# atoms-ufrj/atomsmm

Measured on AMD Instinct MI355X. Metric: ns/day on 100k-atom TIP3P RESPA box; near-nonbonded HBM GB/s vs 8 TB/s peak, higher is better.
Workload: dtype f64

## Files before the change

atomsmm_amd/backend.py:

```python
import ctypes as C
import os

import numpy as np

HERE = os.path.dirname(os.path.abspath(__file__))
LIB_PATH = os.environ.get('AMM_LIB') or os.path.join(HERE, 'libatomsmm_hip.so')

NEAR_NONE, NEAR_SHIFT, NEAR_FSWITCH, DAMPED, NONBONDED, SOFTCORE, LJ_VIRIAL = range(7)
GUARD_RC0, COULOMB_EWALD, COULOMB_RF, SWITCH, NO_SHIFT, GROUP_LJ, GROUP_Q = 1, 2, 4, 8, 16, 32, 64
BOND_HARMONIC, ANGLE_HARMONIC, BOND_LJC, BOND_NEAR, TORSION_PERIODIC, BOND_EWALD_EXCL = range(6)
BOND_VIRIAL_HARMONIC, BOND_VIRIAL_LJ = 6, 7
OP_EVAL, OP_KICK, OP_MOVE, OP_COPY, OP_COMBINE, OP_EXPR, OP_BATH = 1, 2, 3, 4, 5, 6, 7
OP_SAVE_REF, OP_CONSTRAIN_X, OP_CONSTRAIN_V = 8, 9, 10
OP_ALLREDUCE = 11
EXCHANGE_REDUCE, EXCHANGE_GATHER = 0, 1
COMM_ID_BYTES = 128
MAX_SLOTS, SLOT_X, SLOT_V = 64, 62, 63
MAX_STATES = 64
GROUP_ALL = 32
KC = 138.935456
ARITY = {BOND_HARMONIC: 2, ANGLE_HARMONIC: 3, BOND_LJC: 2, BOND_NEAR: 2, TORSION_PERIODIC: 4, BOND_EWALD_EXCL: 2,
         BOND_VIRIAL_HARMONIC: 2, BOND_VIRIAL_LJ: 2}
NPAR = {BOND_HARMONIC: 2, ANGLE_HARMONIC: 2, BOND_LJC: 3, BOND_NEAR: 3, TORSION_PERIODIC: 3, BOND_EWALD_EXCL: 1,
        BOND_VIRIAL_HARMONIC: 2, BOND_VIRIAL_LJ: 3}

EXPORTS = [
    'amm_abi_version', 'amm_last_error', 'amm_create', 'amm_destroy', 'amm_set_stream', 'amm_set_slice',
    'amm_synchronize', 'amm_check', 'amm_pair_create', 'amm_pair_set_params', 'amm_pair_share_list', 'amm_bonded_create',
    'amm_bonded_add_terms', 'amm_bonded_finalize', 'amm_bonded_set_sliced', 'amm_bonded_release', 'amm_force_eval', 'amm_kick',
    'amm_move', 'amm_copy', 'amm_mvv', 'amm_bind_state', 'amm_bind_buffer', 'amm_group_define', 'amm_run_ops',
    'amm_set_fuse_inner', 'amm_set_outer_skin',
    'amm_pair_get_stats', 'amm_profile_enable', 'amm_profile_read', 'amm_pair_count_within', 'amm_pair_row_padding', 'amm_kernel_revision',
    'amm_pme_create', 'amm_pme_set_charges', 'amm_pme_set_sliced', 'amm_pair_set_lambda', 'amm_pair_set_lambda_dev', 'amm_expr_eval', 'amm_expr_eval_scalar', 'amm_expr_define', 'amm_expr_seed', 'amm_bath_define', 'amm_bath_define_nhl', 'amm_bath_define_sin', 'amm_iso_define', 'amm_regulated_define', 'amm_bath_define_regulated', 'amm_pair_energy_derivative', 'amm_constraints_create', 'amm_pair_set_scale',
    'amm_comm_unique_id', 'amm_comm_init', 'amm_comm_destroy', 'amm_comm_allreduce', 'amm_comm_stats', 'amm_group_set_exchange', 'amm_bind_exchange', 'amm_exchange_finish',
    'amm_set_option', 'amm_positions_changed', 'amm_exchange_per', 'amm_run_stats', 'amm_run_ops_from', 'amm_exchange_pending',
    'amm_pair_energy_states',
]


class PairDesc(C.Structure):
    _fields_ = [('family', C.c_int32), ('flags', C.c_int32), ('degree', C.c_int32), ('pad_', C.c_int32),
                ('sign', C.c_double), ('rc', C.c_double), ('rswitch', C.c_double), ('rc0', C.c_double),
                ('rs0', C.c_double), ('alpha', C.c_double), ('Kc', C.c_double), ('krf', C.c_double),
                ('crf', C.c_double)]


class Op(C.Structure):
    _fields_ = [('op', C.c_int32), ('a', C.c_int32), ('b', C.c_int32), ('c', C.c_int32), ('coef', C.c_double)]


class PairStats(C.Structure):
    _fields_ = [('n_builds', C.c_int64), ('n_evals', C.c_int64), ('n_list_pairs', C.c_int64),
                ('n_slice_atoms', C.c_int64), ('capacity', C.c_int32), ('max_neighbors', C.c_int32),
                ('lanes_per_atom', C.c_int32), ('n_cells', C.c_int32), ('rlist', C.c_double),
                ('shares_list', C.c_int32), ('list_kind', C.c_int32), ('n_outer_builds', C.c_int64),
                ('n_outer_pairs', C.c_int64), ('rlist_outer', C.c_double), ('tab_error', C.c_double),
                ('has_table', C.c_int32), ('rode_along', C.c_int32),
                ('has_site_table', C.c_int32), ('n_rest_atoms', C.c_int32), ('site_tab_error', C.c_double),
                ('n_candidates', C.c_int32), ('n_candidate_walks', C.c_int32), ('chargeless', C.c_int32), ('build_split', C.c_int32)]


def slice_per(n, world):
    return 3 * (((n + 2) // 3 + world - 1) // world)


def pair_desc(family, rc, rc0=0.0, rs0=0.0, rswitch=0.0, alpha=0.0, degree=1, flags=0, sign=1.0, Kc=KC,
              krf=0.0, crf=0.0):
    return PairDesc(int(family), int(flags), int(degree), 0, float(sign), float(rc), float(rswitch), float(rc0),
                    float(rs0), float(alpha), float(Kc), float(krf), float(crf))


class HipError(RuntimeError):
    pass


class _LiveSet:

    def __init__(self):
        import weakref
        self._refs = weakref.WeakValueDictionary()

    def add(self, obj):
        self._refs[id(obj)] = obj

    def discard(self, obj):
        self._refs.pop(id(obj), None)

    def close_all(self):
        for obj in list(self._refs.values()):
            try:
                obj.close()
            except Exception:
                pass


_LIVE = _LiveSet()
import atexit
atexit.register(_LIVE.close_all)


_LIB = None


def kernel_revision():
    return lib().amm_kernel_revision().decode()


def lib():
    global _LIB
    if _LIB is None:
        if not os.path.exists(LIB_PATH):
            raise HipError('libatomsmm_hip.so not found at %s: build it with `python -m atomsmm_amd.build` '
                           '(hipcc --offload-arch=gfx950). The HIP path has no CPU fallback.' % LIB_PATH)
        L = C.CDLL(LIB_PATH)
        vp, dp, ip = C.c_void_p, C.POINTER(C.c_double), C.POINTER(C.c_int32)
        L.amm_kernel_revision.restype = C.c_char_p
        revision = L.amm_kernel_revision().decode()
        if revision.endswith('-tune') and os.environ.get('AMM_ALLOW_TUNE') != '1':
            raise HipError('%s is a tuning build (kernel revision %s): rebuild with `python -m atomsmm_amd.build --force`, or set '
                           'AMM_ALLOW_TUNE=1 for a probe script' % (LIB_PATH, revision))
        L.amm_abi_version.restype = C.c_int
        L.amm_last_error.restype = C.c_char_p
        L.amm_create.argtypes = [C.c_int32, dp, C.c_int32, vp, C.POINTER(vp)]
        L.amm_destroy.argtypes = [vp]
        L.amm_set_stream.argtypes = [vp, vp]
        L.amm_set_slice.argtypes = [vp, C.c_int32, C.c_int32]
        L.amm_synchronize.argtypes = [vp]
        L.amm_comm_unique_id.argtypes = [C.c_char_p, C.c_char_p]
        L.amm_comm_init.argtypes = [vp, C.c_char_p, C.c_char_p, C.c_int32, C.c_int32]
        L.amm_comm_allreduce.argtypes = [vp, vp, C.c_int64]
        L.amm_comm_destroy.argtypes = [vp]
        L.amm_comm_stats.argtypes = [vp, C.POINTER(C.c_int64)]
        L.amm_run_stats.argtypes = [vp, C.POINTER(C.c_int64)]
        L.amm_group_set_exchange.argtypes = [vp, C.c_int32, C.c_int32]
        L.amm_bind_exchange.argtypes = [vp, vp, C.c_int64]
        L.amm_exchange_finish.argtypes = [vp]
        L.amm_exchange_pending.argtypes = [vp, C.POINTER(C.c_int32)]
        L.amm_check.argtypes = [vp]
        L.amm_pair_create.argtypes = [vp, C.POINTER(PairDesc), dp, dp, dp, ip, C.c_int32, C.c_double, ip]
# ... 289 lines not shown
                                 int(counter) & (2 ** 64 - 1), _ptr(dst), _ptr(total)))

    def force_eval(self, fid, pos, force, accumulate=False, energy=None):
        _chk(lib().amm_force_eval(self.h, fid, _ptr(pos), _ptr(force), int(bool(accumulate)), _ptr(energy)))

    def kick(self, v, f, mass, coef, fsub=None, fadd=None):
        second = fsub if fsub is not None else fadd
        _chk(lib().amm_kick(self.h, _ptr(v), _ptr(f), _ptr(second), int(fadd is not None), _ptr(mass), float(coef)))

    def move(self, x, v, coef):
        _chk(lib().amm_move(self.h, _ptr(x), _ptr(v), float(coef)))

    def copy(self, dst, src):
        _chk(lib().amm_copy(self.h, _ptr(dst), _ptr(src)))

    def mvv(self, v, mass, out):
        _chk(lib().amm_mvv(self.h, _ptr(v), _ptr(mass), _ptr(out)))

    def bind_state(self, x, v, mass):
        self._keep += [x, v, mass]
        _chk(lib().amm_bind_state(self.h, _ptr(x), _ptr(v), _ptr(mass)))

    def bind_buffer(self, slot, buf):
        self._keep.append(buf)
        _chk(lib().amm_bind_buffer(self.h, slot, _ptr(buf)))

    def group_define(self, group, slot, force_ids):
        ids, p = _hi(np.asarray(force_ids, dtype=np.int32).reshape(-1))
        _chk(lib().amm_group_define(self.h, group, slot, p, len(ids)))

    def group_set_exchange(self, group, mode):
        _chk(lib().amm_group_set_exchange(self.h, int(group), int(mode)))

    def bind_exchange(self, tensor):
        self._keep.append(tensor)
        _chk(lib().amm_bind_exchange(self.h, _ptr(tensor), tensor.numel()))

    def exchange_finish(self):
        _chk(lib().amm_exchange_finish(self.h))

    def run_ops(self, ops, repeat=1):
        arr = (Op * len(ops))(*ops)
        _chk(lib().amm_run_ops(self.h, arr, len(ops), int(repeat)))

    def run_ops_host_exchanges(self, ops, repeat, exchange):
        arr = (Op * len(ops))(*ops)
        cursor = C.c_int64(0)
        total = len(ops) * int(repeat)
        while True:
            _chk(lib().amm_run_ops_from(self.h, arr, len(ops), int(repeat), C.byref(cursor)))
            nf = C.c_int32(0)
            _chk(lib().amm_exchange_pending(self.h, C.byref(nf)))
            if nf.value:
                exchange(nf.value)
            elif cursor.value >= total:
                return

    def set_outer_skin(self, skin_out):
        _chk(lib().amm_set_outer_skin(self.h, float(skin_out)))

    def set_option(self, name, value):
        _chk(lib().amm_set_option(self.h, name.encode(), float(value)))

    def positions_changed(self):
        _chk(lib().amm_positions_changed(self.h))

    def exchange_per(self):
        per = C.c_int32(0)
        _chk(lib().amm_exchange_per(self.h, C.byref(per)))
        return per.value

    def set_fuse_inner(self, on=True):
        _chk(lib().amm_set_fuse_inner(self.h, int(bool(on))))

    def synchronize(self):
        _chk(lib().amm_synchronize(self.h))

    def check(self):
        _chk(lib().amm_check(self.h))

    def pair_stats(self, fid):
        st = PairStats()
        _chk(lib().amm_pair_get_stats(self.h, fid, C.byref(st)))
        return {name: getattr(st, name) for name, _ in PairStats._fields_}

    def pair_row_padding(self, fid):
        out = (C.c_int64 * 2)()
        _chk(lib().amm_pair_row_padding(self.h, fid, out))
        return int(out[0]), int(out[1])

    def pair_count_within(self, fid, pos, r_within):
        n = C.c_int64()
        _chk(lib().amm_pair_count_within(self.h, fid, _ptr(pos), float(r_within), C.byref(n)))
        return n.value

    def profile_enable(self, on=True, only=None):
        _chk(lib().amm_profile_enable(self.h, -(int(only) + 1) if (on and only is not None) else int(bool(on))))

    def profile_read(self, fid):
        n = C.c_int64(); ms = C.c_double()
        _chk(lib().amm_profile_read(self.h, fid, C.byref(n), C.byref(ms)))
        return n.value, ms.value
```

atomsmm_amd/csrc/abi.hip:

```cpp
#include <algorithm>
#include <cmath>
#include <cstring>
#include <numeric>

#include "amm_ctx.h"
#include "cluster.h"

int amm_pair_setup_grid(amm_ctx *ctx, PairForce *pf);
static bool amm_family_allows_cluster(int family, int flags) {
    const bool tab_family = family == AMM_NEAR_NONE || family == AMM_NEAR_SHIFT || family == AMM_NEAR_FSWITCH || family == AMM_DAMPED || family == AMM_NONBONDED;
    return tab_family && !(flags & (AMM_GROUP_LJ | AMM_GROUP_Q));
}
int amm_bonded_arity(int kind);
int amm_bonded_npar(int kind);

static thread_local std::string g_error;
void amm_set_error(const std::string &msg) { g_error = msg; }

static PairForce *get_pair(amm_ctx *ctx, int id) {
    if (!ctx || id < 0 || id >= (int)ctx->forces.size() || ctx->forces[id].type != 1) {
        amm_set_error("invalid pair force id");
        return nullptr;
    }
    return ctx->forces[id].pair;
// ... 1647 lines not shown
                if (amm_bath_impl(ctx, ctx->baths[op.a], ctx->d_v, (1ull << 63) | ++ctx->expr_counter)) return 1;
            } break;
            case AMM_OP_ALLREDUCE: {
                auto bound = [&](const amm_op &o) { return o.a >= 0 && o.a < AMM_MAX_SLOTS && ctx->slots[o.a]; };
                if (!bound(op)) {
                    amm_set_error("amm_run_ops: ALLREDUCE of an unbound buffer");
                    return 1;
                }
                const size_t n3 = 3 * (size_t)ctx->n;
                double *lo = ctx->slots[op.a];
                size_t count = n3;
                while (k + 1 < n_ops && ops[k + 1].op == AMM_OP_ALLREDUCE && bound(ops[k + 1])) {
                    double *nb = ctx->slots[ops[k + 1].a];
                    if (nb == lo + count) count += n3;
                    else if (nb + n3 == lo) { lo = nb; count += n3; }
                    else break;
                    ++k;
                }
                if (amm_comm_allreduce_impl(ctx, lo, count)) return 1;
            } break;
            default: amm_set_error("amm_run_ops: unknown op"); return 1;
            }
        }
    }
    if (flush_deferred()) return 1;
    if (cursor && !yielded) *cursor = total_ops;
    if (!yielded && !ctx->own_only.empty()) {
        const std::vector<const double *> left = ctx->own_only;
        for (const double *b : left)
            if (complete(b)) return 1;
    }
    if (swapped) {
        const size_t bytes = sizeof(double) * 3 * (size_t)ctx->n;
        AMM_HIP(hipMemcpyAsync(user_x, ctx->d_x, bytes, hipMemcpyDeviceToDevice, ctx->stream));
        AMM_HIP(hipMemcpyAsync(user_v, ctx->d_v, bytes, hipMemcpyDeviceToDevice, ctx->stream));
        AMM_HIP(hipMemcpyAsync(user_f0, ctx->slots[f0_slot], bytes, hipMemcpyDeviceToDevice, ctx->stream));
    }
    bindings.restore(false);
    return 0;
}

int amm_pair_get_stats(amm_ctx *ctx, int32_t force_id, amm_pair_stats *out) {
    PairForce *pf = get_pair(ctx, force_id);
    if (!pf || !out) return 1;
    std::memset(out, 0, sizeof(*out));
    AMM_HIP(hipStreamSynchronize(ctx->stream));
    out->n_evals = pf->n_evals;
    PairForce *L = pf->host ? pf->host : pf;
    out->capacity = L->cap;
    out->lanes_per_atom = L->lpa;
    out->n_cells = L->grid.ncell;
    out->rlist = pf->rlist;
    out->n_slice_atoms = L->s_end - L->s_begin;
    out->shares_list = pf->host ? 1 : 0;
    out->list_kind = L->last_kind;
    out->tab_error = pf->tab_error;
    out->has_table = (pf->pc.tab.nint > 0 && pf->d_tab) ? 1 : 0;
    out->rode_along = pf->last_fused;
    out->chargeless = pf->last_chargeless;
    out->build_split = (L->cl && L->last_kind != 0) ? L->cl->split_parts : 0;
    out->has_site_table = (ctx->opt_site_tab && pf->d_tab_ss && pf->pc.tab.ss_first >= 0) ? 1 : 0;
    out->site_tab_error = pf->ss_error;
    out->n_rest_atoms = L->hybrid ? L->n_rest : 0;
    if (pf->small) {
        int cs[2];
        if (amm_small_group_stats(pf->small, cs)) return 1;
        out->n_candidates = cs[0];
        out->n_candidate_walks = cs[1];
    }
    if (L->last_kind >= 1 && L->cl && L->cl->built) {
        ClusterList *cl = L->cl;
        int flags[8];
        unsigned long long cnt[8];
        AMM_HIP(hipMemcpy(flags, cl->d_flags, sizeof(flags), hipMemcpyDeviceToHost));
        AMM_HIP(hipMemcpy(cnt, cl->d_counters, sizeof(cnt), hipMemcpyDeviceToHost));
        out->capacity = cl->cap;
        out->lanes_per_atom = cl->lpa;
        out->n_cells = cl->grid.ncell;
        out->n_slice_atoms = 3 * (int64_t)(cl->c_end - cl->c_begin);
        out->n_builds = (int64_t)cnt[0];
        out->n_list_pairs = 9 * (int64_t)(pf->host ? cnt[2] : cnt[1]);
        out->max_neighbors = flags[2];
        out->rlist_outer = L->desc.rc + L->skin;
        if (L->last_kind == 2 && L->rest && L->rest->built) {
            AMM_HIP(hipMemcpy(cnt, L->rest->d_counters, sizeof(cnt), hipMemcpyDeviceToHost));
            out->n_list_pairs += (int64_t)(pf->host ? cnt[2] : cnt[1]);
        }
        return 0;
    }
    if (L->built) {
        int flags[8];
        unsigned long long cnt[8];
        AMM_HIP(hipMemcpy(flags, L->d_flags, sizeof(flags), hipMemcpyDeviceToHost));
        AMM_HIP(hipMemcpy(cnt, L->d_counters, sizeof(cnt), hipMemcpyDeviceToHost));
        out->n_builds = (int64_t)cnt[0];
        out->n_outer_builds = (int64_t)cnt[4];
        out->n_outer_pairs = (int64_t)cnt[3];
        out->rlist_outer = L->desc.rc + L->skin_out;
        out->n_list_pairs = (int64_t)(pf->host ? cnt[2] : cnt[1]);
        out->max_neighbors = flags[2];
    }
    return 0;
}

int amm_pair_row_padding(amm_ctx *ctx, int32_t force_id, int64_t out[2]) {
    PairForce *pf = get_pair(ctx, force_id);
    if (!pf || !out) {
        amm_set_error("amm_pair_row_padding: null argument or not a pair force");
        return 1;
    }
    PairForce *L = pf->host ? pf->host : pf;
    out[0] = out[1] = 0;
    if (!(L->last_kind >= 1 && L->cl && L->cl->built)) return 0;
    long long v[2];
    if (amm_cluster_row_padding_impl(ctx, pf, v)) return 1;
    out[0] = v[0];
    out[1] = v[1];
    return 0;
}

int amm_pair_count_within(amm_ctx *ctx, int32_t force_id, const double *d_pos, double r_within, int64_t *count) {
    PairForce *pf = get_pair(ctx, force_id);
    if (!pf || !d_pos || !count) {
        amm_set_error("amm_pair_count_within: null argument or not a pair force");
        return 1;
    }
    long long c = 0;
    PairForce *Lw = pf->host ? pf->host : pf;
    if (Lw->last_kind >= 1 && Lw->cl && Lw->cl->built) {
        if (amm_cluster_count_within_impl(ctx, pf, d_pos, r_within, &c)) return 1;
        if (Lw->last_kind == 2 && pf->rest && Lw->rest && Lw->rest->built) {
            long long c2 = 0;
            if (amm_pair_count_within_impl(ctx, pf->rest, d_pos, r_within, &c2)) return 1;
            c += c2;
        }
    } else if (amm_pair_count_within_impl(ctx, pf, d_pos, r_within, &c)) return 1;
    *count = (int64_t)c;
    return 0;
}

const char *amm_kernel_revision(void) { return amm_kernel_revision_impl(); }

int amm_set_outer_skin(amm_ctx *ctx, double skin_out) {
    ctx->skin_out = skin_out;
    return 0;
}

int amm_set_option(amm_ctx *ctx, const char *name, double value) {
    if (!ctx || !name) {
        amm_set_error("amm_set_option: null argument");
        return 1;
    }
    const std::string k(name);
    const int v = (int)value;
    if (k == "cluster") ctx->opt_cluster = v;
    else if (k == "hybrid") ctx->opt_hybrid = v;
    else if (k == "small_group") ctx->opt_small_group = v;
    else if (k == "mixed_terms") ctx->opt_mixed_terms = v;
    else if (k == "rest_skin_factor") ctx->opt_rest_skin_factor = value;
    else if (k == "tab") ctx->opt_tab = v;
    else if (k == "site_trips") ctx->site_trips = v != 0;
    else if (k == "lanes_per_row") ctx->opt_lpa = v;
    else if (k == "build_parts") ctx->opt_parts = v;
    else if (k == "build_split") ctx->opt_build_split = v;
    else if (k == "unroll") ctx->opt_unroll = v;
    else if (k == "dual_unroll") ctx->opt_dual_unroll = v;
    else if (k == "tab_block") ctx->opt_tab_bs = v;
    else if (k == "tab_dual_block") ctx->opt_tab_dual_bs = v;
    else if (k == "no_dual") ctx->opt_no_dual = v;
    else if (k == "fuse_rows") ctx->opt_fuse_rows = v;
    else if (k == "row_phases") ctx->opt_row_phases = v;
    else if (k == "group_candidates") ctx->opt_group_candidates = v;
    else if (k == "positions_private") ctx->opt_positions_private = v;
    else if (k == "site_tab") ctx->opt_site_tab = v;
    else if (k == "no_defer") ctx->opt_no_defer = v;
    else if (k == "terms_from") ctx->opt_terms_from = v;
    else if (k == "no_term_lanes") ctx->opt_no_term_lanes = v;
    else if (k == "fuse_epilogue") ctx->opt_fuse_epilogue = v;
    else if (k == "comm_timeout") ctx->opt_comm_timeout = value;
    else if (k == "spec_assign") ctx->opt_spec_assign = v;
    else if (k == "chargeless") ctx->opt_chargeless = v;
    else if (k == "state_exchange") ctx->opt_state_exchange = v;
    else {
        amm_set_error("amm_set_option: unknown option '" + k + "'");
        return 1;
    }
    return 0;
}

int amm_run_stats(amm_ctx *ctx, int64_t out[4]) {
    if (!ctx || !out) return 1;
    out[0] = ctx->n_epilogues;
    out[1] = ctx->n_copies_current;
    out[2] = ctx->n_state_exchanges;
    out[3] = 0;
    return 0;
}

int amm_exchange_per(amm_ctx *ctx, int32_t *per) {
    if (!ctx || !per) return 1;
    *per = amm_slice_per(ctx->n, ctx->world);
    return 0;
}

int amm_set_fuse_inner(amm_ctx *ctx, int32_t on) {
    ctx->fuse_inner = on != 0;
    return 0;
}

int amm_profile_enable(amm_ctx *ctx, int32_t on) {
    ctx->profile = on != 0;
    ctx->profile_only = on < 0 ? -on - 1 : -1;
    return 0;
}

int amm_profile_read(amm_ctx *ctx, int32_t force_id, int64_t *n_launches, double *total_ms) {
    PairForce *pf = get_pair(ctx, force_id);
    if (!pf) return 1;
    AMM_HIP(hipStreamSynchronize(ctx->stream));
    double tot = 0.0;
    for (size_t k = 0; k + 1 < pf->ev_used; k += 2) {
        float ms = 0.f;
        AMM_HIP(hipEventElapsedTime(&ms, pf->ev[k], pf->ev[k + 1]));
        tot += ms;
    }
    if (n_launches) *n_launches = (int64_t)(pf->ev_used / 2);
    pf->ev_used = 0;
    if (pf->rest) {
        PairForce *rc = pf->rest;
        for (size_t k = 0; k + 1 < rc->ev_used; k += 2) {
            float ms = 0.f;
            AMM_HIP(hipEventElapsedTime(&ms, rc->ev[k], rc->ev[k + 1]));
            tot += ms;
        }
        rc->ev_used = 0;
    }
    if (total_ms) *total_ms = tot;
    return 0;
}

}
```

atomsmm_amd/csrc/amm_ctx.h:

```cpp
#pragma once
#include <hip/hip_runtime.h>

#include <cstdint>
#include <string>
#include <vector>

#include "../../include/atomsmm_hip.h"

#define AMM_WAVE 64
#define AMM_MAX_PRE 6
#define AMM_DERIV_LAMBDA 1024
#define AMM_MAX_GROUPS 33

void amm_set_error(const std::string &msg);
#define AMM_HIP(call)                                                                            \
    do {                                                                                         \
        hipError_t e_ = (call);                                                                  \
        if (e_ != hipSuccess) {                                                                  \
            amm_set_error(std::string(#call) + ": " + hipGetErrorString(e_));                    \
            return 1;                                                                            \
        }                                                                                        \
    } while (0)

struct PairTab {
// ... 200 lines not shown
};

struct RegDef {
    bool on = false;
    double alpha = 1, an_kT = 0;
};

struct IsoDef {
    bool on = false;
    double LkT = 0, Q1 = 0;
    int slot = -1;
};

struct GroupDef {
    int slot = -1;
    std::vector<int> forces;
    int exchange = 0;
};

struct PendingExchange {
    bool active = false;
    int per = 0, nf = 0;
    const int *perm = nullptr;
    double *force = nullptr, *gforce = nullptr;
    int kind = 0;
    ClusterList *cl = nullptr;
    PairForce *next = nullptr;
};

#define AMM_MAX_WATCH 4
struct ListWatch {
    const double *xref = nullptr;
    double thr2 = 0;
    int *flags = nullptr;
    long *pre_epoch = nullptr;
    const double **pre_pos = nullptr;
};

static inline int amm_slice_per(int n, int world) {
    const int nc = (n + 2) / 3;
    return 3 * ((nc + world - 1) / world);
}

struct EpiPlan {
    BondedSet *bs = nullptr;
    double *f0 = nullptr;
    int npre = 0, niter = 0;
    const double *pre_a[AMM_MAX_PRE] = {nullptr}, *pre_b[AMM_MAX_PRE] = {nullptr};
    double pre_coef[AMM_MAX_PRE] = {0};
    int pre_plus[AMM_MAX_PRE] = {0};
    double c1 = 0, d = 0, c2 = 0;
    PairForce *next = nullptr;
    int kind = 0;
    int with_move = 0;
    double dcoef = 0;
};

struct amm_ctx {
    int n = 0;
    int opt_spec_assign = 1;
    int opt_state_exchange = 1;
    int opt_chargeless = 1;
    int opt_fuse_epilogue = 1;
    const EpiPlan *epi_request = nullptr;
    bool epi_done = false;
    long long n_epilogues = 0;
    long long n_state_exchanges = 0;
    std::vector<const double *> own_only;
    long long n_copies_current = 0;
    int opt_cluster = 1;
    int opt_hybrid = 1;
    double opt_rest_skin_factor = 2.0;
    int opt_mixed_terms = 1;
    int opt_small_group = 1;
    bool creating_rest = false;
    int opt_tab = 1;
    int opt_build_split = 0;
    int opt_lpa = 0, opt_parts = 0, opt_unroll = 2, opt_dual_unroll = 2, opt_tab_bs = 0, opt_tab_dual_bs = 0;
    int opt_site_tab = 1;
    CZeroRows zero_rows = CZeroRows{0, nullptr, nullptr, nullptr};
    int opt_positions_private = 0;
    int opt_group_candidates = 1;
    int opt_row_phases = 1;
    int opt_fuse_rows = 1;
    int opt_no_dual = 0, opt_no_defer = 0, opt_terms_from = 8192, opt_no_term_lanes = 0;
    ListWatch watched[AMM_MAX_WATCH];
    int n_watched = 0;
    int device = 0;
    hipStream_t stream = nullptr;
    Box box;
    int rank = 0, world = 1;
    std::vector<ForceObj> forces;
    double *d_x = nullptr, *d_v = nullptr;
    const double *d_mass = nullptr;
    double *slots[AMM_MAX_SLOTS] = {nullptr};
    GroupDef groups[AMM_MAX_GROUPS];
    bool profile = false;
    int profile_only = -1;
    double *d_scratch = nullptr;
    double *d_expr_part = nullptr;
    double *d_fscratch = nullptr;
    ConstraintSet *constraints = nullptr;
    std::vector<ExprDef> exprs;
    std::vector<BathDef> baths;
    IsoDef iso;
    RegDef reg;
    unsigned long long expr_seed = 0, expr_counter = 0;
    double *alt_x = nullptr, *alt_v = nullptr, *alt_f = nullptr;
    bool fuse_inner = true;
    bool site_trips = true;
    long pos_epoch = 0;
    double skin_out = -1.0;
    void *comm = nullptr;
    bool comm_failed = false;
    double opt_comm_timeout = 0;
    double *d_xchg = nullptr;
    long long xchg_doubles = 0;
    PendingExchange pending;
    long long comm_calls = 0, comm_doubles = 0;
};

struct KickList {
    const double *f[4], *f2[4];
    int plus[4];
    double coef[4];
    int n;
};

#define AMM_FLAG_FAR 12
struct WatchArgs {
    int n;
    const double *xref[AMM_MAX_WATCH];
    double thr2[AMM_MAX_WATCH];
    int *flags[AMM_MAX_WATCH];
};
void amm_collect_watches(amm_ctx *ctx, WatchArgs &W);
void amm_watch_moved(amm_ctx *ctx);

int amm_comm_unique_id_impl(const char *rccl_path, unsigned char *out);
int amm_comm_init_impl(amm_ctx *ctx, const char *rccl_path, const unsigned char *id_bytes, int rank, int world);
int amm_comm_destroy_impl(amm_ctx *ctx);
int amm_comm_poll_impl(amm_ctx *ctx);
int amm_comm_wait_impl(amm_ctx *ctx, const char *who);
int amm_comm_allreduce_impl(amm_ctx *ctx, double *d_buf, size_t count);
int amm_comm_allgather_impl(amm_ctx *ctx, double *d_buf, size_t count_per_rank);
int amm_exchange_finish_impl(amm_ctx *ctx);

int amm_small_group_setup(amm_ctx *ctx, PairForce *pf, const std::vector<float> &member);
int amm_small_group_eval_impl(amm_ctx *ctx, PairForce *pf, const double *d_pos, double *d_force, int accumulate, double *d_energy,
                              BondedSet *carry_terms = nullptr, const double **own_rows = nullptr, int rows_unused = 0);
bool amm_small_group_supported(const PairForce *pf);
int amm_small_group_energy_states(amm_ctx *ctx, PairForce *pf, const double *d_pos, const double *d_lambdas, int K, double *d_out);
int amm_small_group_free(SmallGroup *sg);
int amm_small_group_failed(SmallGroup *sg);
int amm_small_group_stats(SmallGroup *sg, int out[2]);
int amm_pair_build_consts(const amm_pair_desc &d, PairConsts &pc);
int amm_pair_eval_impl(amm_ctx *ctx, PairForce *pf, const double *d_pos, double *d_force, int accumulate,
                       double *d_energy, PairForce *guest = nullptr, double *g_force = nullptr, int g_accumulate = 0,
                       int exchange = 0);
bool amm_pair_can_eval_dual(amm_ctx *ctx, PairForce *guest, PairForce *host);
bool amm_pair_can_fuse_discount(amm_ctx *ctx, PairForce *guest, PairForce *host);
int amm_pair_free(PairForce *pf);
int amm_pair_build_table(PairForce *pf);
int amm_pair_count_within_impl(amm_ctx *ctx, PairForce *pf, const double *d_pos, double r_within, long long *count);
const char *amm_kernel_revision_impl();
int amm_bonded_eval_impl(amm_ctx *ctx, BondedSet *bs, const double *d_pos, double *d_force, int accumulate,
                         double *d_energy);
int amm_bonded_finalize_impl(amm_ctx *ctx, BondedSet *bs);
int amm_bonded_eval_kicks_impl(amm_ctx *ctx, BondedSet *bs, const double *d_pos, double *d_force, int accumulate, const KickList &K,
                               int with_move, double dcoef, int terms_done = 0, const double *pair_rows = nullptr);
int amm_bonded_free(BondedSet *bs);
int amm_kicks_move_impl(amm_ctx *ctx, const double *const *fa, const double *const *fb, const int *plus, const double *coef, int nk,
                        int with_move, double dcoef);
int amm_inner_components_impl(amm_ctx *ctx, BondedSet *bs, double *x, double *v, double *f0, int npre, const double *const *pre_a,
                              const double *const *pre_b, const double *pre_coef, const int *pre_plus, double c1, double d,
                              double c2, int niter, const BathDef *bath = nullptr, double d2 = 0.0);
int amm_bath_impl(amm_ctx *ctx, const BathDef &bath, double *d_v, unsigned long long counter);
int amm_isokick_impl(amm_ctx *ctx, double *d_v, const double *d_f, const double *d_f2, int plus, const double *d_mass, double coef);
int amm_constraints_create_impl(amm_ctx *ctx, const int32_t *h_pairs, const double *h_dist, int n_cons, double tol,
                                ConstraintSet **out);
int amm_constraints_save_reference(amm_ctx *ctx, ConstraintSet *cs, const double *d_x);
int amm_constrain_positions(amm_ctx *ctx, ConstraintSet *cs, double *d_x);
int amm_constrain_velocities(amm_ctx *ctx, ConstraintSet *cs, const double *d_x, double *d_v);
int amm_constraints_failed(amm_ctx *ctx, ConstraintSet *cs);
int amm_constraints_free(ConstraintSet *cs);
int amm_fused_inner_impl(amm_ctx *ctx, BondedSet *bs, const double *x_in, const double *v_in, const double *f_in,
                         double *x_out, double *v_out, double *f_out, double c1, double d, double c2);
int amm_pme_create_impl(amm_ctx *ctx, double alpha, const int *K, double Kc, const double *h_q, PmeForce **out);
int amm_pme_set_charges_impl(amm_ctx *ctx, PmeForce *pm, const double *h_q);
int amm_pme_eval_impl(amm_ctx *ctx, PmeForce *pm, const double *d_pos, double *d_force, int accumulate, double *d_energy);
int amm_pme_set_sliced_impl(PmeForce *pm, int on);
int amm_pme_free(PmeForce *pm);
int amm_expr_eval_scalar_impl(amm_ctx *ctx, const int32_t *code, int n_code, const double *consts, int n_consts, double *d_scalars,
                              int n_scalars);
int amm_expr_eval_impl(amm_ctx *ctx, const int32_t *code, int n_code, const double *consts, int n_consts, const double *globals,
                       int n_globals, unsigned long long seed, unsigned long long counter, double *d_dst, double *d_sum);
int amm_kick_impl(amm_ctx *ctx, double *d_v, const double *d_f, const double *d_f2, int plus, const double *d_mass, double coef);
int amm_combine_impl(amm_ctx *ctx, double *d_dst, const double *d_a, const double *d_b, double coef);
int amm_move_impl(amm_ctx *ctx, double *d_x, const double *d_v, double coef);
int amm_copy_impl(amm_ctx *ctx, double *d_dst, const double *d_src);
int amm_mvv_impl(amm_ctx *ctx, const double *d_v, const double *d_m, double *d_out);
int amm_reduce_add(amm_ctx *ctx, const double *d_part, int n, double scale, double *d_out);
```

atomsmm_amd/csrc/bonded.hip:

```cpp
#include <algorithm>
#include <cmath>
#include <type_traits>
#include <cstring>

#include "amm_ctx.h"
#include "cluster.h"
#include "expr_vm.h"
#include "pair_math.h"

#include "bonded_terms.h"

template <class P, bool LOCAL = false>
__device__ __forceinline__ void bonded_atom(const BondedArgs &A, const P &pos, int iglobal, int i, double *f, double &esum) {
    const int rb = A.ref_ptr[iglobal], re = A.ref_ptr[iglobal + 1];
    for (int r = rb; r < re; ++r) {
        const int4 at = LOCAL ? A.rec_l[r] : A.rec_a[r];
        const double4 q = A.rec_q[r];
        const long long code = __double_as_longlong(q.w);
        const int kind = (int)(code & 7), role = (int)((code >> 3) & 3), periodic = (int)((code >> 5) & 1);
        const int ix[4] = {at.x, at.y, at.z, at.w};
        const double p[3] = {q.x, q.y, q.z};
        double fo[4][3], e;
        bonded_term_forces(A, pos, ix, p, kind, periodic, fo, e);
#pragma unroll
// ... 467 lines not shown
            const int ix[4] = {al.x, al.y, al.z, al.w};
            const double p[3] = {q.x, q.y, q.z};
            double fo[4][3], e;
            bonded_term_forces(A, pos, ix, p, kind, periodic, fo, e);
#pragma unroll
            for (int xx = 0; xx < 3; ++xx)
                f[xx] += role == 0 ? fo[0][xx] : (role == 1 ? fo[1][xx] : (role == 2 ? fo[2][xx] : fo[3][xx]));
        };
        if (TERMS) {
            double fo[4][3] = {{0.0, 0.0, 0.0}, {0.0, 0.0, 0.0}, {0.0, 0.0, 0.0}, {0.0, 0.0, 0.0}};
            if (my_tl.x >= 0) {
                const long long code = __double_as_longlong(my_tq.w);
                const int ix[4] = {my_tl.x, my_tl.y, my_tl.z, my_tl.w};
                const double p[3] = {my_tq.x, my_tq.y, my_tq.z};
                double e;
                bonded_term_forces(A, pos, ix, p, HONLY ? (int)(code & 1) : (int)(code & 7), (int)((code >> 5) & 1), fo, e);
            }
#pragma unroll
            for (int r = 0; r < (HONLY ? 3 : 4); ++r)
#pragma unroll
                for (int xx = 0; xx < 3; ++xx) s_out[TERMS ? r * 3 + xx : 0][TERMS ? threadIdx.x : 0] = fo[r][xx];
            __builtin_amdgcn_fence(__ATOMIC_RELEASE, "wavefront");
            __builtin_amdgcn_wave_barrier();
            __builtin_amdgcn_fence(__ATOMIC_ACQUIRE, "wavefront");
            const double *so = &s_out[0][0];
#pragma unroll
            for (int t = 0; t < 4; ++t)
                if (t < rec_n) {
                    f[0] += so[TERMS ? rec_at[t] : 0];
                    f[1] += so[TERMS ? rec_at[t] + 256 : 0];
                    f[2] += so[TERMS ? rec_at[t] + 512 : 0];
                }
            if (rec_n > 4) {
                unsigned long long rr = my_recs >> 20;
                for (int t = 4; t < rec_n; ++t) {
                    const int rcode = (int)(rr & 31ull);
                    rr >>= 5;
                    const int src = gbase + (rcode & 7), row = 3 * (rcode >> 3);
                    f[0] += s_out[TERMS ? row : 0][TERMS ? src : 0];
                    f[1] += s_out[TERMS ? row + 1 : 0][TERMS ? src : 0];
                    f[2] += s_out[TERMS ? row + 2 : 0][TERMS ? src : 0];
                }
            }
        } else
        for (int t = 0; t < nrec; ++t) {
            const bool cached = t < MAXR;
            const int4 al = cached ? s_tl[cached ? t : 0][threadIdx.x] : A.rec_l[rb + t];
            const double4 q = cached ? s_tq[cached ? t : 0][threadIdx.x] : A.rec_q[rb + t];
            do_rec(al, q);
        }
        {
#pragma clang fp contract(off)
#pragma unroll
            for (int j = 0; j < 3; ++j) {
                if (ISO && C.iso) {
                    amm_iso_kick(v[j], u1[j], f[j], m, C.c2, C.iso_LkT, C.iso_Q1);
                    continue;
                }
                const double num = C.c2 * f[j];
                const double dv = amm_div_mass(num, m, rm, rok);
                v[j] = v[j] + dv;
            }
        }
    }
    if (has) {
#pragma unroll
        for (int j = 0; j < 3; ++j) {
            C.x[3 * a + j] = x[j];
            C.v[3 * a + j] = v[j];
            C.f0[3 * a + j] = f[j];
        }
        if (BATH) {
            if (C.bath_kind >= 1) {
#pragma unroll
                for (int j = 0; j < 3; ++j) C.bath_w[3 * a + j] = w[j];
            }
        }
        if (ISO && C.iso) {
#pragma unroll
            for (int j = 0; j < 3; ++j) C.iso_v1[3 * a + j] = u1[j];
        }
        for (int q = 0; q < C.nwatch; ++q) {
            const double dx = x[0] - C.wref[q][3 * a], dy = x[1] - C.wref[q][3 * a + 1], dz = x[2] - C.wref[q][3 * a + 2];
            const double d2 = dx * dx + dy * dy + dz * dz;
            if (!(d2 <= C.wthr2[q])) {
                C.wflags[q][0] = 1;
                if (!(d2 <= 4.0 * C.wthr2[q])) C.wflags[q][AMM_FLAG_FAR] = 1;
            }
        }
    }
}

static const int kArity[8] = {2, 3, 2, 2, 4, 2, 2, 2};
static const int kNpar[8] = {2, 2, 3, 3, 3, 1, 2, 3};

int amm_bonded_finalize_impl(amm_ctx *ctx, BondedSet *bs) {
    const int n = ctx->n;
    std::vector<int> cnt(n + 1, 0);
    for (int kind = 0; kind < 8; ++kind) {
        const int nt = (int)bs->h_idx[kind].size() / kArity[kind];
        bs->n_terms[kind] = nt;
        for (int t = 0; t < nt; ++t)
            for (int r = 0; r < kArity[kind]; ++r) {
                int a = bs->h_idx[kind][t * kArity[kind] + r];
                if (a < 0 || a >= n) {
                    amm_set_error("bonded term references an atom index out of range");
                    return 1;
                }
                cnt[a + 1]++;
            }
        if (nt >= (1 << 26)) {
            amm_set_error("too many bonded terms of one kind");
            return 1;
        }
    }
    for (int i = 0; i < n; ++i) cnt[i + 1] += cnt[i];
    const size_t nref = (size_t)cnt[n];
    std::vector<int4> rec_a(nref);
    std::vector<double4> rec_q(nref);
    std::vector<int> rec_src(nref);
    std::vector<int> fill(cnt.begin(), cnt.end() - 1);
    int gterm = 0;
    for (int kind = 0; kind < 8; ++kind)
        for (int t = 0; t < bs->n_terms[kind]; ++t, ++gterm)
            for (int r = 0; r < kArity[kind]; ++r) {
                const int a = bs->h_idx[kind][t * kArity[kind] + r];
                const size_t slot = (size_t)fill[a]++;
                rec_src[slot] = gterm * 4 + r;
                int at[4] = {-1, -1, -1, -1};
                for (int k = 0; k < kArity[kind]; ++k) at[k] = bs->h_idx[kind][t * kArity[kind] + k];
                rec_a[slot] = make_int4(at[0], at[1], at[2], at[3]);
                double pr[3] = {0.0, 0.0, 0.0};
                for (int k = 0; k < kNpar[kind]; ++k) pr[k] = bs->h_par[kind][(size_t)t * kNpar[kind] + k];
                const long long code = (long long)kind | ((long long)r << 3) | ((long long)(bs->periodic[kind] ? 1 : 0) << 5);
                double w;
                std::memcpy(&w, &code, sizeof(w));
                rec_q[slot] = make_double4(pr[0], pr[1], pr[2], w);
            }
    std::vector<int> parent(n);
    for (int i = 0; i < n; ++i) parent[i] = i;
    auto find = [&](int a) {
        while (parent[a] != a) {
            parent[a] = parent[parent[a]];
            a = parent[a];
        }
        return a;
    };
    for (int kind = 0; kind < 8; ++kind)
        for (int t = 0; t < bs->n_terms[kind]; ++t)
            for (int r = 1; r < kArity[kind]; ++r) {
                int a = find(bs->h_idx[kind][t * kArity[kind]]), b = find(bs->h_idx[kind][t * kArity[kind] + r]);
                if (a != b) parent[std::max(a, b)] = std::min(a, b);
            }
    std::vector<int> comp_of(n), csize;
    std::vector<int> root_to_comp(n, -1);
    for (int i = 0; i < n; ++i) {
        int r = find(i);
        if (root_to_comp[r] < 0) {
            root_to_comp[r] = (int)csize.size();
            csize.push_back(0);
        }
        comp_of[i] = root_to_comp[r];
        csize[comp_of[i]]++;
    }
    const int ncomp = (int)csize.size();
    int maxc = 0;
    for (int c2 = 0; c2 < ncomp; ++c2) maxc = std::max(maxc, csize[c2]);
    std::vector<int> comp_ptr(ncomp + 1, 0), comp_atoms(n), local_of(n);
    for (int c2 = 0; c2 < ncomp; ++c2) comp_ptr[c2 + 1] = comp_ptr[c2] + csize[c2];
    {
        std::vector<int> fillc(comp_ptr.begin(), comp_ptr.end() - 1);
// ... 509 lines not shown
```

atomsmm_amd/csrc/bonded_terms.h:

```cpp
#pragma once
#include "amm_ctx.h"
#include "pair_math.h"

struct BondedArgs {
    int n, row_begin, row_end;
    const int *ref_ptr;
    const int4 *rec_a;
    const double4 *rec_q;
    const int4 *rec_l;
    const double *pos;
    double *force;
    double *epart;
    int accumulate, want_energy;
    Box box;
    PairConsts near_pc;
    double ewald_alpha, ewald_tasp;
    double Kc_ljc;
};

struct PosPlain {
    const double *pos;
    __device__ __forceinline__ double get(int a, int k) const { return pos[3 * a + k]; }
};
struct PosAdvanced {
    const double *x, *v, *f, *m;
    double c1, d;
    __device__ __forceinline__ double vel(int a, int k) const {
#pragma clang fp contract(off)
        const double num = c1 * f[3 * a + k];
        const double dv = num / m[a];
        return v[3 * a + k] + dv;
    }
    __device__ __forceinline__ double get(int a, int k) const {
#pragma clang fp contract(off)
        const double dx = d * vel(a, k);
        return x[3 * a + k] + dx;
    }
};

__device__ __forceinline__ double amm_reg_dx(double v, double m, double coef, double alpha, double an_kT) {
#pragma clang fp contract(off)
    const double c = sqrt(an_kT / m);
    const double t = tanh((alpha * v) / c);
    return (c * t) * coef;
}

__device__ __forceinline__ void amm_watch_atom(const WatchArgs &W, int a, const double *xn) {
    for (int q = 0; q < W.n; ++q) {
        const double dx = xn[0] - W.xref[q][3 * a], dy = xn[1] - W.xref[q][3 * a + 1], dz = xn[2] - W.xref[q][3 * a + 2];
        const double d2 = dx * dx + dy * dy + dz * dz;
        if (!(d2 <= W.thr2[q])) {
            W.flags[q][0] = 1;
            if (!(d2 <= 4.0 * W.thr2[q])) W.flags[q][AMM_FLAG_FAR] = 1;
        }
    }
}

__device__ __forceinline__ double amm_div_mass(double num, double m, double r, bool exact_r) {
    const double q = num * r;
    const double e = fma(-q, m, num);
    const double fast = fma(e, r, q);
    if (__builtin_amdgcn_ballot_w64(!exact_r) == 0ull) return fast;
    return exact_r ? fast : num / m;
}

struct PosLds {
    const double *sx, *sy, *sz;
    __device__ __forceinline__ double get(int slot, int k) const { return k == 0 ? sx[slot] : (k == 1 ? sy[slot] : sz[slot]); }
};

template <class P>
__device__ __forceinline__ void delta3(const P &pos, int a, int b, const Box &box, int periodic, double *d) {
#pragma unroll
    for (int k = 0; k < 3; ++k) {
        double v = pos.get(a, k) - pos.get(b, k);
        if (periodic) v = amm_min_image(v, box.L[k], box.invL[k]);
        d[k] = v;
    }
}
__device__ __forceinline__ double dot3(const double *a, const double *b) { return a[0] * b[0] + a[1] * b[1] + a[2] * b[2]; }
__device__ __forceinline__ void cross3(const double *a, const double *b, double *c) {
    c[0] = a[1] * b[2] - a[2] * b[1];
    c[1] = a[2] * b[0] - a[0] * b[2];
    c[2] = a[0] * b[1] - a[1] * b[0];
}

template <class P>
__device__ __forceinline__ void bonded_term_forces(const BondedArgs &A, const P &pos, const int *ix, const double *p, int kind,
                                                   int periodic, double fo[4][3], double &e) {
    switch (kind) {
    case AMM_BOND_HARMONIC: {
        double d[3];
        delta3(pos, ix[0], ix[1], A.box, periodic, d);
        const double r2 = dot3(d, d);
        const double rinv = amm_rsqrt(r2);
        const double dr = r2 * rinv - p[0];
        const double fr = -p[1] * dr * rinv;
#pragma unroll
        for (int x = 0; x < 3; ++x) {
            fo[0][x] = fr * d[x];
            fo[1][x] = -fo[0][x];
        }
        e = 0.5 * p[1] * dr * dr;
    } break;
    case AMM_ANGLE_HARMONIC: {
        double d1[3], d2[3];
        delta3(pos, ix[0], ix[1], A.box, periodic, d1);
        delta3(pos, ix[2], ix[1], A.box, periodic, d2);
        const double i1 = amm_rsqrt(dot3(d1, d1)), i2 = amm_rsqrt(dot3(d2, d2));
        double c = dot3(d1, d2) * i1 * i2;
        c = c > 1.0 ? 1.0 : (c < -1.0 ? -1.0 : c);
        const double th = acos(c), dth = th - p[0];
        double s2 = 1.0 - c * c;
        if (s2 < 1e-24) s2 = 1e-24;
        const double g = p[1] * dth * amm_rsqrt(s2);
#pragma unroll
        for (int x = 0; x < 3; ++x) {
            const double u1 = d1[x] * i1, u2 = d2[x] * i2;
            const double fi = g * (u2 - c * u1) * i1;
            const double fk = g * (u1 - c * u2) * i2;
            fo[0][x] = fi;
            fo[2][x] = fk;
            fo[1][x] = -(fi + fk);
        }
        e = 0.5 * p[1] * dth * dth;
    } break;
    case AMM_BOND_LJC:
    case AMM_BOND_NEAR: {
        double d[3];
        delta3(pos, ix[0], ix[1], A.box, periodic, d);
        const double r2 = dot3(d, d);
        double fr;
        if (kind == AMM_BOND_LJC) {
            const double rinv2 = 1.0 / r2, rinv = sqrt(rinv2);
            const double s2 = p[1] * p[1] * rinv2, x6 = s2 * s2 * s2;
            e = 4.0 * p[2] * x6 * (x6 - 1.0) + A.Kc_ljc * p[0] * rinv;
            fr = (4.0 * p[2] * (12.0 * x6 * x6 - 6.0 * x6) + A.Kc_ljc * p[0] * rinv) * rinv2;
// ... 76 lines not shown
```

atomsmm_amd/csrc/cluster.h:

```cpp
#pragma once
#include "amm_ctx.h"

struct ClusterList {
    int nc = 0;
    const int *d_first = nullptr;
    const int *d_rest = nullptr;
    int nrest = 0;
    bool built = false;
    CellGrid grid;
    int capc = 0;
    int parts = 1;
    int *d_slice_cells = nullptr;
    int split_parts = 0;
    double rext = 0;
    double rlist_build = 0, rnear_build = 0, skin = 0;
    int *d_cell_count = nullptr, *d_cell_start = nullptr, *d_cell_members = nullptr;
    int *d_cperm = nullptr;
    int *d_aperm = nullptr;
    float4 *d_pos4f = nullptr;
    double *d_xref = nullptr;
    int c_begin = 0, c_end = 0;
    int cap = 0;
    int lpa = 8;
    int *d_nl = nullptr, *d_nnb = nullptr, *d_nnb_near = nullptr;
    int *d_flags = nullptr;
    unsigned long long *d_counters = nullptr;
    unsigned long long *d_blockstats = nullptr;
    int *d_ticket = nullptr;
    long checked_epoch = -1, pre_epoch = -1;
    const double *checked_pos = nullptr, *pre_pos = nullptr;
    PairForce *sorted_for = nullptr;
    long sorted_epoch = -1;
    const double *sorted_pos = nullptr;
    int *d_spec_count[2] = {nullptr, nullptr};
    int *d_spec_ticket = nullptr;
    int spec_parity = 0;
    long assigned_epoch = -1;
    const double *assigned_pos = nullptr;
    bool per_pair_image = false;
};

void amm_cluster_classify(int n, const std::vector<int> &excl_ptr, const std::vector<int> &excl_idx, std::vector<int> &mol_first,
                          std::vector<int> &rest);
int amm_cluster_eval_impl(amm_ctx *ctx, PairForce *pf, const double *d_pos, double *d_force, int accumulate, PairForce *guest,
                          double *g_force, int g_accumulate, int exchange);
int amm_cluster_count_within_impl(amm_ctx *ctx, PairForce *pf, const double *d_pos, double r_within, long long *count);
int amm_cluster_row_padding_impl(amm_ctx *ctx, PairForce *pf, long long out[2]);
int amm_cluster_state_finish_impl(amm_ctx *ctx);
int amm_cluster_free(ClusterList *cl);
```

atomsmm_amd/csrc/cluster.hip:

```cpp
#include <algorithm>
#include <cmath>
#include <cstdio>
#include <cstdlib>
#include <cstring>
#include <type_traits>
#include <vector>

#include "amm_ctx.h"
#include "bonded_terms.h"
#include "cluster.h"
#include "device_utils.h"
#include "pair_math.h"
#include "pair_tab.h"

#ifndef AMM_EXP_NOLJ
#define AMM_EXP_NOLJ 0
#endif

__device__ double amm_erfcx_table_dev_c[AMM_ERFCX_NI * AMM_ERFCX_NC];
static bool g_erfcx_uploaded_c[64] = {false};

void amm_cluster_classify(int n, const std::vector<int> &ptr, const std::vector<int> &idx, std::vector<int> &mol_first, std::vector<int> &rest) {
    mol_first.clear();
    rest.clear();
    auto own_pairs_only = [&](int i, int i0) {
        if (ptr[i + 1] - ptr[i] != 2) return false;
        const int a = i - i0;
        const int p0 = i0 + (a == 0 ? 1 : 0), p1 = i0 + (a == 2 ? 1 : 2);
        const int e0 = idx[ptr[i]], e1 = idx[ptr[i] + 1];
        return (e0 == p0 && e1 == p1) || (e0 == p1 && e1 == p0);
    };
    int i = 0;
    while (i < n) {
        if (i + 2 < n && own_pairs_only(i, i) && own_pairs_only(i + 1, i) && own_pairs_only(i + 2, i)) {
            mol_first.push_back(i);
            i += 3;
        } else {
            rest.push_back(i);
            i += 1;
        }
    }
}

__device__ __forceinline__ double cwrap1(double x, double L, double invL) {
    double w = x - L * floor(x * invL);
    if (w >= L) w -= L;
    if (w < 0.0) w = 0.0;
    return w;
}

__global__ void k_ccheck_displacement(int n, const double *__restrict__ pos, const double *__restrict__ xref, double thr2, int *flags) {
    const int i = blockIdx.x * blockDim.x + threadIdx.x;
    if (i >= n) return;
    const double dx = pos[3 * i] - xref[3 * i], dy = pos[3 * i + 1] - xref[3 * i + 1], dz = pos[3 * i + 2] - xref[3 * i + 2];
    const double d2 = dx * dx + dy * dy + dz * dz;
    if (!(d2 <= thr2)) {
        flags[0] = 1;
        if (!(d2 <= 4.0 * thr2)) flags[AMM_FLAG_FAR] = 1;
    }
}

__device__ __forceinline__ int cfirst(const int *__restrict__ first, int m) { return first ? first[m] : 3 * m; }

__global__ void __launch_bounds__(256) k_cassign(int nc, const double *__restrict__ pos, Box box, CellGrid g, int *count, int *start,
                                                 int *members, int capc, double *xref, int *flags, int *ticket, int force,
                                                 const int *__restrict__ first, const int *__restrict__ rest, int nrest) {
    if (!force && !flags[0]) return;
    const int m = blockIdx.x * blockDim.x + threadIdx.x;
    if (m >= nc && m < nc + nrest && xref) {
        const int i = rest[m - nc];
#pragma unroll
        for (int k = 0; k < 3; ++k) xref[3 * i + k] = pos[3 * i + k];
    }
    if (m < nc) {
        const int i0 = cfirst(first, m);
        int cidx[3];
#pragma unroll
        for (int k = 0; k < 3; ++k) {
            const double w = cwrap1(pos[3 * i0 + k], box.L[k], box.invL[k]);
            const int ck = (w == w) ? (int)(w * g.inv_cw[k]) : 0;
            cidx[k] = ck >= g.nc[k] ? g.nc[k] - 1 : (ck < 0 ? 0 : ck);
        }
        const int cell = (cidx[2] * g.nc[1] + cidx[1]) * g.nc[0] + cidx[0];
        const int rank = atomicAdd(&count[cell], 1);
        if (members) {
            if (rank < capc) members[(size_t)cell * capc + rank] = m;
            else flags[7] = 1;
        }
    }
    if (!amm_last_block(ticket)) return;
    const int fullest = amm_block_scan_counts(g.ncell, count, start);
    if (threadIdx.x == 0) flags[6] = fullest;
}

__device__ __forceinline__ double csorted_image(double x, double x0, double sh, double L, double invL) {
    return x + (sh - L * rint((x - x0) * invL));
}

__device__ __forceinline__ void cgather_one(int c, int i0, const double *__restrict__ pos, Box box, const double *__restrict__ q,
                                            const double *__restrict__ hsig, const double *__restrict__ seps2, double4 *posq_s, double2 *lj_s) {
    double sh[3];
#pragma unroll
    for (int k = 0; k < 3; ++k) sh[k] = cwrap1(pos[3 * i0 + k], box.L[k], box.invL[k]) - pos[3 * i0 + k];
#pragma unroll
    for (int a = 0; a < 3; ++a) {
        const int i = i0 + a;
        double4 p;
        p.x = csorted_image(pos[3 * i], pos[3 * i0], sh[0], box.L[0], box.invL[0]);
        p.y = csorted_image(pos[3 * i + 1], pos[3 * i0 + 1], sh[1], box.L[1], box.invL[1]);
        p.z = csorted_image(pos[3 * i + 2], pos[3 * i0 + 2], sh[2], box.L[2], box.invL[2]);
        p.w = q[i];
        posq_s[3 * c + a] = p;
        lj_s[3 * c + a] = make_double2(hsig[i], seps2[i]);
    }
}

__global__ void __launch_bounds__(256) k_csort_gather(int ncell, int nc, const int *__restrict__ start, const int *__restrict__ members,
                                                      int capc, int *cperm, int *aperm, const double *__restrict__ pos, Box box,
                                                      float4 *pos4f, const int *flags, int *wflags, int force, const double *__restrict__ q,
                                                      const double *__restrict__ hsig, const double *__restrict__ seps2, double4 *posq_s,
                                                      double2 *lj_s, float rext, const double *__restrict__ site_eps,
                                                      const int *__restrict__ first, CZeroRows Z, int copies_current, double *xref,
                                                      int c_begin, int c_end, int *slice_cells) {
    const int gid = blockIdx.x * blockDim.x + threadIdx.x;
    if (gid < Z.n) {
        const int i = Z.idx[gid];
        if (Z.f0) Z.f0[3 * i] = Z.f0[3 * i + 1] = Z.f0[3 * i + 2] = 0.0;
        if (Z.f1) Z.f1[3 * i] = Z.f1[3 * i + 1] = Z.f1[3 * i + 2] = 0.0;
    }
    if (!force && !flags[0]) {
        if (!copies_current && posq_s && gid < nc) cgather_one(gid, cfirst(first, cperm[gid]), pos, box, q, hsig, seps2, posq_s, lj_s);
        return;
    }
    const int wave = gid >> 6, lane = threadIdx.x & 63;
    if (wave >= ncell) return;
    const int b = start[wave];
    const int cnt = min(start[wave + 1] - b, capc);
    if (lane == 0 && c_begin < c_end) {
        if (b <= c_begin && c_begin < start[wave + 1]) slice_cells[0] = wave;
        if (b <= c_end - 1 && c_end - 1 < start[wave + 1]) slice_cells[1] = wave;
    }
    const int *mem = members + (size_t)wave * capc;
    for (int a0 = 0; a0 < cnt; a0 += 64) {
        const int a = a0 + lane;
        const int me = a < cnt ? mem[a] : 0x7fffffff;
        int rank = 0;
        for (int k0 = 0; k0 < cnt; k0 += 64) {
            const int kk = k0 + lane;
            const int other = kk < cnt ? mem[kk] : 0x7fffffff;
            const int nk = min(64, cnt - k0);
            for (int jj = 0; jj < nk; ++jj) rank += __builtin_amdgcn_readlane(other, jj) < me;
        }
        if (a >= cnt) continue;
        const int sl = b + rank;
        cperm[sl] = me;
        const int i0 = cfirst(first, me);
        double sh[3], p0[3];
#pragma unroll
        for (int k = 0; k < 3; ++k) {
            p0[k] = pos[3 * i0 + k];
            sh[k] = cwrap1(p0[k], box.L[k], box.invL[k]) - p0[k];
        }
        float ext2 = 0.f;
        int sites = 0;
        float4 pf[3];
#pragma unroll
        for (int t = 0; t < 3; ++t) {
            const int i = i0 + t;
            aperm[3 * sl + t] = i;
            const double x = csorted_image(pos[3 * i], p0[0], sh[0], box.L[0], box.invL[0]);
            const double y = csorted_image(pos[3 * i + 1], p0[1], sh[1], box.L[1], box.invL[1]);
            const double z = csorted_image(pos[3 * i + 2], p0[2], sh[2], box.L[2], box.invL[2]);
            if (xref) {
                xref[3 * i] = pos[3 * i];
                xref[3 * i + 1] = pos[3 * i + 1];
                xref[3 * i + 2] = pos[3 * i + 2];
            }
            pf[t] = make_float4((float)x, (float)y, (float)z, 0.f);
            const float dx = pf[t].x - pf[0].x, dy = pf[t].y - pf[0].y, dz = pf[t].z - pf[0].z;
            ext2 = fmaxf(ext2, dx * dx + dy * dy + dz * dz);
            if (site_eps[i] != 0.0) sites |= 1 << t;
            if (posq_s) {
                posq_s[3 * sl + t] = make_double4(x, y, z, q[i]);
                lj_s[3 * sl + t] = make_double2(hsig[i], seps2[i]);
            }
        }
        const float ext = sqrtf(ext2) * 1.000001f + 1e-6f;
        if (!(ext <= rext)) wflags[7] = 1;
        pf[0].w = ext;
        pf[1].w = __int_as_float(sites);
        pos4f[3 * sl] = pf[0];
        pos4f[3 * sl + 1] = pf[1];
        pos4f[3 * sl + 2] = pf[2];
    }
}

struct CBoxF {
    float L[3], invL[3];
};

#ifndef CB_BATCH
#define CB_BATCH 5
#endif
#define CB_COARSE 256
#define CB_QCAP 256
__device__ __forceinline__ int cq_wrap(int i) { return i & (CB_QCAP - 1); }
typedef float v2f __attribute__((ext_vector_type(2)));

__device__ void cfinish_build_block(int *flags, unsigned long long *counters, const unsigned long long *blockstats, int nblocks, int count_only) {
    __shared__ unsigned long long sh_part[4][3];
    unsigned long long sum = 0, mx = 0, nr = 0;
    for (int b0 = threadIdx.x; b0 < nblocks; b0 += 8 * 256) {
        unsigned long long v[8][3];
#pragma unroll
        for (int j = 0; j < 8; ++j) {
            const int b = b0 + j * 256;
            const bool in = b < nblocks;
#pragma unroll
            for (int q = 0; q < 3; ++q) v[j][q] = in ? amm_ld_l2(&blockstats[3 * (in ? b : 0) + q]) : 0ull;
        }
#pragma unroll
        for (int j = 0; j < 8; ++j) {
            sum += v[j][0];
            mx = max(mx, v[j][1]);
            nr += v[j][2];
        }
    }
    for (int off = 32; off > 0; off >>= 1) {
        sum += __shfl_xor(sum, off);
        nr += __shfl_xor(nr, off);
        mx = max(mx, __shfl_xor(mx, off));
    }
    if ((threadIdx.x & 63) == 0) {
        sh_part[threadIdx.x >> 6][0] = sum;
        sh_part[threadIdx.x >> 6][1] = mx;
        sh_part[threadIdx.x >> 6][2] = nr;
    }
    __syncthreads();
    if (threadIdx.x == 0) {
        flags[2] = (int)max(max(sh_part[0][1], sh_part[1][1]), max(sh_part[2][1], sh_part[3][1]));
        counters[1] = sh_part[0][0] + sh_part[1][0] + sh_part[2][0] + sh_part[3][0];
        counters[2] = sh_part[0][2] + sh_part[1][2] + sh_part[2][2] + sh_part[3][2];
        if (!count_only) {
            flags[0] = 0;
            flags[AMM_FLAG_FAR] = 0;
            counters[0] += 1;
        }
    }
}

#ifndef CB_WAVES
#define CB_WAVES 5
#endif
#define CB_OCC __attribute__((amdgpu_waves_per_eu(CB_WAVES)))
#ifdef AMM_CBS_TIMING
__device__ unsigned long long g_cbs_t[8];
#define CBS_STAMP(i) do { const unsigned long long now_ = wall_clock64(); if (w == 0 && lane == 0) atomicAdd(&g_cbs_t[i], now_ - t_last); t_last = now_; } while (0)
#else
#define CBS_STAMP(i) do { } while (0)
#endif
template <bool COUNT_ONLY, bool RINT, bool SLICE = false>
__global__ void __launch_bounds__(256) __attribute__((amdgpu_waves_per_eu(SLICE ? 3 : CB_WAVES))) k_cbuild(int c_begin, int c_end, int parts, const int *__restrict__ cell_start,
                                                const float4 *__restrict__ pos4f, CBoxF box, CellGrid g, float rlist, float rnear2, int cap,
                                                int *nl, int *nnb, int *nnb_near, int *flags, unsigned long long *blockstats,
                                                unsigned long long *counters, int *ticket, int force, const int *slice_cells) {
    if (!force && !flags[0]) return;
    __shared__ int s_rstart[4][128];
    __shared__ int s_rpref[4][128];
    __shared__ float s_rshift[4][3][128];
    __shared__ int s_q[4][CB_BATCH][CB_QCAP];
    __shared__ unsigned char s_coarse[4][CB_COARSE];
    const int lane = threadIdx.x & 63, w = threadIdx.x >> 6;
    const int wave = __builtin_amdgcn_readfirstlane((int)((blockIdx.x * blockDim.x + threadIdx.x) >> 6));
    const float FAR = 1.0e9f;
    const float rlist2 = rlist * rlist;
    unsigned long long wsum = 0, wnear = 0;
    int wmax = 0;
    const int first_cell = SLICE ? __builtin_amdgcn_readfirstlane(slice_cells[0]) : 0;
    const int nunits = SLICE ? (__builtin_amdgcn_readfirstlane(slice_cells[1]) - first_cell + 1) * parts : g.ncell * parts;
    int unit = wave;
#ifdef AMM_CBS_TIMING
    unsigned long long t_last = wall_clock64(), t_drain = 0, n_drain = 0;
#endif
    do {
    const int c = unit < nunits ? first_cell + unit / parts : g.ncell, part = unit % parts;
    int a_begin = 0, a_end = 0;
    if (c < g.ncell) {
        const int cb0 = __builtin_amdgcn_readfirstlane(cell_start[c]), cb1 = __builtin_amdgcn_readfirstlane(cell_start[c + 1]);
        const int per = (cb1 - cb0 + parts - 1) / parts;
        a_begin = max(cb0 + part * per, c_begin);
        a_end = min(min(cb0 + (part + 1) * per, cb1), c_end);
    }
    if (a_begin < a_end) {
        const int ncx = g.nc[0], ncy = g.nc[1], ncz = g.nc[2];
        const int cx = c % ncx, cy = (c / ncx) % ncy, cz = c / (ncx * ncy);
        const int nsx = g.nstencil[0], nsy = g.nstencil[1], ne = nsx * nsy * g.nstencil[2];
        int total;
        {
            int ecs[2] = {0, 0}, len[2] = {0, 0}, inc[2];
            float esx[2] = {0.f, 0.f}, esy[2] = {0.f, 0.f}, esz[2] = {0.f, 0.f};
#pragma unroll
            for (int hh = 0; hh < 2; ++hh) {
                const int e = lane + 64 * hh;
                if (e < ne) {
                    const int ox = e % nsx, oy = (e / nsx) % nsy, oz = e / (nsx * nsy);
                    int nz = ncz < 2 * g.h[2] + 1 ? oz : cz - g.h[2] + oz;
                    esz[hh] = nz < 0 ? -box.L[2] : (nz >= ncz ? box.L[2] : 0.f);
                    nz = nz < 0 ? nz + ncz : (nz >= ncz ? nz - ncz : nz);
                    int ny = ncy < 2 * g.h[1] + 1 ? oy : cy - g.h[1] + oy;
                    esy[hh] = ny < 0 ? -box.L[1] : (ny >= ncy ? box.L[1] : 0.f);
                    ny = ny < 0 ? ny + ncy : (ny >= ncy ? ny - ncy : ny);
                    int nx = ncx < 2 * g.h[0] + 1 ? ox : cx - g.h[0] + ox;
                    esx[hh] = nx < 0 ? -box.L[0] : (nx >= ncx ? box.L[0] : 0.f);
                    nx = nx < 0 ? nx + ncx : (nx >= ncx ? nx - ncx : nx);
                    const int cc = (nz * ncy + ny) * ncx + nx;
                    ecs[hh] = cell_start[cc];
                    len[hh] = cell_start[cc + 1] - ecs[hh];
                }
                inc[hh] = len[hh];
                for (int off = 1; off < 64; off <<= 1) {
                    const int v = __shfl_up(inc[hh], off);
                    if (lane >= off) inc[hh] += v;
                }
            }
            const int lower = __builtin_amdgcn_readlane(inc[0], 63);
            total = lower + __builtin_amdgcn_readlane(inc[1], 63);
#pragma unroll
            for (int hh = 0; hh < 2; ++hh) {
                s_rstart[w][lane + 64 * hh] = ecs[hh];
                s_rpref[w][lane + 64 * hh] = (hh ? lower : 0) + inc[hh] - len[hh];
                s_rshift[w][0][lane + 64 * hh] = esx[hh];
                s_rshift[w][1][lane + 64 * hh] = esy[hh];
                s_rshift[w][2][lane + 64 * hh] = esz[hh];
            }
            __builtin_amdgcn_fence(__ATOMIC_RELEASE, "wavefront");
            __builtin_amdgcn_wave_barrier();
            __builtin_amdgcn_fence(__ATOMIC_ACQUIRE, "wavefront");
        }
        int cshift = 3;
        while (((total + 127) >> cshift) > CB_COARSE) ++cshift;
#pragma unroll
        for (int q = 0; q < CB_COARSE / 64; ++q) {
            const int idx = (lane + 64 * q) << cshift;
            int r = 0;
#pragma unroll
            for (int step = 64; step > 0; step >>= 1)
                if (s_rpref[w][r + step] <= idx) r += step;
            s_coarse[w][lane + 64 * q] = (unsigned char)r;
// ... 8 lines not shown
            const int nt = min(CB_BATCH, a_end - tb);
            float4 my = make_float4(0.f, 0.f, 0.f, 0.f);
            if (lane < 3 * nt) my = pos4f[3 * tb + lane];
            int row_cnt = 0;
            int q_head = 0, q_cnt = 0;
            auto rl = [&](float v, int l) { return __int_as_float(__builtin_amdgcn_readlane(__float_as_int(v), l)); };
            auto drain = [&](int t, int n) {
#ifdef AMM_CBS_TIMING
                const unsigned long long t_d0 = wall_clock64();
                n_drain++;
#endif
                const int head = __builtin_amdgcn_readlane(q_head, t);
                int slot[2];
                bool v[2];
                float4 A[2][3];
#pragma unroll
                for (int u = 0; u < 2; ++u) {
                    const bool v0 = lane + 64 * u < n;
                    slot[u] = v0 ? s_q[w][t][cq_wrap(head + lane + 64 * u)] : tb + t;
                    v[u] = v0 && slot[u] != tb + t;
                }
#pragma unroll
                for (int u = 0; u < 2; ++u)
#pragma unroll
                    for (int b = 0; b < 3; ++b) A[u][b] = pos4f[3 * slot[u] + b];
                const int sites[2] = {__float_as_int(A[0][1].w), __float_as_int(A[1][1].w)};
                float px[3], py[3], pz[3];
#pragma unroll
                for (int a = 0; a < 3; ++a) {
                    px[a] = rl(my.x, 3 * t + a);
                    py[a] = rl(my.y, 3 * t + a);
                    pz[a] = rl(my.z, 3 * t + a);
                }
                v2f ax[3], ay[3], az[3];
#pragma unroll
                for (int b = 0; b < 3; ++b) {
                    ax[b] = v2f{A[0][b].x, A[1][b].x};
                    ay[b] = v2f{A[0][b].y, A[1][b].y};
                    az[b] = v2f{A[0][b].z, A[1][b].z};
                }
                if (!RINT) {
                    const v2f sx = box.L[0] * __builtin_elementwise_rint((ax[0] - px[0]) * box.invL[0]);
                    const v2f sy = box.L[1] * __builtin_elementwise_rint((ay[0] - py[0]) * box.invL[1]);
                    const v2f sz = box.L[2] * __builtin_elementwise_rint((az[0] - pz[0]) * box.invL[2]);
#pragma unroll
                    for (int b = 0; b < 3; ++b) {
                        ax[b] -= sx;
                        ay[b] -= sy;
                        az[b] -= sz;
                    }
                }
                v2f m2 = v2f{3.0e38f, 3.0e38f};
#pragma unroll
                for (int a = 0; a < 3; ++a)
#pragma unroll
                    for (int b = 0; b < 3; ++b) {
                        v2f dx = px[a] - ax[b], dy = py[a] - ay[b], dz = pz[a] - az[b];
                        if (RINT) {
                            dx -= box.L[0] * __builtin_elementwise_rint(dx * box.invL[0]);
                            dy -= box.L[1] * __builtin_elementwise_rint(dy * box.invL[1]);
                            dz -= box.L[2] * __builtin_elementwise_rint(dz * box.invL[2]);
                        }
                        v2f r2 = dx * dx;
                        r2 = __builtin_elementwise_fma(dy, dy, r2);
                        r2 = __builtin_elementwise_fma(dz, dz, r2);
                        m2 = __builtin_elementwise_min(m2, r2);
                    }
#pragma unroll
                for (int u = 0; u < 2; ++u) {
                    const float m2u = u ? m2.y : m2.x;
                    const bool pass = v[u] && m2u < rlist2;
                    const unsigned long long m_pass = __builtin_amdgcn_ballot_w64(pass);
                    if (m_pass != 0ull) {
                        const bool is_near = pass && m2u < rnear2;
                        const unsigned long long m_near = __builtin_amdgcn_ballot_w64(is_near);
                        const int np_ = __popcll(m_pass), nn_ = __popcll(m_near);
                        const int c2 = __builtin_amdgcn_readlane(row_cnt, t);
                        const int cnt = c2 & 0xffff, cntf = (int)((unsigned)c2 >> 16);
                        if (!COUNT_ONLY) {
                            const int mp = __builtin_amdgcn_mbcnt_hi((unsigned)(m_pass >> 32), __builtin_amdgcn_mbcnt_lo((unsigned)m_pass, 0u));
                            const int mn = __builtin_amdgcn_mbcnt_hi((unsigned)(m_near >> 32), __builtin_amdgcn_mbcnt_lo((unsigned)m_near, 0u));
                            const int pos_near = cnt + mn, pos_far = (cap - 1 - cntf) - (mp - mn);
                            if (cnt + cntf + np_ <= cap) {
                                int *row_out = nl + (size_t)(tb + t - c_begin) * cap;
                                if (pass) row_out[is_near ? pos_near : pos_far] = slot[u] | (sites[u] << 29);
                            }
                        }
                        row_cnt = lane == t ? c2 + nn_ + ((np_ - nn_) << 16) : row_cnt;
                    }
                }
                q_head = lane == t ? cq_wrap(head + n) : q_head;
                q_cnt = lane == t ? q_cnt - n : q_cnt;
#ifdef AMM_CBS_TIMING
                t_drain += wall_clock64() - t_d0;
#endif
            };
            auto fetch = [&](int cb, float4 (&cand)[2], int (&js)[2]) {
#pragma unroll
                for (int u = 0; u < 2; ++u) {
                    const int idx = cb + u * 64 + lane;
                    const bool in = idx < total;
                    int r = s_coarse[w][idx >> cshift];
                    while (r < 127 && s_rpref[w][r + 1] <= idx) ++r;
                    const int slot = in ? s_rstart[w][r] + idx - s_rpref[w][r] : 0;
                    float4 q = pos4f[3 * slot];
                    if (!RINT) {
                        const float sx = s_rshift[w][0][r], sy = s_rshift[w][1][r], sz = s_rshift[w][2][r];
                        q.x = in ? q.x + sx : FAR;
                        q.y = in ? q.y + sy : FAR;
                        q.z = in ? q.z + sz : FAR;
                    } else if (!in) {
                        q.w = -1.0e9f;
                    }
                    cand[u] = q;
                    js[u] = slot;
                }
            };
            float4 cand[2], cand_n[2];
            int js[2], js_n[2];
            fetch(0, cand, js);
            const float plim_l = my.w + rlist;
            for (int cb = 0; cb < total; cb += 128) {
                if (cb + 128 < total) fetch(cb + 128, cand_n, js_n);
                const v2f cx = v2f{cand[0].x, cand[1].x}, cy = v2f{cand[0].y, cand[1].y}, cz = v2f{cand[0].z, cand[1].z};
                const v2f cw = v2f{cand[0].w, cand[1].w};
                for (int t = 0; t < nt; ++t) {
                    const float p0x = rl(my.x, 3 * t), p0y = rl(my.y, 3 * t), p0z = rl(my.z, 3 * t), plim = rl(plim_l, 3 * t);
                    int qn = __builtin_amdgcn_readlane(q_cnt, t);
                    const int head = __builtin_amdgcn_readlane(q_head, t);
                    v2f dx = p0x - cx, dy = p0y - cy, dz = p0z - cz;
                    if (RINT) {
                        dx -= box.L[0] * __builtin_elementwise_rint(dx * box.invL[0]);
                        dy -= box.L[1] * __builtin_elementwise_rint(dy * box.invL[1]);
                        dz -= box.L[2] * __builtin_elementwise_rint(dz * box.invL[2]);
                    }
                    v2f r2 = dx * dx;
                    r2 = __builtin_elementwise_fma(dy, dy, r2);
                    r2 = __builtin_elementwise_fma(dz, dz, r2);
                    const v2f lim = plim + cw;
                    const v2f lim2 = lim * lim;
#pragma unroll
                    for (int u = 0; u < 2; ++u) {
                        const bool pass = (u ? r2.y < lim2.y : r2.x < lim2.x) && (!RINT || (u ? lim.y : lim.x) > 0.f);
                        const unsigned long long m = __builtin_amdgcn_ballot_w64(pass);
                        if (m == 0ull) continue;
                        const int at = qn + __builtin_amdgcn_mbcnt_hi((unsigned)(m >> 32), __builtin_amdgcn_mbcnt_lo((unsigned)m, 0u));
                        if (pass) s_q[w][t][cq_wrap(head + at)] = js[u];
                        qn += __popcll(m);
                    }
                    q_cnt = lane == t ? qn : q_cnt;
                    if (qn >= 128) {
                        __builtin_amdgcn_fence(__ATOMIC_RELEASE, "wavefront");
                        __builtin_amdgcn_wave_barrier();
                        __builtin_amdgcn_fence(__ATOMIC_ACQUIRE, "wavefront");
                        drain(t, 128);
                    }
                }
#pragma unroll
                for (int u = 0; u < 2; ++u) {
                    cand[u] = cand_n[u];
                    js[u] = js_n[u];
                }
            }
            __builtin_amdgcn_fence(__ATOMIC_RELEASE, "wavefront");
            __builtin_amdgcn_wave_barrier();
            __builtin_amdgcn_fence(__ATOMIC_ACQUIRE, "wavefront");
            for (int t = 0; t < nt; ++t) {
                const int n = __builtin_amdgcn_readlane(q_cnt, t);
                if (n > 0) drain(t, n);
            }
            __builtin_amdgcn_fence(__ATOMIC_RELEASE, "wavefront");
            __builtin_amdgcn_wave_barrier();
            if (lane < nt) {
                const int count = row_cnt & 0xffff, countf = (int)((unsigned)row_cnt >> 16);
                const int total_nb = count + countf;
                if (!COUNT_ONLY) {
                    const bool over = total_nb > cap;
                    nnb[tb + lane - c_begin] = over ? 0 : total_nb;
                    nnb_near[tb + lane - c_begin] = over ? 0 : count;
                    if (over) flags[1] = 1;
                }
                wsum += (unsigned long long)total_nb;
                wnear += (unsigned long long)count;
                wmax = max(wmax, total_nb);
            }
        }
    }
#ifdef AMM_CBS_TIMING
    if (SLICE && lane == 0 && a_begin < a_end) { atomicAdd(&g_cbs_t[1], wall_clock64() - t_last); atomicAdd(&g_cbs_t[2], t_drain); atomicAdd(&g_cbs_t[3], n_drain); }
#endif
    unit += (int)(gridDim.x * (blockDim.x >> 6));
    } while (SLICE && unit < nunits);
    for (int off = 32; off > 0; off >>= 1) {
        wsum += __shfl_xor(wsum, off);
        wnear += __shfl_xor(wnear, off);
        wmax = max(wmax, __shfl_xor(wmax, off));
    }
    __shared__ unsigned long long s_sum[4], s_near[4];
    __shared__ int s_max[4];
    if (lane == 0) {
        s_sum[w] = wsum;
        s_near[w] = wnear;
        s_max[w] = wmax;
    }
    __syncthreads();
    if (threadIdx.x == 0) {
        amm_st_l2(&blockstats[3 * blockIdx.x], s_sum[0] + s_sum[1] + s_sum[2] + s_sum[3]);
        amm_st_l2(&blockstats[3 * blockIdx.x + 1], (unsigned long long)max(max(s_max[0], s_max[1]), max(s_max[2], s_max[3])));
        amm_st_l2(&blockstats[3 * blockIdx.x + 2], s_near[0] + s_near[1] + s_near[2] + s_near[3]);
    }
    if (amm_last_block(ticket)) cfinish_build_block(flags, counters, blockstats, (int)gridDim.x, COUNT_ONLY ? 1 : 0);
}

#ifndef CBS_BATCH
#define CBS_BATCH 3
#endif
#ifndef CBS_SEG
#define CBS_SEG 384
#endif
#define CBS_MAXCH (4 * CBS_SEG / 128)
template <bool RINT>
__global__ void __launch_bounds__(256) k_cbuild_split(int c_begin, int c_end, int parts, const int *__restrict__ cell_start,
                                                      const float4 *__restrict__ pos4f, CBoxF box, CellGrid g, float rlist, float rnear2, int cap,
                                                      int *nl, int *nnb, int *nnb_near, int *flags, unsigned long long *blockstats,
                                                      unsigned long long *counters, int *ticket, int force, const int *slice_cells) {
    if (!force && !flags[0]) return;
    __shared__ int s_rstart[128];
    __shared__ int s_rpref[128];
    __shared__ float s_rshift[3][128];
    __shared__ unsigned char s_coarse[CB_COARSE];
    __shared__ int s_total;
    __shared__ int s_ring[4][CBS_BATCH][CBS_SEG];
    __shared__ int s_cnt[4][CBS_BATCH];
    __shared__ int s_stage[CBS_BATCH * CBS_MAXCH][128];
    __shared__ int s_ccnt[CBS_BATCH * CBS_MAXCH];
    const int lane = threadIdx.x & 63, w = threadIdx.x >> 6;
    const float FAR = 1.0e9f;
    const float rlist2 = rlist * rlist;
    unsigned long long wsum = 0, wnear = 0;
    int wmax = 0;
    const int first_cell = __builtin_amdgcn_readfirstlane(slice_cells[0]);
    const int nunits = (__builtin_amdgcn_readfirstlane(slice_cells[1]) - first_cell + 1) * parts;
    for (int unit = (int)blockIdx.x; unit < nunits; unit += (int)gridDim.x) {
    const int c = first_cell + unit / parts, part = unit % parts;
    int a_begin = 0, a_end = 0;
    if (c < g.ncell) {
        const int cb0 = __builtin_amdgcn_readfirstlane(cell_start[c]), cb1 = __builtin_amdgcn_readfirstlane(cell_start[c + 1]);
        const int per = (cb1 - cb0 + parts - 1) / parts;
        a_begin = max(cb0 + part * per, c_begin);
        a_end = min(min(cb0 + (part + 1) * per, cb1), c_end);
    }
    if (a_begin < a_end) {
#ifdef AMM_CBS_TIMING
        unsigned long long t_last = wall_clock64();
        if (w == 0 && lane == 0) atomicAdd(&g_cbs_t[7], 1ull);
#endif
        const int ncx = g.nc[0], ncy = g.nc[1], ncz = g.nc[2];
        const int cx = c % ncx, cy = (c / ncx) % ncy, cz = c / (ncx * ncy);
        if (w == 0) {
            const int nsx = g.nstencil[0], nsy = g.nstencil[1], ne = nsx * nsy * g.nstencil[2];
            int ecs[2] = {0, 0}, len[2] = {0, 0}, inc[2];
            float esx[2] = {0.f, 0.f}, esy[2] = {0.f, 0.f}, esz[2] = {0.f, 0.f};
#pragma unroll
            for (int hh = 0; hh < 2; ++hh) {
                const int e = lane + 64 * hh;
                if (e < ne) {
                    const int ox = e % nsx, oy = (e / nsx) % nsy, oz = e / (nsx * nsy);
                    int nz = ncz < 2 * g.h[2] + 1 ? oz : cz - g.h[2] + oz;
                    esz[hh] = nz < 0 ? -box.L[2] : (nz >= ncz ? box.L[2] : 0.f);
                    nz = nz < 0 ? nz + ncz : (nz >= ncz ? nz - ncz : nz);
                    int ny = ncy < 2 * g.h[1] + 1 ? oy : cy - g.h[1] + oy;
                    esy[hh] = ny < 0 ? -box.L[1] : (ny >= ncy ? box.L[1] : 0.f);
                    ny = ny < 0 ? ny + ncy : (ny >= ncy ? ny - ncy : ny);
                    int nx = ncx < 2 * g.h[0] + 1 ? ox : cx - g.h[0] + ox;
                    esx[hh] = nx < 0 ? -box.L[0] : (nx >= ncx ? box.L[0] : 0.f);
                    nx = nx < 0 ? nx + ncx : (nx >= ncx ? nx - ncx : nx);
                    const int cc = (nz * ncy + ny) * ncx + nx;
                    ecs[hh] = cell_start[cc];
                    len[hh] = cell_start[cc + 1] - ecs[hh];
                }
                inc[hh] = len[hh];
                for (int off = 1; off < 64; off <<= 1) {
                    const int v = __shfl_up(inc[hh], off);
                    if (lane >= off) inc[hh] += v;
                }
            }
            const int lower = __builtin_amdgcn_readlane(inc[0], 63);
            if (lane == 0) s_total = lower + __builtin_amdgcn_readlane(inc[1], 63);
#pragma unroll
            for (int hh = 0; hh < 2; ++hh) {
                s_rstart[lane + 64 * hh] = ecs[hh];
                s_rpref[lane + 64 * hh] = (hh ? lower : 0) + inc[hh] - len[hh];
                s_rshift[0][lane + 64 * hh] = esx[hh];
                s_rshift[1][lane + 64 * hh] = esy[hh];
                s_rshift[2][lane + 64 * hh] = esz[hh];
            }
        }
        __syncthreads();
        const int total = s_total;
        int cshift = 3;
        while (((total + 127) >> cshift) > CB_COARSE) ++cshift;
        {
            const int idx = (int)threadIdx.x << cshift;
            int r = 0;
#pragma unroll
            for (int step = 64; step > 0; step >>= 1)
                if (s_rpref[r + step] <= idx) r += step;
            s_coarse[threadIdx.x] = (unsigned char)r;
// ... 76 lines not shown
                CBS_STAMP(1);
                if (lane < CBS_BATCH) s_cnt[w][lane] = q_cnt;
                __syncthreads();
                CBS_STAMP(2);
                int j0 = 0;
                for (int t = 0; t < nt; ++t) {
                    const int c0 = __builtin_amdgcn_readfirstlane(s_cnt[0][t]), c1 = c0 + __builtin_amdgcn_readfirstlane(s_cnt[1][t]);
                    const int c2 = c1 + __builtin_amdgcn_readfirstlane(s_cnt[2][t]), T = c2 + __builtin_amdgcn_readfirstlane(s_cnt[3][t]);
                    const int nch = (T + 127) >> 7;
                    for (int k = 0; k < nch; ++k) {
                        const int j = j0 + k;
                        if ((j & 3) != w) continue;
                        const int n = min(128, T - 128 * k);
                        int slot[2];
                        bool v[2];
                        float4 A[2][3];
#pragma unroll
                        for (int u = 0; u < 2; ++u) {
                            const int gi = 128 * k + lane + 64 * u;
                            const bool v0 = lane + 64 * u < n;
                            const int ww = (gi >= c0 ? 1 : 0) + (gi >= c1 ? 1 : 0) + (gi >= c2 ? 1 : 0);
                            const int off = gi - (ww == 0 ? 0 : (ww == 1 ? c0 : (ww == 2 ? c1 : c2)));
                            slot[u] = v0 ? s_ring[ww][t][off] : tb + t;
                            v[u] = v0 && slot[u] != tb + t;
                        }
#pragma unroll
                        for (int u = 0; u < 2; ++u)
#pragma unroll
                            for (int b = 0; b < 3; ++b) A[u][b] = pos4f[3 * slot[u] + b];
                        const int sites[2] = {__float_as_int(A[0][1].w), __float_as_int(A[1][1].w)};
                        float px[3], py[3], pz[3];
#pragma unroll
                        for (int a = 0; a < 3; ++a) {
                            px[a] = rl(my.x, 3 * t + a);
                            py[a] = rl(my.y, 3 * t + a);
                            pz[a] = rl(my.z, 3 * t + a);
                        }
                        v2f ax[3], ay[3], az[3];
#pragma unroll
                        for (int b = 0; b < 3; ++b) {
                            ax[b] = v2f{A[0][b].x, A[1][b].x};
                            ay[b] = v2f{A[0][b].y, A[1][b].y};
                            az[b] = v2f{A[0][b].z, A[1][b].z};
                        }
                        if (!RINT) {
                            const v2f sx = box.L[0] * __builtin_elementwise_rint((ax[0] - px[0]) * box.invL[0]);
                            const v2f sy = box.L[1] * __builtin_elementwise_rint((ay[0] - py[0]) * box.invL[1]);
                            const v2f sz = box.L[2] * __builtin_elementwise_rint((az[0] - pz[0]) * box.invL[2]);
#pragma unroll
                            for (int b = 0; b < 3; ++b) {
                                ax[b] -= sx;
                                ay[b] -= sy;
                                az[b] -= sz;
                            }
                        }
                        v2f m2 = v2f{3.0e38f, 3.0e38f};
#pragma unroll
                        for (int a = 0; a < 3; ++a)
#pragma unroll
                            for (int b = 0; b < 3; ++b) {
                                v2f dx = px[a] - ax[b], dy = py[a] - ay[b], dz = pz[a] - az[b];
                                if (RINT) {
                                    dx -= box.L[0] * __builtin_elementwise_rint(dx * box.invL[0]);
                                    dy -= box.L[1] * __builtin_elementwise_rint(dy * box.invL[1]);
                                    dz -= box.L[2] * __builtin_elementwise_rint(dz * box.invL[2]);
                                }
                                v2f r2 = dx * dx;
                                r2 = __builtin_elementwise_fma(dy, dy, r2);
                                r2 = __builtin_elementwise_fma(dz, dz, r2);
                                m2 = __builtin_elementwise_min(m2, r2);
                            }
                        int cnt = 0, cntf = 0;
#pragma unroll
                        for (int u = 0; u < 2; ++u) {
                            const float m2u = u ? m2.y : m2.x;
                            const bool pass = v[u] && m2u < rlist2;
                            const unsigned long long m_pass = __builtin_amdgcn_ballot_w64(pass);
                            if (m_pass != 0ull) {
                                const bool is_near = pass && m2u < rnear2;
                                const unsigned long long m_near = __builtin_amdgcn_ballot_w64(is_near);
                                const int np_ = __popcll(m_pass), nn_ = __popcll(m_near);
                                const int mp = __builtin_amdgcn_mbcnt_hi((unsigned)(m_pass >> 32), __builtin_amdgcn_mbcnt_lo((unsigned)m_pass, 0u));
                                const int mn = __builtin_amdgcn_mbcnt_hi((unsigned)(m_near >> 32), __builtin_amdgcn_mbcnt_lo((unsigned)m_near, 0u));
                                if (pass) s_stage[j][is_near ? cnt + mn : 127 - cntf - (mp - mn)] = slot[u] | (sites[u] << 29);
                                cnt += nn_;
                                cntf += np_ - nn_;
                            }
                        }
                        if (lane == 0) s_ccnt[j] = cnt | (cntf << 16);
                    }
                    j0 += nch;
                }
                CBS_STAMP(3);
                __syncthreads();
                CBS_STAMP(4);
                j0 = 0;
                for (int t = 0; t < nt; ++t) {
                    const int T = __builtin_amdgcn_readfirstlane(s_cnt[0][t] + s_cnt[1][t] + s_cnt[2][t] + s_cnt[3][t]);
                    const int nch = (T + 127) >> 7;
                    const int have = __builtin_amdgcn_readlane(row_cnt, t);
                    int nf = have & 0xffff, nb_ = (int)((unsigned)have >> 16);
                    int *row_out = nl + (size_t)(tb + t - c_begin) * cap;
                    for (int k = 0; k < nch; ++k) {
                        const int j = j0 + k;
                        const int cc = __builtin_amdgcn_readfirstlane(s_ccnt[j]);
                        const int cn = cc & 0xffff, cf = (int)((unsigned)cc >> 16);
                        if ((j & 3) == w && nf + nb_ + cn + cf <= cap) {
                            for (int i = lane; i < cn; i += 64) row_out[nf + i] = s_stage[j][i];
                            for (int i = lane; i < cf; i += 64) row_out[cap - 1 - nb_ - i] = s_stage[j][127 - i];
                        }
                        nf = min(nf + cn, 0xffff);
                        nb_ = min(nb_ + cf, 0xffff);
                    }
                    row_cnt = lane == t ? (nf | (nb_ << 16)) : row_cnt;
                    j0 += nch;
                }
                CBS_STAMP(5);
                __syncthreads();
                CBS_STAMP(6);
            }
            if (w == 0 && lane < nt) {
                const int count = row_cnt & 0xffff, countf = (int)((unsigned)row_cnt >> 16);
                const int total_nb = count + countf;
                const bool over = total_nb > cap;
                nnb[tb + lane - c_begin] = over ? 0 : total_nb;
                nnb_near[tb + lane - c_begin] = over ? 0 : count;
                if (over) flags[1] = 1;
                wsum += (unsigned long long)total_nb;
                wnear += (unsigned long long)count;
                wmax = max(wmax, total_nb);
            }
        }
    }
    __syncthreads();
    }
    for (int off = 32; off > 0; off >>= 1) {
        wsum += __shfl_xor(wsum, off);
        wnear += __shfl_xor(wnear, off);
        wmax = max(wmax, __shfl_xor(wmax, off));
    }
    if (w == 0 && lane == 0) {
        amm_st_l2(&blockstats[3 * blockIdx.x], wsum);
        amm_st_l2(&blockstats[3 * blockIdx.x + 1], (unsigned long long)wmax);
        amm_st_l2(&blockstats[3 * blockIdx.x + 2], wnear);
    }
    if (amm_last_block(ticket)) cfinish_build_block(flags, counters, blockstats, (int)gridDim.x, 0);
}

#define AMM_CPHASES 6
struct CPairArgs {
    int c_begin, nrows, lpa_shift, cap;
    const int *aperm;
    const int *nl, *nnb, *nnb_total;
    const double4 *posq;
    const double2 *lj;
    double *force;
    int accumulate, sorted_out;
    Box box;
    const double *host_tab;
    int host_bytes;
    double margin;
    int ntask;
    int per_pair_image;
    int rpx, nphase;
    int ph_off[AMM_CPHASES], ph_shift[AMM_CPHASES], ph_ntask[AMM_CPHASES];
#ifdef AMM_CPAIR_TIMING
    unsigned long long *wave_times;
#endif
    const double *host_tab_ss;
    int host_ss_bytes, host_ss_off, site_atoms;
    double hsig_site, seps2_site;
    const double *guest_tab, *guest_tab_ss;
    int guest_bytes, guest_ss_bytes, guest_ss_off, g_accumulate;
    double *gforce;
    double gfac, gsr;
};

template <int FAM, int CMODE, int GFAM, int IMG, int SMASK>
__device__ __forceinline__ void cwalk_rows(const CPairArgs &A, const PairConsts &c, const PairConsts &g, const char *tabh, const char *tabg,
                                           const double *erfcx, const double4 (&pi)[3], const double2 *li, int i_sites, const int (&so)[3],
                                           const int (&sog)[3], double sign_lj, const int *row, int nfront, int nn, int sub, int lpa,
                                           int self, double (&f)[9], double (&fg)[9]) {
    constexpr bool DUAL = GFAM >= 0;
    constexpr bool SS = SMASK != 0;
    const int back = A.cap - 1 + nfront;
    const double r2low = DUAL ? fmax(c.tab.r2min, g.tab.r2min) : c.tab.r2min;
    const double r2low_ss = DUAL ? fmax(c.tab.ss_r2min, g.tab.ss_r2min) : c.tab.ss_r2min;
    auto entry = [&](int k) { return k < nn ? row[k < nfront ? k : back - k] : self; };
    auto load_pos = [&](int e, int b) {
        return *reinterpret_cast<const double4 *>(reinterpret_cast<const char *>(A.posq) + (size_t)((unsigned)e & 0x1fffffffu) * 96u + 32 * b);
    };
    auto load_lj = [&](int e, int b) {
        double2 l = make_double2(0.0, 0.0);
        if (i_sites != 0 && __builtin_amdgcn_ballot_w64((((unsigned)e >> 29) >> b) & 1u) != 0ull)
            l = *reinterpret_cast<const double2 *>(reinterpret_cast<const char *>(A.lj) + (size_t)((unsigned)e & 0x1fffffffu) * 48u + 16 * b);
        return l;
    };
    double4 pj[3];
    double2 lj[3];
    int k = sub;
    int e = entry(k), en = entry(k + lpa);
#pragma unroll
    for (int b = 0; b < 3; ++b) {
        pj[b] = load_pos(e, b);
        if (!SS) lj[b] = load_lj(e, b);
    }
    while (__builtin_amdgcn_ballot_w64(k < nn) != 0ull) {
        const bool ok = k < nn;
        const bool front = k < nfront;
        const bool any_front = DUAL && __builtin_amdgcn_ballot_w64(front) != 0ull;
        const unsigned bits = (unsigned)e >> 29;
        const int e2 = entry(k + 2 * lpa);
        double sx = 0.0, sy = 0.0, sz = 0.0;
        if (IMG == 1) {
            sx = A.box.L[0] * rint((pj[0].x - pi[0].x) * A.box.invL[0]);
            sy = A.box.L[1] * rint((pj[0].y - pi[0].y) * A.box.invL[1]);
            sz = A.box.L[2] * rint((pj[0].z - pi[0].z) * A.box.invL[2]);
        }
#pragma unroll
        for (int b = 0; b < 3; ++b) {
            const double xb = pj[b].x - sx, yb = pj[b].y - sy, zb = pj[b].z - sz, qb = pj[b].w;
            const int mb = SS ? -(int)((bits >> b) & 1u) : 0;
            double dx[3], dy[3], dz[3], r2[3], fr[3], gl[3];
            {
                TabLookup th[3];
#pragma unroll
                for (int a = 0; a < 3; ++a) {
                    dx[a] = pi[a].x - xb;
                    dy[a] = pi[a].y - yb;
                    dz[a] = pi[a].z - zb;
                    if (IMG == 2) {
                        dx[a] = amm_min_image(dx[a], A.box.L[0], A.box.invL[0]);
                        dy[a] = amm_min_image(dy[a], A.box.L[1], A.box.invL[1]);
                        dz[a] = amm_min_image(dz[a], A.box.L[2], A.box.invL[2]);
                    }
                    r2[a] = dx[a] * dx[a] + dy[a] * dy[a] + dz[a] * dz[a];
                    th[a] = amm_tab_fetch(tabh, c.tab, r2[a], ((SMASK >> a) & 1) ? (unsigned)(so[a] & mb) : 0u);
                    if (DUAL) gl[a] = 0.0;
                }
                __builtin_amdgcn_sched_barrier(0);
#pragma unroll
                for (int a = 0; a < 3; ++a) fr[a] = (pi[a].w * qb) * amm_tab_horner(th[a]);
            }
            if (!SS && !AMM_EXP_NOLJ && i_sites != 0 && __builtin_amdgcn_ballot_w64(ok && ((bits >> b) & 1u)) != 0ull) {
#pragma unroll
                for (int a = 0; a < 3; ++a)
                    if ((i_sites >> a) & 1) {
                        const double2 la = li[64 * a];
                        const double sig = la.x + lj[b].x, eps4 = la.y * lj[b].y;
                        const LJCommon L = amm_lj_common(r2[a], sig, eps4);
                        fr[a] = amm_sum_unfused(fr[a], amm_lj_force<FAM, CMODE>(c, L, sig, eps4));
                        if (DUAL && any_front) {
                            LJCommon Lg = L;
                            Lg.dlj_r *= A.gsr;
                            gl[a] = amm_lj_force<(DUAL ? GFAM : FAM), 0>(g, Lg, sig, eps4 * A.gsr);
                        }
                    }
            }
            bool any_low = false;
            bool lowp[3];
#pragma unroll
            for (int a = 0; a < 3; ++a) {
                bool low = r2[a] < r2low;
                if ((SMASK >> a) & 1) low = low || ((so[a] & mb) != 0 && r2[a] < r2low_ss);
                lowp[a] = low;
                const bool pass = ok && (r2[a] < c.rc2);
                any_low = any_low || (ok && low);
                const double fh = (pass && !low) ? fr[a] : 0.0;
                f[3 * a] += fh * dx[a];
                f[3 * a + 1] += fh * dy[a];
                f[3 * a + 2] += fh * dz[a];
            }
            if (DUAL) {
                __builtin_amdgcn_sched_barrier(0);
                if (any_front) {
                    TabLookup tg[3];
#pragma unroll
                    for (int a = 0; a < 3; ++a) tg[a] = amm_tab_fetch(tabg, g.tab, r2[a], ((SMASK >> a) & 1) ? (unsigned)(sog[a] & mb) : 0u);
                    __builtin_amdgcn_sched_barrier(0);
#pragma unroll
                    for (int a = 0; a < 3; ++a) {
                        const double gr = amm_sum_unfused(((pi[a].w * qb) * A.gfac) * amm_tab_horner(tg[a]), gl[a]);
                        const bool pass = front && (r2[a] < g.rc2) && !lowp[a];
                        const double gh = pass ? gr : 0.0;
                        fg[3 * a] += gh * dx[a];
                        fg[3 * a + 1] += gh * dy[a];
                        fg[3 * a + 2] += gh * dz[a];
                    }
                }
            }
            if (__builtin_amdgcn_ballot_w64(any_low) != 0ull) {
                for (int a = 0; a < 3; ++a) {
// ... 28 lines not shown
            pj[b] = load_pos(en, b);
            if (!SS) lj[b] = load_lj(en, b);
        }
        e = en;
        en = e2;
        k += lpa;
    }
}

struct CEpiPre {
    const double *a, *b;
    double coef;
    int plus;
};
struct CEpiArgs {
    int niter, npre;
    int recompute_f0;
    double *x, *v, *f0;
    const double *mass;
    double c1, d, c2;
    CEpiPre pre[AMM_MAX_PRE];
    const int *cperm;
    const int4 *term_l;
    const double4 *term_q;
    const unsigned long long *atom_recs;
    int *spec_count, *spec_clear, *spec_members, *spec_start, *spec_flags, *spec_ticket;
    int spec_capc;
    CellGrid grid;
    double *xchg_x, *xchg_v;
    int c_first;
    double4 *posq_next;
    double2 *lj_next;
    const double *q_next, *hsig_next, *seps2_next;
    WatchArgs W;
};

#ifndef CEPI_INLINE
#define CEPI_INLINE __forceinline__
#endif

struct CEpiArgs;
template <int Q>
__device__ __forceinline__ double cquad_bcast(double v) {
    constexpr int ctrl = Q | (Q << 2) | (Q << 4) | (Q << 6);
    const long long b = __double_as_longlong(v);
    const int lo = __builtin_amdgcn_mov_dpp((int)(b & 0xffffffffll), ctrl, 0xf, 0xf, true);
    const int hi = __builtin_amdgcn_mov_dpp((int)(b >> 32), ctrl, 0xf, 0xf, true);
    return __longlong_as_double(((long long)hi << 32) | (unsigned int)lo);
}

struct PosTermRegs {
    double p[3][3];
    __device__ __forceinline__ double get(int r, int k) const { return p[r][k]; }
};

__device__ __forceinline__ void cepi_positions_final(const CEpiArgs &E, const Box &box, int cs, int a, int l, int mol, bool has, const double (&x)[3],
                                                     double q_nx, double hs_nx, double se_nx) {
    double x0[3];
#pragma unroll
    for (int k = 0; k < 3; ++k) x0[k] = cquad_bcast<0>(x[k]);
    if (!has) return;
    if (l == 0 && E.spec_count) {
        int cidx[3];
#pragma unroll
        for (int k = 0; k < 3; ++k) {
            const double w = cwrap1(x[k], box.L[k], box.invL[k]);
            const int ck = (w == w) ? (int)(w * E.grid.inv_cw[k]) : 0;
            cidx[k] = ck >= E.grid.nc[k] ? E.grid.nc[k] - 1 : (ck < 0 ? 0 : ck);
        }
        const int cell = (cidx[2] * E.grid.nc[1] + cidx[1]) * E.grid.nc[0] + cidx[0];
        const int rank = atomicAdd(&E.spec_count[cell], 1);
        if (rank < E.spec_capc) E.spec_members[(size_t)cell * E.spec_capc + rank] = mol;
        else E.spec_flags[7] = 1;
    }
#pragma unroll
    for (int j = 0; j < 3; ++j) E.x[3 * a + j] = x[j];
    if (E.xchg_x) {
        const size_t sl = 3 * (size_t)(cs - E.c_first) + l;
#pragma unroll
        for (int j = 0; j < 3; ++j) E.xchg_x[3 * sl + j] = x[j];
    }
    for (int q = 0; q < E.W.n; ++q) {
        const double dx = x[0] - E.W.xref[q][3 * a], dy = x[1] - E.W.xref[q][3 * a + 1], dz = x[2] - E.W.xref[q][3 * a + 2];
        const double d2 = dx * dx + dy * dy + dz * dz;
        if (!(d2 <= E.W.thr2[q])) {
            amm_st_l2(&E.W.flags[q][0], 1);
            if (!(d2 <= 4.0 * E.W.thr2[q])) amm_st_l2(&E.W.flags[q][AMM_FLAG_FAR], 1);
        }
    }
    if (E.posq_next) {
        double4 pq;
        pq.x = csorted_image(x[0], x0[0], cwrap1(x0[0], box.L[0], box.invL[0]) - x0[0], box.L[0], box.invL[0]);
        pq.y = csorted_image(x[1], x0[1], cwrap1(x0[1], box.L[1], box.invL[1]) - x0[1], box.L[1], box.invL[1]);
        pq.z = csorted_image(x[2], x0[2], cwrap1(x0[2], box.L[2], box.invL[2]) - x0[2], box.L[2], box.invL[2]);
        pq.w = q_nx;
        E.posq_next[3 * cs + l] = pq;
        if (E.lj_next) E.lj_next[3 * cs + l] = make_double2(hs_nx, se_nx);
    }
}

#ifdef AMM_CPAIR_TIMING
#define CEPI_STAMP(k) (tstamp[k] = wall_clock64())
__device__ CEPI_INLINE void cepi_rows(const CEpiArgs &E, const Box box, int cs, bool valid, int sub, unsigned long long (&tstamp)[3]) {
#else
#define CEPI_STAMP(k)
__device__ CEPI_INLINE void cepi_rows(const CEpiArgs &E, const Box box, int cs, bool valid, int sub) {
#endif
    const int lane = threadIdx.x & 63;
    const int l = sub & 3;
    const int qb = lane - sub;
    const bool has = valid && sub < 3;
    const bool tlane = valid && sub < 4;
    const int mol = E.cperm[cs];
    const int a = 3 * mol + (l < 3 ? l : 0);
    const double m = E.mass[a];
    double x[3], v[3], f[3];
#pragma unroll
    for (int j = 0; j < 3; ++j) {
        x[j] = E.x[3 * a + j];
        v[j] = E.v[3 * a + j];
        f[j] = E.f0[3 * a + j];
    }
    int4 my_tl = make_int4(-1, -1, -1, -1);
    double4 my_tq = make_double4(0.0, 0.0, 0.0, 0.0);
    unsigned long long my_recs = 0ull;
    if (tlane) {
        my_tl = E.term_l[4 * mol + l];
        my_tq = E.term_q[4 * mol + l];
    }
    if (has) my_recs = E.atom_recs[a];
    double q_nx = 0.0, hs_nx = 0.0, se_nx = 0.0;
    if (has && E.posq_next && E.niter > 0) {
        q_nx = E.q_next[a];
        if (E.lj_next) {
            hs_nx = E.hsig_next[a];
            se_nx = E.seps2_next[a];
        }
    }
    const double rm = 1.0 / m;
    const bool rok = (__double_as_longlong(m) & 0xFFFFFFFFFFFFFll) != 0xFFFFFFFFFFFFFll && m > 1e-200 && m < 1e200;
    __builtin_amdgcn_fence(__ATOMIC_RELEASE, "workgroup");
    __builtin_amdgcn_fence(__ATOMIC_ACQUIRE, "workgroup");
    CEPI_STAMP(0);
    {
#pragma clang fp contract(off)
        double pa[4][3], pb[4][3];
#pragma unroll
        for (int p = 0; p < 4; ++p) {
            const bool on = p < E.npre;
#pragma unroll
            for (int j = 0; j < 3; ++j) {
                pa[p][j] = on ? E.pre[p].a[3 * a + j] : 0.0;
                pb[p][j] = (on && E.pre[p].b) ? E.pre[p].b[3 * a + j] : 0.0;
            }
        }
#pragma unroll
        for (int p = 0; p < 4; ++p) {
            if (p < E.npre) {
                const CEpiPre pk = E.pre[p];
#pragma unroll
                for (int j = 0; j < 3; ++j) {
                    double ff = pa[p][j];
                    if (pk.b) ff = pk.plus ? ff + pb[p][j] : ff - pb[p][j];
                    const double num = pk.coef * ff;
                    const double dv = amm_div_mass(num, m, rm, rok);
                    v[j] = v[j] + dv;
                }
            }
        }
        for (int p = 4; p < E.npre; ++p) {
            const CEpiPre pk = E.pre[p];
// ... 113 lines not shown
    if (lane == 63) {
        s_part[w] = incl;
        s_most[w] = most;
    }
    __syncthreads();
    int base = 0, all_most = 0;
#pragma unroll
    for (int k = 0; k < BS / 64; ++k) {
        if (k < w) base += s_part[k];
        all_most = max(all_most, s_most[k]);
    }
    int run = base + incl - sum;
    for (int c = c0; c < c1; ++c) {
        start[c] = run;
        run += amm_ld_l2(&count[c]);
    }
    if (t == BS - 1) start[ncell] = run;
    return all_most;
}

#ifndef AMM_CBS_SINGLE
#define AMM_CBS_SINGLE 512
#endif

#ifndef AMM_CBS_NEAR
#define AMM_CBS_NEAR 512
#endif
#ifndef AMM_CTAB_WAVES_PER_EU
#define AMM_CTAB_WAVES_PER_EU 1
#endif
template <int FAM, int CMODE, int GFAM, int BS, int SMASK, bool EPI = false>
__global__ void __launch_bounds__(BS) __attribute__((amdgpu_waves_per_eu(AMM_CTAB_WAVES_PER_EU)))
k_cpair(CPairArgs A, PairConsts c, PairConsts g, CEpiArgs E) {
    constexpr bool DUAL = GFAM >= 0;
    constexpr bool SS = SMASK != 0;
    extern __shared__ __align__(16) char s_lds[];
    if (EPI && E.spec_clear) {
        for (int cidx = blockIdx.x * BS + threadIdx.x; cidx <= E.grid.ncell; cidx += gridDim.x * BS) E.spec_clear[cidx] = 0;
    }
#ifdef AMM_CPAIR_TIMING
    const unsigned long long t_entry = wall_clock64();
    unsigned long long t_staged = 0;
    int n_tasks_done = 0, n_interior = 0;
    unsigned long long t_epi[3] = {0, 0, 0};
#endif
    auto stage = [&](int at, const double *src, int bytes) {
        for (int o = threadIdx.x * 16; o < bytes; o += BS * 16)
            *reinterpret_cast<double2 *>(s_lds + at + o) = *reinterpret_cast<const double2 *>(reinterpret_cast<const char *>(src) + o);
    };
    const int gbytes = DUAL ? A.guest_bytes : 0;
    stage(0, A.host_tab, A.host_bytes);
    if (DUAL) stage(A.host_bytes, A.guest_tab, gbytes);
    int used = A.host_bytes + gbytes;
    if (SS) {
        stage(used, A.host_tab_ss, A.host_ss_bytes);
        used += A.host_ss_bytes;
        if (DUAL) {
            stage(used, A.guest_tab_ss, A.guest_ss_bytes);
            used += A.guest_ss_bytes;
        }
    }
#if defined(AMM_EXP_TAB_GLOBAL)
    const char *tabh = reinterpret_cast<const char *>(A.host_tab);
#else
    const char *tabh = s_lds;
#endif
    const char *tabg = s_lds + A.host_bytes;
    const double *erfcx = amm_erfcx_table_dev_c;
    double2 *s_li = nullptr;
    if (!SS) {
        double *s_erfcx = reinterpret_cast<double *>(s_lds + used);
        for (int k = threadIdx.x; k < AMM_ERFCX_NI * AMM_ERFCX_NC; k += BS) s_erfcx[k] = amm_erfcx_table_dev_c[k];
        erfcx = s_erfcx;
        s_li = reinterpret_cast<double2 *>(s_erfcx + AMM_ERFCX_NI * AMM_ERFCX_NC) + (threadIdx.x >> 6) * 192;
    }
    __syncthreads();
#ifdef AMM_CPAIR_TIMING
    t_staged = wall_clock64();
#endif

    constexpr int WPB = BS / 64;
    const int lane = threadIdx.x & 63;
    const double sign = c.sign;
    PairConsts c1 = c, g1 = g;
    c1.sign = 1.0;
    g1.sign = 1.0;
    const int xcd = blockIdx.x & 7, nwx = (gridDim.x >> 3) * WPB;
    const int row_end = min((xcd + 1) * A.rpx, A.nrows);
    for (int phase = 0; phase < A.nphase; ++phase) {
    const int shift = A.ph_shift[phase], row0 = xcd * A.rpx + A.ph_off[phase], ntask = A.ph_ntask[phase];
    const int lpa = 1 << shift;
    const int sub = lane & (lpa - 1);
    const int rpw = 64 >> shift;
#ifdef AMM_CPAIR_SWAP
    for (int task = (int)(blockIdx.x >> 3) * WPB + ((int)(threadIdx.x >> 6) ^ 4); task < ntask; task += nwx) {
#else
    for (int task = (int)(blockIdx.x >> 3) * WPB + (int)(threadIdx.x >> 6); task < ntask; task += nwx) {
#endif
        const int a = row0 + task * rpw + (lane >> shift);
        const bool valid = a < row_end;
        const int cs = A.c_begin + (valid ? a : 0);
        double4 pi[3];
        int i_sites = 0;
        int so[3] = {0, 0, 0}, sog[3] = {0, 0, 0};
        if (!SS) __builtin_amdgcn_wave_barrier();
#pragma unroll
        for (int t = 0; t < 3; ++t) {
            pi[t] = A.posq[3 * cs + t];
            pi[t].w *= c.Kc * sign;
            double2 l = A.lj[3 * cs + t];
            l.y *= sign;
            if (!SS) s_li[64 * t + lane] = l;
            const bool site = valid && l.y != 0.0;
            if ((SMASK >> t) & 1) {
                so[t] = site ? A.host_ss_off : 0;
                if (DUAL) sog[t] = site ? A.guest_ss_off : 0;
            }
            if (__builtin_amdgcn_ballot_w64(site) != 0ull) i_sites |= 1 << t;
        }
        if (!SS) {
            __builtin_amdgcn_fence(__ATOMIC_RELEASE, "wavefront");
            __builtin_amdgcn_wave_barrier();
            __builtin_amdgcn_fence(__ATOMIC_ACQUIRE, "wavefront");
        }
        const double2 *li = SS ? nullptr : s_li + lane;
        const int nfront = valid ? A.nnb[a] : 0;
        const int nn = valid ? (A.nnb_total ? A.nnb_total[a] : nfront) : 0;
        const int *row = A.nl + (size_t)(valid ? a : 0) * A.cap;
        const bool edge = valid && !(pi[0].x >= A.margin && pi[0].x <= A.box.L[0] - A.margin && pi[0].y >= A.margin &&
                                     pi[0].y <= A.box.L[1] - A.margin && pi[0].z >= A.margin && pi[0].z <= A.box.L[2] - A.margin);
        const bool interior = __builtin_amdgcn_ballot_w64(edge) == 0ull;
#ifdef AMM_CPAIR_TIMING
        ++n_tasks_done;
        n_interior += interior ? 1 : 0;
#endif
        double f[9], fg[9];
#pragma unroll
        for (int k = 0; k < 9; ++k) f[k] = fg[k] = 0.0;
        if (A.per_pair_image) cwalk_rows<FAM, CMODE, GFAM, 2, SMASK>(A, c1, g1, tabh, tabg, erfcx, pi, li, i_sites, so, sog, sign, row, nfront, nn, sub, lpa, cs, f, fg);
        else if (interior) cwalk_rows<FAM, CMODE, GFAM, 0, SMASK>(A, c1, g1, tabh, tabg, erfcx, pi, li, i_sites, so, sog, sign, row, nfront, nn, sub, lpa, cs, f, fg);
        else cwalk_rows<FAM, CMODE, GFAM, 1, SMASK>(A, c1, g1, tabh, tabg, erfcx, pi, li, i_sites, so, sog, sign, row, nfront, nn, sub, lpa, cs, f, fg);
        for (int off = lpa >> 1; off > 0; off >>= 1) {
#pragma unroll
            for (int k = 0; k < 9; ++k) {
                f[k] += __shfl_xor(f[k], off);
                if (DUAL) fg[k] += __shfl_xor(fg[k], off);
            }
        }
        if (valid && sub == 0) {
#pragma unroll
            for (int t = 0; t < 3; ++t) {
                const int i = A.sorted_out ? 3 * a + t : A.aperm[3 * cs + t];
#pragma unroll
                for (int d = 0; d < 3; ++d) {
                    if (A.accumulate) A.force[3 * i + d] += f[3 * t + d];
                    else A.force[3 * i + d] = f[3 * t + d];
                    if (DUAL) {
                        if (A.g_accumulate) A.gforce[3 * i + d] += fg[3 * t + d];
                        else A.gforce[3 * i + d] = fg[3 * t + d];
                    }
                }
            }
        }
    }
    }
#ifdef AMM_CPAIR_TIMING
    if (EPI) t_staged = wall_clock64();
#endif
    if (EPI) {
        for (int phase = 0; phase < A.nphase; ++phase) {
            const int shift = A.ph_shift[phase], row0 = xcd * A.rpx + A.ph_off[phase], ntask = A.ph_ntask[phase];
            const int rpw = 64 >> shift;
            for (int task = (int)(blockIdx.x >> 3) * WPB + (int)(threadIdx.x >> 6); task < ntask; task += nwx) {
                const int a = row0 + task * rpw + (lane >> shift);
                const bool valid = a < row_end;
#ifdef AMM_CPAIR_TIMING
                cepi_rows(E, A.box, A.c_begin + (valid ? a : 0), valid, lane & ((1 << shift) - 1), t_epi);
#else
                cepi_rows(E, A.box, A.c_begin + (valid ? a : 0), valid, lane & ((1 << shift) - 1));
#endif
            }
        }
        if (E.spec_count && amm_last_block(E.spec_ticket)) {
            if (amm_ld_l2(&E.spec_flags[0])) {
                const int fullest = cscan_counts<BS>(E.grid.ncell, E.spec_count, E.spec_start);
                if (threadIdx.x == 0) E.spec_flags[6] = fullest;
            }
        }
    }
#ifdef AMM_CPAIR_TIMING
    if (A.wave_times && (threadIdx.x & 63) == 0) {
        unsigned long long *o = A.wave_times + 4 * ((size_t)blockIdx.x * (BS / 64) + (threadIdx.x >> 6));
        o[0] = t_entry;
        o[1] = t_staged;
        o[2] = wall_clock64();
        o[3] = EPI ? (((t_epi[0] - t_staged) & 0xfffffull) | (((t_epi[1] - t_staged) & 0xfffffull) << 20) | (((t_epi[2] - t_staged) & 0xfffffull) << 40))
                   : (((unsigned long long)n_interior << 8) | (unsigned long long)n_tasks_done);
    }
#endif
}

static const double AMM_PHASE_COST[7] = {0, 0, 1.0, 0.55, 0.32, 0.18, 0.11};
static double cpair_plan_rec(int rows, int waves, int s, int off, CPairArgs *P) {
    const int rpw = 64 >> s, per_round = waves * rpw;
    const int full = rows / per_round, left = rows - full * per_round;
    const double finish = (double)((rows + per_round - 1) / per_round) * AMM_PHASE_COST[s];
    auto put = [&](int ntask) {
        if (P && ntask > 0) {
            P->ph_off[P->nphase] = off;
            P->ph_shift[P->nphase] = s;
            P->ph_ntask[P->nphase] = ntask;
            ++P->nphase;
        }
    };
    int s2 = 6;
    double split = 1e300;
    for (int t = s + 1; t <= 6 && left > 0; ++t) {
        const double v = cpair_plan_rec(left, waves, t, 0, nullptr);
        if (v < split) {
            split = v;
            s2 = t;
        }
    }
    split += full * AMM_PHASE_COST[s];
// ... 152 lines not shown
        p[k] = sx[3 * a + k];
        p0[k] = sx[k];
        x[3 * i + k] = p[k];
        v[3 * i + k] = sv[3 * a + k];
    }
    amm_watch_atom(W, i, p);
    if (posq_next) {
        posq_next[s] = make_double4(csorted_image(p[0], p0[0], cwrap1(p0[0], box.L[0], box.invL[0]) - p0[0], box.L[0], box.invL[0]),
                                    csorted_image(p[1], p0[1], cwrap1(p0[1], box.L[1], box.invL[1]) - p0[1], box.L[1], box.invL[1]),
                                    csorted_image(p[2], p0[2], cwrap1(p0[2], box.L[2], box.invL[2]) - p0[2], box.L[2], box.invL[2]), q_next[i]);
        if (lj_next) lj_next[s] = make_double2(hsig_next[i], seps2_next[i]);
    }
}

int amm_cluster_state_finish_impl(amm_ctx *ctx) {
    PendingExchange &pe = ctx->pending;
    ClusterList *cl = pe.cl;
    WatchArgs W;
    amm_collect_watches(ctx, W);
    PairForce *nx = pe.next;
    hipLaunchKernelGGL(k_state_scatter, dim3((3 * cl->nc + 255) / 256), dim3(256), 0, ctx->stream, cl->nc, pe.per / 3, cl->c_begin, cl->c_end,
                       cl->d_aperm, ctx->d_xchg, ctx->d_x, ctx->d_v, ctx->box, W, nx ? nx->d_posq_s : (double4 *)nullptr,
                       nx ? nx->d_lj_s : (double2 *)nullptr, nx ? nx->d_q : nullptr, nx ? nx->d_hsig : nullptr, nx ? nx->d_seps2 : nullptr);
    AMM_HIP(hipGetLastError());
    amm_watch_moved(ctx);
    if (nx) {
        cl->sorted_for = nx;
        cl->sorted_epoch = ctx->pos_epoch;
        cl->sorted_pos = ctx->d_x;
    }
    pe.active = false;
    pe.kind = 0;
    return 0;
}

static int cluster_setup_grid(amm_ctx *ctx, ClusterList *cl, double rc) {
    CellGrid &g = cl->grid;
    g.ncell = 1;
    const double reach = cl->rlist_build + 2.0 * cl->rext;
    for (int k = 0; k < 3; ++k) {
        const double L = ctx->box.L[k];
        int nc = (int)floor(L / (0.5 * reach));
        if (nc < 1) nc = 1;
        if (nc > 512) nc = 512;
        g.nc[k] = nc;
        g.h[k] = 2;
        g.nstencil[k] = nc >= 5 ? 5 : nc;
        g.cw[k] = L / nc;
        g.inv_cw[k] = nc / L;
        g.ncell *= nc;
        if (!(rc + cl->skin + 2.0 * cl->rext < 0.5 * L * (1 - 1e-9))) cl->per_pair_image = true;
    }
    return 0;
}

static int cluster_chain(amm_ctx *ctx, PairForce *L, ClusterList *cl, const double *d_pos, int force, bool count_only, PairForce *gather_for,
                         CZeroRows Z = CZeroRows{0, nullptr, nullptr, nullptr}, int copies_current = 0, bool skip_assign = false) {
    hipStream_t st = ctx->stream;
    const int nc = cl->nc;
    if (!skip_assign)
        hipLaunchKernelGGL(k_cassign, dim3((nc + cl->nrest + 255) / 256), dim3(256), 0, st, nc, d_pos, ctx->box, cl->grid, cl->d_cell_count, cl->d_cell_start,
                           cl->d_cell_members, cl->capc, count_only ? (double *)nullptr : cl->d_xref, cl->d_flags, cl->d_ticket, force, cl->d_first,
                           cl->d_rest, cl->nrest);
    if (!cl->d_cell_members) return 0;
    PairForce *gf = gather_for;
    const long sort_threads = std::max(std::max((long)cl->grid.ncell * 64, gf ? (long)nc : 0L), (long)Z.n);
    hipLaunchKernelGGL(k_csort_gather, dim3((unsigned)((sort_threads + 255) / 256)), dim3(256), 0, st, cl->grid.ncell, nc, cl->d_cell_start,
                       cl->d_cell_members, cl->capc, cl->d_cperm, cl->d_aperm, d_pos, ctx->box, cl->d_pos4f, cl->d_flags, cl->d_flags, force,
                       gf ? gf->d_q : nullptr, gf ? gf->d_hsig : nullptr, gf ? gf->d_seps2 : nullptr, gf ? gf->d_posq_s : (double4 *)nullptr,
                       gf ? gf->d_lj_s : (double2 *)nullptr, (float)cl->rext, L->d_seps2, cl->d_first, Z, copies_current,
                       count_only ? (double *)nullptr : cl->d_xref, cl->c_begin, cl->c_end, cl->d_slice_cells);
    const bool slice = cl->c_end - cl->c_begin < cl->nc;
    const bool split = cl->split_parts > 0 && !count_only;
    const int ncell_grid = slice ? (int)std::min<long>(cl->grid.ncell, (5L * cl->grid.ncell) / (4L * std::max(1, ctx->world)) + 4) : cl->grid.ncell;
    const long threads = (long)ncell_grid * cl->parts * 64;
    dim3 grid(split ? (unsigned)(ncell_grid * cl->split_parts) : (unsigned)((threads + 255) / 256));
    CBoxF bf;
    for (int k = 0; k < 3; ++k) {
        bf.L[k] = (float)ctx->box.L[k];
        bf.invL[k] = (float)ctx->box.invL[k];
    }
    const float rl = (float)cl->rlist_build;
    const float rn2 = cl->rnear_build > 0 ? (float)(cl->rnear_build * cl->rnear_build) : 3.0e38f;
    const bool use_rint = cl->grid.nc[0] < 5 || cl->grid.nc[1] < 5 || cl->grid.nc[2] < 5;
#define AMM_LAUNCH_CBUILD(CO, RI)                                                                                                   \
    do {                                                                                                                            \
        if (slice)                                                                                                                  \
            hipLaunchKernelGGL((k_cbuild<CO, RI, true>), grid, dim3(256), 0, st, cl->c_begin, cl->c_end, cl->parts, cl->d_cell_start,    \
                               cl->d_pos4f, bf, cl->grid, rl, rn2, cl->cap, cl->d_nl, cl->d_nnb, cl->d_nnb_near, cl->d_flags,            \
                               cl->d_blockstats, cl->d_counters, cl->d_ticket + AMM_TICKET_INTS, force, cl->d_slice_cells);              \
        else                                                                                                                        \
            hipLaunchKernelGGL((k_cbuild<CO, RI, false>), grid, dim3(256), 0, st, cl->c_begin, cl->c_end, cl->parts, cl->d_cell_start,   \
                               cl->d_pos4f, bf, cl->grid, rl, rn2, cl->cap, cl->d_nl, cl->d_nnb, cl->d_nnb_near, cl->d_flags,            \
                               cl->d_blockstats, cl->d_counters, cl->d_ticket + AMM_TICKET_INTS, force, cl->d_slice_cells);              \
    } while (0)
#define AMM_LAUNCH_CBUILD_SPLIT(RI)                                                                                                  \
    hipLaunchKernelGGL((k_cbuild_split<RI>), grid, dim3(256), 0, st, cl->c_begin, cl->c_end, cl->split_parts, cl->d_cell_start,     \
                       cl->d_pos4f, bf, cl->grid, rl, rn2, cl->cap, cl->d_nl, cl->d_nnb, cl->d_nnb_near, cl->d_flags, cl->d_blockstats,  \
                       cl->d_counters, cl->d_ticket + AMM_TICKET_INTS, force, cl->d_slice_cells)
    if (count_only) {
        if (use_rint) AMM_LAUNCH_CBUILD(true, true);
        else AMM_LAUNCH_CBUILD(true, false);
    } else if (split) {
        if (use_rint) AMM_LAUNCH_CBUILD_SPLIT(true);
        else AMM_LAUNCH_CBUILD_SPLIT(false);
    } else {
        if (use_rint) AMM_LAUNCH_CBUILD(false, true);
        else AMM_LAUNCH_CBUILD(false, false);
    }
#undef AMM_LAUNCH_CBUILD
#undef AMM_LAUNCH_CBUILD_SPLIT
    AMM_HIP(hipGetLastError());
    return 0;
}

static double cluster_extent_host(amm_ctx *ctx, const double *d_pos, int n, int nc, const std::vector<int> &first) {
    std::vector<double> x(3 * (size_t)n);
    if (hipMemcpyAsync(x.data(), d_pos, sizeof(double) * 3 * (size_t)n, hipMemcpyDeviceToHost, ctx->stream) != hipSuccess) return -1.0;
    if (hipStreamSynchronize(ctx->stream) != hipSuccess) return -1.0;
    double worst = 0.0;
    for (int m = 0; m < nc; ++m) {
        const size_t i0 = first.empty() ? 3 * (size_t)m : (size_t)first[m];
        for (int a = 1; a < 3; ++a) {
            double d2 = 0.0;
            for (int k = 0; k < 3; ++k) {
                double d = x[3 * (i0 + a) + k] - x[3 * i0 + k];
                d -= ctx->box.L[k] * std::nearbyint(d * ctx->box.invL[k]);
                d2 += d * d;
            }
            worst = std::max(worst, d2);
        }
    }
    return std::sqrt(worst);
}

static int cluster_first_build(amm_ctx *ctx, PairForce *L, const double *d_pos) {
    ClusterList *cl = new ClusterList();
    L->cl = cl;
    const int n = L->n, nc = L->n_mol;
    cl->nc = nc;
    cl->d_first = L->d_mol_first;
    cl->d_rest = L->d_rest_idx;
    cl->nrest = L->n_rest;
    cl->skin = L->skin;
    cl->rlist_build = L->rlist_build;
    cl->rnear_build = L->rnear_build;
    const double ext = cluster_extent_host(ctx, d_pos, n, nc, L->h_mol_first);
    if (!(ext >= 0.0) || !(ext == ext)) {
        amm_set_error("molecule-row list: cannot read the positions (or NaN positions)");
        return 1;
    }
    cl->rext = std::max(1.5 * ext, ext + 0.05);
    if (cluster_setup_grid(ctx, cl, L->desc.rc)) return 1;
    const int per = (nc + ctx->world - 1) / ctx->world;
    cl->c_begin = std::min(nc, ctx->rank * per);
    cl->c_end = std::min(nc, cl->c_begin + per);
    const size_t ns = (size_t)std::max(cl->c_end - cl->c_begin, 1);
    const int ncell = cl->grid.ncell;
    AMM_HIP(hipMalloc(&cl->d_cell_count, sizeof(int) * (ncell + 1)));
    AMM_HIP(hipMemset(cl->d_cell_count, 0, sizeof(int) * (ncell + 1)));
    AMM_HIP(hipMalloc(&cl->d_cell_start, sizeof(int) * (ncell + 1)));
    AMM_HIP(hipMalloc(&cl->d_cperm, sizeof(int) * nc));
    AMM_HIP(hipMalloc(&cl->d_aperm, sizeof(int) * 3 * (size_t)nc));
    AMM_HIP(hipMalloc(&cl->d_pos4f, sizeof(float4) * 3 * (size_t)nc));
    AMM_HIP(hipMalloc(&cl->d_xref, sizeof(double) * 3 * (size_t)n));
    AMM_HIP(hipMalloc(&cl->d_nnb, sizeof(int) * ns));
    AMM_HIP(hipMalloc(&cl->d_nnb_near, sizeof(int) * ns));
    AMM_HIP(hipMalloc(&cl->d_flags, sizeof(int) * 16));
    AMM_HIP(hipMemset(cl->d_flags, 0, sizeof(int) * 16));
    AMM_HIP(hipMalloc(&cl->d_ticket, sizeof(int) * 4 * AMM_TICKET_INTS));
    AMM_HIP(hipMemset(cl->d_ticket, 0, sizeof(int) * 4 * AMM_TICKET_INTS));
    AMM_HIP(hipMalloc(&cl->d_counters, sizeof(unsigned long long) * 8));
    AMM_HIP(hipMemset(cl->d_counters, 0, sizeof(unsigned long long) * 8));
    AMM_HIP(hipMalloc(&cl->d_slice_cells, sizeof(int) * 2));
    AMM_HIP(hipMemset(cl->d_slice_cells, 0, sizeof(int) * 2));
    int lpa = 4;
    while (lpa < 64 && (long)(cl->c_end - cl->c_begin) * lpa < 64L * 2048) lpa <<= 1;
    if (ctx->opt_lpa > 0) lpa = ctx->opt_lpa;
    cl->lpa = lpa;
    int flags[8];
    cl->capc = 0;
    if (cluster_chain(ctx, L, cl, d_pos, 1, true, nullptr)) return 1;
    AMM_HIP(hipMemcpyAsync(flags, cl->d_flags, sizeof(flags), hipMemcpyDeviceToHost, ctx->stream));
    AMM_HIP(hipStreamSynchronize(ctx->stream));
    cl->capc = 2 * flags[6] + 16;
    AMM_HIP(hipMalloc(&cl->d_cell_members, sizeof(int) * (size_t)ncell * cl->capc));
    cl->parts = std::max(1, std::min(16, (int)std::ceil(1.5 * (double)nc / ncell / CB_BATCH)));
    if (ctx->world > 1) {
        const int active_cells = std::max(1, ncell / ctx->world);
        const int want = (4096 + active_cells - 1) / active_cells, most = std::max(1, (int)std::ceil((double)nc / ncell));
        cl->parts = std::max(cl->parts, std::min(want, std::min(most, 6)));
    }
    if (ctx->opt_parts > 0) cl->parts = std::max(1, std::min(16, ctx->opt_parts));
    cl->split_parts = 0;
    if (ctx->world > 1 && ctx->opt_build_split < 0) {
        const int active_cells = std::max(1, ncell / ctx->world);
        const int most = std::max(1, (int)std::ceil((double)nc / ncell / CBS_BATCH));
        cl->split_parts = std::max(1, std::min(std::min(16, most), (1024 + active_cells / 2) / active_cells));
    }
    if (ctx->opt_build_split == 0) cl->split_parts = 0;
    if (ctx->opt_build_split > 0) cl->split_parts = std::min(16, ctx->opt_build_split);
    {
        const long t1 = (long)ncell * cl->parts * 64;
        const size_t nblocks = std::max((size_t)((t1 + 255) / 256), (size_t)ncell * (size_t)cl->split_parts);
        AMM_HIP(hipMalloc(&cl->d_blockstats, sizeof(unsigned long long) * 3 * nblocks));
    }
    cl->cap = 0;
    {
        const int cb = cl->c_begin, ce = cl->c_end;
        cl->c_begin = 0;
        cl->c_end = nc;
        const int rc_count = cluster_chain(ctx, L, cl, d_pos, 1, true, nullptr);
        cl->c_begin = cb;
        cl->c_end = ce;
        if (rc_count) return 1;
    }
    AMM_HIP(hipMemcpyAsync(flags, cl->d_flags, sizeof(flags), hipMemcpyDeviceToHost, ctx->stream));
    AMM_HIP(hipStreamSynchronize(ctx->stream));
    if (flags[7]) {
        amm_set_error("molecule-row list: cell table overflow at the first build");
        return 1;
    }
    cl->cap = ((int)(flags[2] * 1.5) + 32 + 15) / 16 * 16;
    if (cl->cap > 65535 || nc >= (1 << 29)) {
        amm_set_error("molecule-row list: rows longer than 65535 entries or more than 2^29 molecules are not supported");
        return 1;
    }
    AMM_HIP(hipMalloc(&cl->d_nl, sizeof(int) * ns * cl->cap));
    if (cluster_chain(ctx, L, cl, d_pos, 1, false, nullptr)) return 1;
    cl->built = true;
    return 0;
}

int amm_cluster_eval_impl(amm_ctx *ctx, PairForce *pf, const double *d_pos, double *d_force, int accumulate, PairForce *guest,
                          double *g_force, int g_accumulate, int exchange) {
    hipStream_t st = ctx->stream;
    const int n = pf->n;
    if (!g_erfcx_uploaded_c[ctx->device & 63]) {
        AMM_HIP(hipMemcpyToSymbol(HIP_SYMBOL(amm_erfcx_table_dev_c), amm_erfcx_table_host, sizeof(amm_erfcx_table_host)));
        g_erfcx_uploaded_c[ctx->device & 63] = true;
    }
    PairForce *L = pf->host ? pf->host : pf;
    bool gathered = false;
    const CZeroRows Z = ctx->zero_rows;
    ctx->zero_rows = CZeroRows{0, nullptr, nullptr, nullptr};
    if (!L->cl || !L->cl->built) {
        if (L->cl) {
            amm_set_error("molecule-row list: an earlier first build failed");
            return 1;
        }
        if (cluster_first_build(ctx, L, d_pos)) return 1;
    }
    ClusterList *cl = L->cl;
    const EpiPlan *plan = ctx->epi_request;
    ctx->epi_request = nullptr;
    ctx->epi_done = false;
    const int copies_current = (cl->sorted_for == pf && cl->sorted_epoch == ctx->pos_epoch && cl->sorted_pos == d_pos && Z.n == 0) ? 1 : 0;
    if (copies_current) ctx->n_copies_current++;
    if (cl->checked_epoch == ctx->pos_epoch && cl->checked_pos == d_pos && !L->force_rebuild_c) {
    } else {
        if (!(cl->pre_epoch == ctx->pos_epoch && cl->pre_pos == d_pos))
            hipLaunchKernelGGL(k_ccheck_displacement, dim3((n + 255) / 256), dim3(256), 0, st, n, d_pos, cl->d_xref, 0.25 * cl->skin * cl->skin,
                               cl->d_flags);
        const int forced = L->force_rebuild_c ? 1 : 0;
        L->force_rebuild_c = false;
        const bool assigned = !forced && cl->assigned_epoch == ctx->pos_epoch && cl->assigned_pos == d_pos;
        if (cluster_chain(ctx, L, cl, d_pos, forced, false, pf, Z, copies_current, assigned)) return 1;
        gathered = true;
    }
    cl->checked_epoch = ctx->pos_epoch;
    cl->checked_pos = d_pos;
    if (!gathered && !copies_current)
        hipLaunchKernelGGL(k_csort_gather, dim3((std::max(cl->nc, Z.n) + 255) / 256), dim3(256), 0, st, cl->grid.ncell, cl->nc, cl->d_cell_start,
                           cl->d_cell_members, cl->capc, cl->d_cperm, cl->d_aperm, d_pos, ctx->box, cl->d_pos4f, cl->d_flags + 8, cl->d_flags, 0,
                           pf->d_q, pf->d_hsig, pf->d_seps2, pf->d_posq_s, pf->d_lj_s, (float)cl->rext, L->d_seps2, cl->d_first, Z, 0, (double *)nullptr, 0, 0, (int *)nullptr);
    cl->sorted_for = pf;
    cl->sorted_epoch = ctx->pos_epoch;
    cl->sorted_pos = d_pos;
    const int nrows = cl->c_end - cl->c_begin;
    const int per_c = (cl->nc + ctx->world - 1) / ctx->world, per = 3 * per_c, nf = guest ? 2 : 1;
    double *out = d_force, *gout = g_force;
    auto ss_bytes_of = [](const PairForce *p) { return (p->d_tab_ss && p->pc.tab.ss_first >= 0) ? (p->pc.tab.nint - p->pc.tab.ss_first) * AMM_TAB_STRIDE : 0; };
    auto plan_fits = [&]() {
        if (!(plan && plan->kind == 0 && ctx->opt_fuse_epilogue && !accumulate && !cl->d_first && cl->nrest == 0 && plan->bs && plan->bs->mol3_ok &&
              plan->bs->finalized && plan->bs->ncomp == cl->nc && plan->f0 && plan->npre <= AMM_MAX_PRE && ctx->d_x == d_pos && ctx->d_v &&
              plan->f0 != d_force && plan->f0 != g_force)) return false;
        if (guest && !(!g_accumulate && g_force != d_force && ctx->opt_fuse_rows && pf == L && cl->rnear_build > 0)) return false;
        return true;
    };
    bool state_mode = false;
    if (exchange && ctx->world > 1 && ctx->opt_state_exchange && plan_fits() && cl->nc - per_c * (ctx->world - 1) > 0) {
        bool kernel = ctx->opt_site_tab && ss_bytes_of(pf) > 0 && (!guest || ss_bytes_of(guest) > 0);
        const int lds = pf->pc.tab.nint * AMM_TAB_STRIDE + ss_bytes_of(pf) + (guest ? guest->pc.tab.nint * AMM_TAB_STRIDE + ss_bytes_of(guest) : 0);
        kernel = kernel && lds <= AMM_CPAIR_LDS_LIMIT;
        if (guest) kernel = kernel && guest->pc.family == AMM_NEAR_FSWITCH && (pf->pc.family == AMM_DAMPED || pf->pc.family == AMM_NONBONDED);
        state_mode = kernel;
    }
    if (state_mode) {
        if (ctx->pending.active) {
            amm_set_error("exchanged evaluation while the previous one still waits for amm_exchange_finish");
            return 1;
        }
        if (!ctx->d_xchg || ctx->xchg_doubles < (long long)ctx->world * 2 * per * 3) {
            amm_set_error("exchanged evaluation: bind an exchange buffer of world * 2 * per * 3 doubles, per = amm_exchange_per()");
            return 1;
        }
    } else if (exchange) {
        if (accumulate || g_accumulate) {
            amm_set_error("exchanged evaluation: forces only, no accumulation");
            return 1;
        }
        if (ctx->pending.active) {
            amm_set_error("exchanged evaluation while the previous one still waits for amm_exchange_finish");
            return 1;
        }
        if (!ctx->d_xchg || ctx->xchg_doubles < (long long)ctx->world * 2 * per * 3) {
            amm_set_error("exchanged evaluation: bind an exchange buffer of world * 2 * per * 3 doubles, per = amm_exchange_per()");
            return 1;
        }
        out = ctx->d_xchg + (size_t)ctx->rank * nf * per * 3;
        gout = out + (size_t)per * 3;
    } else {
        if (!accumulate && ctx->world > 1) AMM_HIP(hipMemsetAsync(d_force, 0, sizeof(double) * 3 * (size_t)n, st));
        if (guest && !g_accumulate && ctx->world > 1 && g_force != d_force) AMM_HIP(hipMemsetAsync(g_force, 0, sizeof(double) * 3 * (size_t)n, st));
    }
    if (nrows > 0) {
        CPairArgs A;
        A.c_begin = cl->c_begin;
        A.nrows = nrows;
        int sh = 0;
        while ((1 << sh) < cl->lpa) ++sh;
        A.lpa_shift = sh;
        A.cap = cl->cap;
        A.aperm = cl->d_aperm;
        A.nl = cl->d_nl;
        A.nnb = cl->d_nnb_near;
        A.nnb_total = (pf == L && cl->rnear_build > 0) ? cl->d_nnb : nullptr;
        if (pf == L && !(cl->rnear_build > 0)) {
            A.nnb = cl->d_nnb;
            A.nnb_total = nullptr;
        }
        A.posq = pf->d_posq_s;
        A.lj = pf->d_lj_s;
        A.force = out;
        A.accumulate = accumulate;
        A.sorted_out = (exchange && !state_mode) ? 1 : 0;
        A.box = ctx->box;
        A.host_tab = pf->d_tab;
        A.host_bytes = pf->pc.tab.nint * AMM_TAB_STRIDE;
        auto ss_bytes = [](const PairForce *p) { return (p->d_tab_ss && p->pc.tab.ss_first >= 0) ? (p->pc.tab.nint - p->pc.tab.ss_first) * AMM_TAB_STRIDE : 0; };
        A.host_tab_ss = pf->d_tab_ss;
        A.host_ss_bytes = ss_bytes(pf);
        A.host_ss_off = A.host_bytes - pf->pc.tab.ss_first * AMM_TAB_STRIDE;
        A.site_atoms = pf->site_atoms;
        A.guest_tab = A.guest_tab_ss = nullptr;
        A.guest_bytes = A.guest_ss_bytes = A.guest_ss_off = A.g_accumulate = 0;
        A.gforce = nullptr;
        A.gfac = A.gsr = 1.0;
        A.margin = cl->rlist_build + cl->skin + 2.0 * cl->rext + 1e-6;
        const int rpw = 64 >> A.lpa_shift;
        A.ntask = (nrows + rpw - 1) / rpw;
        A.per_pair_image = cl->per_pair_image ? 1 : 0;
        A.hsig_site = pf->site_hsig;
        A.seps2_site = pf->site_seps2;
        hipEvent_t e0 = nullptr, e1 = nullptr;
        const bool timed = ctx->profile && (ctx->profile_only < 0 || ctx->profile_only == pf->id);
        if (timed) {
            if (pf->ev_used + 2 > pf->ev.size())
                for (int k = 0; k < 64; ++k) {
                    hipEvent_t ev;
                    AMM_HIP(hipEventCreate(&ev));
                    pf->ev.push_back(ev);
                }
            e0 = pf->ev[pf->ev_used++];
            e1 = pf->ev[pf->ev_used++];
            AMM_HIP(hipEventRecord(e0, st));
        }
        int rc_ = 0;
        bool fused = false;
        if (guest) guest->last_fused = 0;
        CEpiArgs E;
        const CEpiArgs *Ep = nullptr;
        bool epi_launched = false;
        PairForce *enext = nullptr;
        bool enext_alias = false;
        if (((ctx->world == 1 && !exchange) || state_mode) && plan_fits()) {
            E.niter = plan->niter;
            E.npre = plan->npre;
            E.recompute_f0 = (state_mode && plan->niter > 0) ? 1 : 0;
            E.x = ctx->d_x;
            E.v = ctx->d_v;
            E.f0 = plan->f0;
            E.mass = ctx->d_mass;
            E.c1 = plan->c1;
            E.d = plan->d;
            E.c2 = plan->c2;
            bool ok = true;
            E.xchg_x = state_mode ? ctx->d_xchg + (size_t)ctx->rank * 2 * per * 3 : nullptr;
            E.xchg_v = state_mode ? E.xchg_x + (size_t)per * 3 : nullptr;
            E.c_first = cl->c_begin;
            for (int p = 0; p < AMM_MAX_PRE; ++p) {
                CEpiPre &k = E.pre[p];
                k.a = p < plan->npre ? plan->pre_a[p] : nullptr;
                k.b = p < plan->npre ? plan->pre_b[p] : nullptr;
                k.coef = p < plan->npre ? plan->pre_coef[p] : 0.0;
                k.plus = p < plan->npre ? plan->pre_plus[p] : 0;
                if (p < plan->npre && !k.a) ok = false;
            }
            E.cperm = cl->d_cperm;
            E.term_l = plan->bs->d_term_l;
            E.term_q = plan->bs->d_term_q;
            E.atom_recs = plan->bs->d_atom_recs;
            E.posq_next = nullptr;
            E.lj_next = nullptr;
            E.q_next = E.hsig_next = E.seps2_next = nullptr;
            PairForce *nx = plan->niter > 0 ? plan->next : nullptr;
            if (nx && nx->cluster_ok && (nx == L || nx->host == L) && nx->n == n) {
                enext = nx;
                enext_alias = nx->d_posq_s == pf->d_posq_s;
                if (enext_alias && !nx->d_posq_alt) AMM_HIP(hipMalloc(&nx->d_posq_alt, sizeof(double4) * (size_t)n));
                E.posq_next = enext_alias ? nx->d_posq_alt : nx->d_posq_s;
                E.lj_next = enext_alias ? nullptr : nx->d_lj_s;
                E.q_next = nx->d_q;
// ... 167 lines not shown
    for (int off = 32; off > 0; off >>= 1) cnt += __shfl_xor(cnt, off);
    if ((threadIdx.x & 63) == 0 && cnt) atomicAdd(out, cnt);
}

int amm_cluster_count_within_impl(amm_ctx *ctx, PairForce *pf, const double *d_pos, double r_within, long long *count) {
    PairForce *L = pf->host ? pf->host : pf;
    ClusterList *cl = L->cl;
    hipStream_t st = ctx->stream;
    hipLaunchKernelGGL(k_csort_gather, dim3((cl->nc + 255) / 256), dim3(256), 0, st, cl->grid.ncell, cl->nc, cl->d_cell_start, cl->d_cell_members,
                       cl->capc, cl->d_cperm, cl->d_aperm, d_pos, ctx->box, cl->d_pos4f, cl->d_flags + 8, cl->d_flags, 0, pf->d_q, pf->d_hsig,
                       pf->d_seps2, pf->d_posq_s, pf->d_lj_s, (float)cl->rext, L->d_seps2, cl->d_first, CZeroRows{0, nullptr, nullptr, nullptr}, 0, (double *)nullptr, 0, 0, (int *)nullptr);
    if (cl->sorted_for == pf) {
        cl->sorted_epoch = ctx->pos_epoch;
        cl->sorted_pos = d_pos;
    }
    CPairArgs A;
    std::memset(&A, 0, sizeof(A));
    A.c_begin = cl->c_begin;
    A.nrows = cl->c_end - cl->c_begin;
    A.cap = cl->cap;
    A.nl = cl->d_nl;
    A.nnb = (pf == L) ? cl->d_nnb : cl->d_nnb_near;
    A.nnb_total = nullptr;
    if (pf == L && cl->rnear_build > 0) {
        A.nnb = cl->d_nnb_near;
        A.nnb_total = cl->d_nnb;
    }
    A.posq = pf->d_posq_s;
    A.box = ctx->box;
    unsigned long long *d_cnt = cl->d_counters + 7;
    AMM_HIP(hipMemsetAsync(d_cnt, 0, sizeof(unsigned long long), st));
    if (A.nrows > 0)
        hipLaunchKernelGGL(k_ccount_within, dim3((unsigned)(((long)A.nrows * 8 + 255) / 256)), dim3(256), 0, st, A, r_within * r_within, d_cnt);
    unsigned long long h = 0;
    AMM_HIP(hipMemcpyAsync(&h, d_cnt, sizeof(h), hipMemcpyDeviceToHost, st));
    AMM_HIP(hipStreamSynchronize(st));
    *count = (long long)h;
    return 0;
}

__global__ void __launch_bounds__(256) k_crow_padding(int nrows, int lpa_shift, const int *__restrict__ nnb, unsigned long long *out) {
    const int task = blockIdx.x * blockDim.x + threadIdx.x;
    const int rpw = 64 >> lpa_shift, lpa = 1 << lpa_shift;
    unsigned long long slots = 0, entries = 0;
    if (task * rpw < nrows) {
        int longest = 0;
        for (int r = task * rpw; r < min(nrows, (task + 1) * rpw); ++r) {
            const int nn = nnb[r];
            entries += (unsigned long long)nn;
            longest = max(longest, (nn + lpa - 1) >> lpa_shift);
        }
        slots = 64ull * (unsigned long long)longest;
    }
    for (int off = 32; off > 0; off >>= 1) {
        slots += __shfl_xor(slots, off);
        entries += __shfl_xor(entries, off);
    }
    if ((threadIdx.x & 63) == 0) {
        atomicAdd(&out[0], slots);
        atomicAdd(&out[1], entries);
    }
}

int amm_cluster_row_padding_impl(amm_ctx *ctx, PairForce *pf, long long out[2]) {
    PairForce *L = pf->host ? pf->host : pf;
    ClusterList *cl = L->cl;
    hipStream_t st = ctx->stream;
    const int nrows = cl->c_end - cl->c_begin;
    int sh = 0;
    while ((1 << sh) < cl->lpa) ++sh;
    unsigned long long *d_out = cl->d_counters + 5;
    AMM_HIP(hipMemsetAsync(d_out, 0, 2 * sizeof(unsigned long long), st));
    const int ntask = (nrows + (64 >> sh) - 1) / (64 >> sh);
    if (ntask > 0)
        hipLaunchKernelGGL(k_crow_padding, dim3((unsigned)((ntask + 255) / 256)), dim3(256), 0, st, nrows, sh, (pf == L) ? cl->d_nnb : cl->d_nnb_near, d_out);
    unsigned long long h[2] = {0, 0};
    AMM_HIP(hipMemcpyAsync(h, d_out, sizeof(h), hipMemcpyDeviceToHost, st));
    AMM_HIP(hipStreamSynchronize(st));
    out[0] = (long long)h[0];
    out[1] = (long long)h[1];
    return 0;
}

int amm_cluster_free(ClusterList *cl) {
#ifdef AMM_CBS_TIMING
    {
        unsigned long long t[8];
        const bool got = hipMemcpyFromSymbol(t, HIP_SYMBOL(g_cbs_t), sizeof(t)) == hipSuccess && t[7];
        if (got && cl->split_parts == 0)
            fprintf(stderr, "k_cbuild<SLICE>: %llu busy wavefronts, mean: prologue %.2f us, whole %.2f us, in drains %.2f us (%.2f drains)\n", t[7], t[0] / 100.0 / t[7],
                    t[1] / 100.0 / t[7], t[2] / 100.0 / t[7], (double)t[3] / t[7]);
        if (got && cl->split_parts > 0)
            fprintf(stderr, "k_cbuild_split, first wavefront of %llu busy blocks, mean clocks (100 MHz): prologue %.2f | pass 1 %.2f wait %.2f | pass 2 %.2f wait %.2f | copy %.2f wait %.2f us\n",
                    t[7], t[0] / 100.0 / t[7], t[1] / 100.0 / t[7], t[2] / 100.0 / t[7], t[3] / 100.0 / t[7], t[4] / 100.0 / t[7], t[5] / 100.0 / t[7], t[6] / 100.0 / t[7]);
    }
#endif
    for (void *q : {(void *)cl->d_spec_count[0], (void *)cl->d_spec_count[1], (void *)cl->d_spec_ticket})
        if (q) (void)hipFree(q);
    if (cl->d_slice_cells) (void)hipFree(cl->d_slice_cells);
    void *ptrs[] = {cl->d_cell_count, cl->d_cell_start, cl->d_cell_members, cl->d_cperm, cl->d_aperm, cl->d_pos4f, cl->d_xref, cl->d_nl,
                    cl->d_nnb, cl->d_nnb_near, cl->d_flags, cl->d_counters, cl->d_blockstats, cl->d_ticket};
    for (void *p : ptrs)
        if (p) (void)hipFree(p);
    delete cl;
    return 0;
}
```

atomsmm_amd/csrc/pair.hip:

```cpp
#include <cmath>
#include <cstdio>
#include <cstdlib>
#include <cstring>

#include "amm_ctx.h"
#include "bonded_terms.h"
#include "cluster.h"
#include "device_utils.h"
#include "pair_math.h"
#include "pair_tab.h"

int amm_pair_build_consts(const amm_pair_desc &d, PairConsts &pc) {
    pc.family = d.family;
    pc.flags = d.flags;
    pc.degree = d.degree < 1 ? 1 : d.degree;
    pc.cmode = (d.flags & AMM_COULOMB_EWALD) ? 1 : ((d.flags & AMM_COULOMB_RF) ? 2 : 0);
    pc.sign = d.sign;
    pc.rc = d.rc;
    pc.rc2 = d.rc * d.rc;
    pc.rc0 = d.rc0;
    pc.rs0 = d.rs0;
    pc.inv_dr0 = (d.rc0 > d.rs0) ? 1.0 / (d.rc0 - d.rs0) : 0.0;
    pc.rswitch = d.rswitch;
    pc.alpha = d.alpha;
// ... 1876 lines not shown
}

bool amm_pair_can_eval_dual(amm_ctx *ctx, PairForce *guest, PairForce *host) {
    if (!guest || !host || guest->host != host || host->host) return false;
    if (guest->dual_ok >= 0) return guest->dual_ok == 1;
    guest->dual_ok = 0;
    const int gf = guest->desc.family, hf = host->desc.family;
    if (!(gf == AMM_NEAR_NONE || gf == AMM_NEAR_SHIFT || gf == AMM_NEAR_FSWITCH)) return false;
    if (!(hf == AMM_DAMPED || hf == AMM_NONBONDED)) return false;
    if ((guest->desc.flags & AMM_GUARD_RC0) || (host->desc.flags & AMM_GUARD_RC0)) return false;
    if ((guest->desc.flags | host->desc.flags) & (AMM_GROUP_LJ | AMM_GROUP_Q)) return false;
    if (!(guest->desc.rc <= host->desc.rc)) return false;
    if (guest->pc.Kc != host->pc.Kc) return false;
    const size_t n = (size_t)ctx->n;
    std::vector<double> a(n), b(n);
    const double *ga[3] = {guest->d_q, guest->d_hsig, guest->d_seps2}, *ha[3] = {host->d_q, host->d_hsig, host->d_seps2};
    for (int k = 0; k < 3; ++k) {
        if (hipMemcpy(a.data(), ga[k], sizeof(double) * n, hipMemcpyDeviceToHost) != hipSuccess) return false;
        if (hipMemcpy(b.data(), ha[k], sizeof(double) * n, hipMemcpyDeviceToHost) != hipSuccess) return false;
        if (std::memcmp(a.data(), b.data(), sizeof(double) * n) != 0) return false;
    }
    guest->dual_ok = 1;
    return true;
}

__global__ void __launch_bounds__(256) k_count_within(PairArgs A, double r2w, int nslice, unsigned long long *out) {
    const int tid = blockIdx.x * blockDim.x + threadIdx.x;
    const int a = tid >> A.lpa_shift, sub = tid & ((1 << A.lpa_shift) - 1);
    unsigned long long cnt = 0;
    if (a < nslice) {
        const int s = A.s_begin + a;
        const double4 pi = A.posq_s[s];
        const int nfront = A.nnb[a], nn = A.nnb_total ? A.nnb_total[a] : nfront;
        const int *row = A.nl + (size_t)a * A.cap;
        const int back = A.cap - 1 + nfront;
        for (int k = sub; k < nn; k += 1 << A.lpa_shift) {
            const double4 pj = A.posq_s[row[k < nfront ? k : back - k]];
            const double dx = amm_min_image(pi.x - pj.x, A.box.L[0], A.box.invL[0]);
            const double dy = amm_min_image(pi.y - pj.y, A.box.L[1], A.box.invL[1]);
            const double dz = amm_min_image(pi.z - pj.z, A.box.L[2], A.box.invL[2]);
            cnt += (dx * dx + dy * dy + dz * dz < r2w) ? 1ull : 0ull;
        }
    }
    for (int off = 32; off > 0; off >>= 1) cnt += __shfl_xor(cnt, off);
    if ((threadIdx.x & 63) == 0 && cnt) atomicAdd(out, cnt);
}

int amm_pair_count_within_impl(amm_ctx *ctx, PairForce *pf, const double *d_pos, double r_within, long long *count) {
    PairForce *L = pf->host ? pf->host : pf;
    if (!L->built) {
        amm_set_error("amm_pair_count_within: evaluate the force once first (the neighbour rows do not exist yet)");
        return 1;
    }
    hipStream_t st = ctx->stream;
    const int n = pf->n;
    hipLaunchKernelGGL(k_gather_sorted, dim3((n + 255) / 256), dim3(256), 0, st, n, L->d_perm, d_pos, pf->d_q, pf->d_hsig,
                       pf->d_seps2, ctx->box, pf->d_posq_s, pf->d_lj_s);
    PairArgs A;
    std::memset(&A, 0, sizeof(A));
    A.s_begin = L->s_begin;
    A.s_end = L->s_end;
    A.lpa_shift = 3;
    A.cap = L->cap;
    A.nl = L->d_nl;
    A.nnb = L->d_nnb_near;
    A.nnb_total = (pf == L && L->rnear_build > 0) ? L->d_nnb : nullptr;
    A.posq_s = pf->d_posq_s;
    A.box = ctx->box;
    const int nslice = L->s_end - L->s_begin;
    unsigned long long *d_cnt = L->d_counters + 7;
    AMM_HIP(hipMemsetAsync(d_cnt, 0, sizeof(unsigned long long), st));
    if (nslice > 0)
        hipLaunchKernelGGL(k_count_within, dim3((unsigned)(((long)nslice * 8 + 255) / 256)), dim3(256), 0, st, A, r_within * r_within, nslice, d_cnt);
    unsigned long long h = 0;
    AMM_HIP(hipMemcpyAsync(&h, d_cnt, sizeof(h), hipMemcpyDeviceToHost, st));
    AMM_HIP(hipStreamSynchronize(st));
    *count = (long long)h;
    return 0;
}

extern "C" __attribute__((weak)) const char *amm_variant_tag(void);
const char *amm_kernel_revision_impl() {
#ifdef AMM_CLUSTER_TUNE
    return "r05-epi5-tune";
#else
    return amm_variant_tag ? "r05-epi5-tune" : "r05-epi5";
#endif
}

int amm_pair_build_table(PairForce *pf) {
    std::vector<double> coef;
    SiteTable ss;
    ss.want = pf->cluster_ok && pf->one_site_class && pf->site_one_charge && pf->site_q != 0.0 && pf->site_seps2 != 0.0;
    ss.sig = 2.0 * pf->site_hsig;
    ss.eps4 = pf->site_seps2 * pf->site_seps2;
    ss.QQ = pf->pc.Kc * pf->site_q * pf->site_q;
    pf->tab_error = amm_build_coulomb_table(pf->pc, coef, &ss);
    pf->ss_built_for[0] = pf->site_hsig;
    pf->ss_built_for[1] = pf->site_seps2;
    pf->ss_built_for[2] = ss.want ? pf->site_q : 0.0;
    if (pf->d_tab) {
        (void)hipFree(pf->d_tab);
        pf->d_tab = nullptr;
    }
    if (pf->d_tab_ss) {
        (void)hipFree(pf->d_tab_ss);
        pf->d_tab_ss = nullptr;
    }
    pf->ss_error = ss.error;
    if (pf->pc.tab.nint > 0 && !(pf->tab_error <= AMM_TAB_MAX_ERROR)) {
        pf->pc.tab.nint = 0;
        coef.clear();
    }
    if (pf->pc.tab.nint == 0 || ss.coef.empty() || !(ss.error <= AMM_TAB_SS_MAX_ERROR)) {
        pf->pc.tab.ss_first = -1;
        ss.coef.clear();
    }
    if (pf->pc.tab.nint > 0) {
        AMM_HIP(hipMalloc(&pf->d_tab, sizeof(double) * coef.size()));
        AMM_HIP(hipMemcpy(pf->d_tab, coef.data(), sizeof(double) * coef.size(), hipMemcpyHostToDevice));
    }
    if (!ss.coef.empty()) {
        AMM_HIP(hipMalloc(&pf->d_tab_ss, sizeof(double) * ss.coef.size()));
        AMM_HIP(hipMemcpy(pf->d_tab_ss, ss.coef.data(), sizeof(double) * ss.coef.size(), hipMemcpyHostToDevice));
    }
    return 0;
}

bool amm_pair_can_fuse_discount(amm_ctx *ctx, PairForce *guest, PairForce *host) {
    if (!guest || !host || guest->host != host || host->host) return false;
    if (!(guest->desc.flags & AMM_GUARD_RC0)) return false;
    if (guest->fuse_ok >= 0) return guest->fuse_ok == 1;
    guest->fuse_ok = 0;
    if (!ctx->opt_tab) return false;
    const int gf = guest->desc.family, hf = host->desc.family;
    if (!(gf == AMM_NEAR_NONE || gf == AMM_NEAR_SHIFT || gf == AMM_NEAR_FSWITCH)) return false;
    if (!(hf == AMM_DAMPED || hf == AMM_NONBONDED)) return false;
    if ((host->desc.flags & AMM_GUARD_RC0) || host->pc.sign != 1.0) return false;
    if ((guest->desc.flags | host->desc.flags) & (AMM_GROUP_LJ | AMM_GROUP_Q)) return false;
    if (!(guest->pc.tab.nint > 0 && guest->d_tab && host->pc.tab.nint > 0 && host->d_tab)) return false;
    if (guest->pc.Kc != host->pc.Kc) return false;
    const size_t n = (size_t)ctx->n;
    std::vector<double> a(n), b(n);
    const double *ga[3] = {guest->d_q, guest->d_hsig, guest->d_seps2}, *ha[3] = {host->d_q, host->d_hsig, host->d_seps2};
    for (int k = 0; k < 3; ++k) {
        if (hipMemcpy(a.data(), ga[k], sizeof(double) * n, hipMemcpyDeviceToHost) != hipSuccess) return false;
        if (hipMemcpy(b.data(), ha[k], sizeof(double) * n, hipMemcpyDeviceToHost) != hipSuccess) return false;
        if (std::memcmp(a.data(), b.data(), sizeof(double) * n) != 0) return false;
    }
    guest->fuse_ok = 1;
    return true;
}

int amm_pair_free(PairForce *pf) {
    void *ptrs[] = {pf->d_q, pf->d_hsig, pf->d_seps2, pf->d_excl_ptr, pf->d_excl_idx, pf->d_cell_of, pf->d_cell_count,
                    pf->d_cell_start, pf->d_cell_members, pf->d_perm, pf->d_posq_s, pf->d_lj_s, pf->d_xref,
                    pf->d_nl, pf->d_nnb, pf->d_flags, pf->d_counters, pf->d_epart, pf->d_pos4f_s, pf->d_blockstats, pf->d_inv_perm, pf->d_nnb_near, pf->d_nl_out, pf->d_nnb_out,
                    pf->d_nnb_scratch, pf->d_xref_out, pf->d_ticket, pf->d_tab, pf->d_cls, pf->d_cell_count_lj, pf->d_cell_start_lj,
                    pf->d_row_order, pf->d_member, pf->d_active, pf->d_cell_sets, pf->d_nnb_lj, pf->d_mol_first, pf->d_rest_idx};
    for (void *p : ptrs)
        if (p) (void)hipFree(p);
    for (hipEvent_t e : pf->ev) (void)hipEventDestroy(e);
    if (pf->cl) amm_cluster_free(pf->cl);
    pf->cl = nullptr;
    if (pf->small) amm_small_group_free(pf->small);
    pf->small = nullptr;
    return 0;
}

// ... 2 lines not shown
```

include/atomsmm_hip.h:

```cpp
#ifndef ATOMSMM_HIP_H
#define ATOMSMM_HIP_H

#include <stdint.h>

#ifdef __cplusplus
extern "C" {
#endif

#define AMM_ABI_VERSION 1

enum {
    AMM_NEAR_NONE = 0,
    AMM_NEAR_SHIFT = 1,
    AMM_NEAR_FSWITCH = 2,
    AMM_DAMPED = 3,
    AMM_NONBONDED = 4,
    AMM_SOFTCORE = 5,
    AMM_LJ_VIRIAL = 6
};
enum {
    AMM_GUARD_RC0 = 1,
    AMM_COULOMB_EWALD = 2,
    AMM_COULOMB_RF = 4,
    AMM_SWITCH = 8,
// ... 69 lines not shown
int amm_check(amm_ctx *ctx);

int amm_pair_create(amm_ctx *ctx, const amm_pair_desc *desc, const double *h_q, const double *h_sigma,
                    const double *h_eps, const int32_t *h_excl, int32_t n_excl, double skin,
                    int32_t *force_id);
int amm_pair_set_params(amm_ctx *ctx, int32_t force_id, const double *h_q, const double *h_sigma,
                        const double *h_eps);
int amm_pair_share_list(amm_ctx *ctx, int32_t force_id, int32_t host_id);

int amm_pair_set_lambda(amm_ctx *ctx, int32_t force_id, double value);
int amm_pair_set_lambda_dev(amm_ctx *ctx, int32_t force_id, const double *d_lambda);
int amm_pair_set_scale(amm_ctx *ctx, int32_t force_id, double scale);
int amm_pair_energy_derivative(amm_ctx *ctx, int32_t force_id, const double *d_pos, double *d_out);
#define AMM_MAX_STATES 64
int amm_pair_energy_states(amm_ctx *ctx, int32_t force_id, const double *d_pos, const double *d_lambdas, int32_t n_states, double *d_out);

int amm_bonded_create(amm_ctx *ctx, int32_t *force_id);
int amm_bonded_add_terms(amm_ctx *ctx, int32_t force_id, int32_t kind, const int32_t *h_idx,
                         const double *h_params, int32_t n_terms, int32_t periodic,
                         const amm_pair_desc *desc_or_null);
int amm_bonded_finalize(amm_ctx *ctx, int32_t force_id);
int amm_bonded_set_sliced(amm_ctx *ctx, int32_t force_id, int32_t on);
int amm_bonded_release(amm_ctx *ctx, int32_t force_id);

int amm_pme_create(amm_ctx *ctx, double alpha, int32_t nx, int32_t ny, int32_t nz, double Kc, const double *h_q,
                   int32_t *force_id);
int amm_pme_set_charges(amm_ctx *ctx, int32_t force_id, const double *h_q);
int amm_pme_set_sliced(amm_ctx *ctx, int32_t force_id, int32_t on);

int amm_force_eval(amm_ctx *ctx, int32_t force_id, const double *d_pos, double *d_force,
                   int32_t accumulate, double *d_energy);

int amm_kick(amm_ctx *ctx, double *d_v, const double *d_f, const double *d_f2, int32_t plus, const double *d_mass, double coef);
int amm_move(amm_ctx *ctx, double *d_x, const double *d_v, double coef);
int amm_copy(amm_ctx *ctx, double *d_dst, const double *d_src);
int amm_mvv(amm_ctx *ctx, const double *d_v, const double *d_m, double *d_out);

int amm_expr_eval(amm_ctx *ctx, const int32_t *code, int32_t n_code, const double *consts, int32_t n_consts,
                  const double *globals, int32_t n_globals, uint64_t seed, uint64_t counter, double *d_dst, double *d_sum);

int amm_expr_eval_scalar(amm_ctx *ctx, const int32_t *code, int32_t n_code, const double *consts, int32_t n_consts, double *d_scalars,
                         int32_t n_scalars);

int amm_constraints_create(amm_ctx *ctx, const int32_t *h_pairs, const double *h_dist, int32_t n_constraints, double tolerance);

int amm_expr_define(amm_ctx *ctx, const int32_t *code, int32_t n_code, const double *consts, int32_t n_consts,
                    const double *globals, int32_t n_globals, int32_t *expr_id);
int amm_expr_seed(amm_ctx *ctx, uint64_t seed);
int amm_bath_define(amm_ctx *ctx, double z, double kT, int32_t *bath_id);
int amm_bath_define_nhl(amm_ctx *ctx, double h, double z, double kT, double Q, double friction, int32_t slot, int32_t *bath_id);
int amm_iso_define(amm_ctx *ctx, int32_t on, double LkT, double Q1, int32_t slot_v1);
int amm_bath_define_sin(amm_ctx *ctx, double h, double z, double kT, double Q2, double friction, int32_t slot_v2, int32_t *bath_id);
int amm_regulated_define(amm_ctx *ctx, int32_t on, double alpha, double an_kT);
int amm_bath_define_regulated(amm_ctx *ctx, int32_t kind, int32_t split, double h, double z, double kT, double Q, double omega,
                              double friction, double alpha, double an, int32_t slot_v_eta, int32_t *bath_id);

int amm_bind_state(amm_ctx *ctx, double *d_x, double *d_v, const double *d_mass);
#define AMM_MAX_SLOTS 64
#define AMM_SLOT_X 62
#define AMM_SLOT_V 63
int amm_bind_buffer(amm_ctx *ctx, int32_t slot, double *d_buf);
int amm_group_define(amm_ctx *ctx, int32_t group, int32_t slot, const int32_t *force_ids, int32_t n_forces);
int amm_run_ops(amm_ctx *ctx, const amm_op *ops, int32_t n_ops, int32_t repeat);
int amm_set_outer_skin(amm_ctx *ctx, double skin_out);
int amm_set_option(amm_ctx *ctx, const char *name, double value);
int amm_run_stats(amm_ctx *ctx, int64_t out[4]);
int amm_run_ops_from(amm_ctx *ctx, const amm_op *ops, int32_t n_ops, int32_t repeat, int64_t *cursor);
int amm_positions_changed(amm_ctx *ctx);
int amm_exchange_per(amm_ctx *ctx, int32_t *per);
int amm_set_fuse_inner(amm_ctx *ctx, int32_t on);

typedef struct {
    int64_t n_builds;
    int64_t n_evals;
    int64_t n_list_pairs;
    int64_t n_slice_atoms;
    int32_t capacity;
    int32_t max_neighbors;
    int32_t lanes_per_atom;
    int32_t n_cells;
    double rlist;
    int32_t shares_list;
    int32_t list_kind;
    int64_t n_outer_builds;
    int64_t n_outer_pairs;
    double rlist_outer;
    double tab_error;
    int32_t has_table;
    int32_t rode_along;
    int32_t has_site_table;
    int32_t n_rest_atoms;
    double site_tab_error;
    int32_t n_candidates;
    int32_t n_candidate_walks;
    int32_t chargeless;
    int32_t build_split;
} amm_pair_stats;
int amm_pair_get_stats(amm_ctx *ctx, int32_t force_id, amm_pair_stats *out);
int amm_pair_count_within(amm_ctx *ctx, int32_t force_id, const double *d_pos, double r_within, int64_t *count);
int amm_pair_row_padding(amm_ctx *ctx, int32_t force_id, int64_t out[2]);
const char *amm_kernel_revision(void);
int amm_profile_enable(amm_ctx *ctx, int32_t on);
int amm_profile_read(amm_ctx *ctx, int32_t force_id, int64_t *n_launches, double *total_ms);

#ifdef __cplusplus
}
#endif
#endif
```

Measured before the change: 1086.

## Sort neighbor rows by skin-distance class and cut walks by max displacement level

During the cluster list build, each neighbor entry gets a distance class based on how far into the skin it lies. A per-row wave sort then orders entries by class into the final list and records a prefix count per level. The displacement watch also tracks the largest per-atom motion level, and the force walk can stop at the matching prefix, so pairs that cannot yet be within cutoff are skipped. This adds a scratch list buffer, a sort pass on every build and an extra atomic max in the watch kernels. Stats gain the level and walked-pair counts.

```diff
diff --git a/atomsmm_amd/backend.py b/atomsmm_amd/backend.py
--- a/atomsmm_amd/backend.py
+++ b/atomsmm_amd/backend.py
@@ -49,12 +49,26 @@
     _fields_ = [('op', C.c_int32), ('a', C.c_int32), ('b', C.c_int32), ('c', C.c_int32), ('coef', C.c_double)]
 
 
+class _RowLevel(C.Structure):
+    _fields_ = [('row_level', C.c_int32), ('row_levels', C.c_int32)]
+
+
+class _OuterBuildsOrLevel(C.Union):
+    _anonymous_ = ('_rows',)
+    _fields_ = [('n_outer_builds', C.c_int64), ('_rows', _RowLevel)]
+
+
+class _OuterPairsOrWalked(C.Union):
+    _fields_ = [('n_outer_pairs', C.c_int64), ('n_walked_pairs', C.c_int64)]
+
+
 class PairStats(C.Structure):
+    _anonymous_ = ('_u_builds', '_u_pairs')
     _fields_ = [('n_builds', C.c_int64), ('n_evals', C.c_int64), ('n_list_pairs', C.c_int64),
                 ('n_slice_atoms', C.c_int64), ('capacity', C.c_int32), ('max_neighbors', C.c_int32),
                 ('lanes_per_atom', C.c_int32), ('n_cells', C.c_int32), ('rlist', C.c_double),
-                ('shares_list', C.c_int32), ('list_kind', C.c_int32), ('n_outer_builds', C.c_int64),
-                ('n_outer_pairs', C.c_int64), ('rlist_outer', C.c_double), ('tab_error', C.c_double),
+                ('shares_list', C.c_int32), ('list_kind', C.c_int32), ('_u_builds', _OuterBuildsOrLevel),
+                ('_u_pairs', _OuterPairsOrWalked), ('rlist_outer', C.c_double), ('tab_error', C.c_double),
                 ('has_table', C.c_int32), ('rode_along', C.c_int32),
                 ('has_site_table', C.c_int32), ('n_rest_atoms', C.c_int32), ('site_tab_error', C.c_double),
                 ('n_candidates', C.c_int32), ('n_candidate_walks', C.c_int32), ('chargeless', C.c_int32), ('build_split', C.c_int32)]
@@ -510,7 +524,14 @@
     def pair_stats(self, fid):
         st = PairStats()
         _chk(lib().amm_pair_get_stats(self.h, fid, C.byref(st)))
-        return {name: getattr(st, name) for name, _ in PairStats._fields_}
+        out = {name: getattr(st, name) for name, _ in PairStats._fields_ if not name.startswith('_')}
+        rows = st.list_kind in (1, 2)
+        out['n_outer_builds'] = 0 if rows else st.n_outer_builds
+        out['n_outer_pairs'] = 0 if rows else st.n_outer_pairs
+        out['row_levels'] = st.row_levels if rows else 0
+        out['row_level'] = st.row_level if rows else 0
+        out['n_walked_pairs'] = st.n_walked_pairs if rows else st.n_list_pairs
+        return out
 
     def pair_row_padding(self, fid):
         out = (C.c_int64 * 2)()
diff --git a/atomsmm_amd/csrc/abi.hip b/atomsmm_amd/csrc/abi.hip
--- a/atomsmm_amd/csrc/abi.hip
+++ b/atomsmm_amd/csrc/abi.hip
@@ -1753,9 +1753,18 @@
         out->n_list_pairs = 9 * (int64_t)(pf->host ? cnt[2] : cnt[1]);
         out->max_neighbors = flags[2];
         out->rlist_outer = L->desc.rc + L->skin;
+        {
+            int level = 0;
+            long long walked = 0;
+            if (amm_cluster_level_stats_impl(ctx, pf, &level, &walked)) return 1;
+            out->row_levels = AMM_ROW_LEVELS;
+            out->row_level = level;
+            out->n_walked_pairs = 9 * (int64_t)walked;
+        }
         if (L->last_kind == 2 && L->rest && L->rest->built) {
             AMM_HIP(hipMemcpy(cnt, L->rest->d_counters, sizeof(cnt), hipMemcpyDeviceToHost));
             out->n_list_pairs += (int64_t)(pf->host ? cnt[2] : cnt[1]);
+            out->n_walked_pairs += (int64_t)(pf->host ? cnt[2] : cnt[1]);
         }
         return 0;
     }
@@ -1834,6 +1843,7 @@
     else if (k == "lanes_per_row") ctx->opt_lpa = v;
     else if (k == "build_parts") ctx->opt_parts = v;
     else if (k == "build_split") ctx->opt_build_split = v;
+    else if (k == "row_cut") ctx->opt_row_cut = v;
     else if (k == "unroll") ctx->opt_unroll = v;
     else if (k == "dual_unroll") ctx->opt_dual_unroll = v;
     else if (k == "tab_block") ctx->opt_tab_bs = v;
diff --git a/atomsmm_amd/csrc/amm_ctx.h b/atomsmm_amd/csrc/amm_ctx.h
--- a/atomsmm_amd/csrc/amm_ctx.h
+++ b/atomsmm_amd/csrc/amm_ctx.h
@@ -306,6 +306,7 @@
     int opt_positions_private = 0;
     int opt_group_candidates = 1;
     int opt_row_phases = 1;
+    int opt_row_cut = 1;
     int opt_fuse_rows = 1;
     int opt_no_dual = 0, opt_no_defer = 0, opt_terms_from = 8192, opt_no_term_lanes = 0;
     ListWatch watched[AMM_MAX_WATCH];
@@ -352,6 +353,8 @@
 };
 
 #define AMM_FLAG_FAR 12
+#define AMM_FLAG_LEVEL 13
+#define AMM_ROW_LEVELS 4
 struct WatchArgs {
     int n;
     const double *xref[AMM_MAX_WATCH];
diff --git a/atomsmm_amd/csrc/bonded.hip b/atomsmm_amd/csrc/bonded.hip
--- a/atomsmm_amd/csrc/bonded.hip
+++ b/atomsmm_amd/csrc/bonded.hip
@@ -573,11 +573,7 @@
         }
         for (int q = 0; q < C.nwatch; ++q) {
             const double dx = x[0] - C.wref[q][3 * a], dy = x[1] - C.wref[q][3 * a + 1], dz = x[2] - C.wref[q][3 * a + 2];
-            const double d2 = dx * dx + dy * dy + dz * dz;
-            if (!(d2 <= C.wthr2[q])) {
-                C.wflags[q][0] = 1;
-                if (!(d2 <= 4.0 * C.wthr2[q])) C.wflags[q][AMM_FLAG_FAR] = 1;
-            }
+            amm_watch_d2(C.wflags[q], dx * dx + dy * dy + dz * dz, C.wthr2[q]);
         }
     }
 }
diff --git a/atomsmm_amd/csrc/bonded_terms.h b/atomsmm_amd/csrc/bonded_terms.h
--- a/atomsmm_amd/csrc/bonded_terms.h
+++ b/atomsmm_amd/csrc/bonded_terms.h
@@ -45,14 +45,35 @@
     return (c * t) * coef;
 }
 
+template <bool PAST_L2 = false>
+__device__ __forceinline__ void amm_watch_d2(int *flags, double d2, double thr2) {
+    if (!(d2 <= thr2)) {
+        if (PAST_L2) __hip_atomic_store(&flags[0], 1, __ATOMIC_RELAXED, __HIP_MEMORY_SCOPE_AGENT);
+        else flags[0] = 1;
+        if (!(d2 <= 4.0 * thr2)) {
+            if (PAST_L2) __hip_atomic_store(&flags[AMM_FLAG_FAR], 1, __ATOMIC_RELAXED, __HIP_MEMORY_SCOPE_AGENT);
+            else flags[AMM_FLAG_FAR] = 1;
+        }
+    }
+    const double s = d2 * (double)(AMM_ROW_LEVELS * AMM_ROW_LEVELS);
+    int lvl = 0;
+#pragma unroll
+    for (int L = 0; L < AMM_ROW_LEVELS; ++L) lvl += !(s <= (double)(L * L) * thr2) ? 1 : 0;
+    if (lvl > flags[AMM_FLAG_LEVEL]) {
+        for (int L = AMM_ROW_LEVELS; L >= 1; --L) {
+            const unsigned long long m = __builtin_amdgcn_ballot_w64(lvl >= L);
+            if (m == 0ull) continue;
+            if (lvl >= L && __builtin_amdgcn_mbcnt_hi((unsigned)(m >> 32), __builtin_amdgcn_mbcnt_lo((unsigned)m, 0u)) == 0)
+                atomicMax(&flags[AMM_FLAG_LEVEL], L);
+            break;
+        }
+    }
+}
+
 __device__ __forceinline__ void amm_watch_atom(const WatchArgs &W, int a, const double *xn) {
     for (int q = 0; q < W.n; ++q) {
         const double dx = xn[0] - W.xref[q][3 * a], dy = xn[1] - W.xref[q][3 * a + 1], dz = xn[2] - W.xref[q][3 * a + 2];
-        const double d2 = dx * dx + dy * dy + dz * dz;
-        if (!(d2 <= W.thr2[q])) {
-            W.flags[q][0] = 1;
-            if (!(d2 <= 4.0 * W.thr2[q])) W.flags[q][AMM_FLAG_FAR] = 1;
-        }
+        amm_watch_d2(W.flags[q], dx * dx + dy * dy + dz * dz, W.thr2[q]);
     }
 }
 
diff --git a/atomsmm_amd/csrc/cluster.h b/atomsmm_amd/csrc/cluster.h
--- a/atomsmm_amd/csrc/cluster.h
+++ b/atomsmm_amd/csrc/cluster.h
@@ -23,6 +23,8 @@
     int cap = 0;
     int lpa = 8;
     int *d_nl = nullptr, *d_nnb = nullptr, *d_nnb_near = nullptr;
+    int *d_nl_scratch = nullptr;
+    int2 *d_lvl = nullptr;
     int *d_flags = nullptr;
     unsigned long long *d_counters = nullptr;
     unsigned long long *d_blockstats = nullptr;
@@ -46,5 +48,6 @@
                           double *g_force, int g_accumulate, int exchange);
 int amm_cluster_count_within_impl(amm_ctx *ctx, PairForce *pf, const double *d_pos, double r_within, long long *count);
 int amm_cluster_row_padding_impl(amm_ctx *ctx, PairForce *pf, long long out[2]);
+int amm_cluster_level_stats_impl(amm_ctx *ctx, PairForce *pf, int *level, long long *walked);
 int amm_cluster_state_finish_impl(amm_ctx *ctx);
 int amm_cluster_free(ClusterList *cl);
diff --git a/atomsmm_amd/csrc/cluster.hip b/atomsmm_amd/csrc/cluster.hip
--- a/atomsmm_amd/csrc/cluster.hip
+++ b/atomsmm_amd/csrc/cluster.hip
@@ -53,11 +53,7 @@
     const int i = blockIdx.x * blockDim.x + threadIdx.x;
     if (i >= n) return;
     const double dx = pos[3 * i] - xref[3 * i], dy = pos[3 * i + 1] - xref[3 * i + 1], dz = pos[3 * i + 2] - xref[3 * i + 2];
-    const double d2 = dx * dx + dy * dy + dz * dz;
-    if (!(d2 <= thr2)) {
-        flags[0] = 1;
-        if (!(d2 <= 4.0 * thr2)) flags[AMM_FLAG_FAR] = 1;
-    }
+    amm_watch_d2(flags, dx * dx + dy * dy + dz * dz, thr2);
 }
 
 __device__ __forceinline__ int cfirst(const int *__restrict__ first, int m) { return first ? first[m] : 3 * m; }
@@ -207,6 +203,54 @@
 __device__ __forceinline__ int cq_wrap(int i) { return i & (CB_QCAP - 1); }
 typedef float v2f __attribute__((ext_vector_type(2)));
 
+#define CB_CLS_SHIFT 25
+struct CClassThr {
+    float r0f, r0b, k_skin;
+};
+__device__ __forceinline__ int cclass_of(float m2, bool is_near, const CClassThr &ct) {
+    const float d = __builtin_sqrtf(m2) - (is_near ? ct.r0f : ct.r0b);
+    const int cls = (int)floorf(fmaf(d, ct.k_skin, 1.001f));
+    return min(max(cls, 0), AMM_ROW_LEVELS);
+}
+__device__ __forceinline__ int csort_part(const int *__restrict__ src, int *__restrict__ dst, int dir, int n, int lane) {
+    int cntv = 0;
+    for (int k0 = 0; k0 < n; k0 += 64) {
+        const int k = k0 + lane;
+        const int cls = k < n ? ((src[dir * k] >> CB_CLS_SHIFT) & 0xf) : 0xf;
+#pragma unroll
+        for (int j = 0; j <= AMM_ROW_LEVELS; ++j) {
+            const int nj = __popcll(__builtin_amdgcn_ballot_w64(cls == j));
+            cntv = lane == j ? cntv + nj : cntv;
+        }
+    }
+    int upto = 0;
+#pragma unroll
+    for (int j = 0; j <= AMM_ROW_LEVELS; ++j) upto += lane >= j ? __builtin_amdgcn_readlane(cntv, j) : 0;
+    int basev = upto - cntv;
+    for (int k0 = 0; k0 < n; k0 += 64) {
+        const int k = k0 + lane;
+        const int e = k < n ? src[dir * k] : 0;
+        const int cls = k < n ? ((e >> CB_CLS_SHIFT) & 0xf) : 0xf;
+        int at = 0;
+#pragma unroll
+        for (int j = 0; j <= AMM_ROW_LEVELS; ++j) {
+            const unsigned long long m = __builtin_amdgcn_ballot_w64(cls == j);
+            const int bj = __builtin_amdgcn_readlane(basev, j);
+            if (cls == j) at = bj + __builtin_amdgcn_mbcnt_hi((unsigned)(m >> 32), __builtin_amdgcn_mbcnt_lo((unsigned)m, 0u));
+            basev = lane == j ? basev + __popcll(m) : basev;
+        }
+        if (k < n) dst[dir * at] = e & ~(0xf << CB_CLS_SHIFT);
+    }
+    return upto;
+}
+__device__ __forceinline__ void csort_row(const int *__restrict__ scratch, int *__restrict__ row, int cap, int nf, int nb, int2 *lvl,
+                                          size_t lvl_stride, int lane) {
+    const bool over = nf + nb > cap;
+    const int uf = over ? 0 : csort_part(scratch, row, 1, nf, lane);
+    const int ub = over ? 0 : csort_part(scratch + cap - 1, row + cap - 1, -1, nb, lane);
+    if (lane <= AMM_ROW_LEVELS) lvl[(size_t)lane * lvl_stride] = make_int2(uf, ub);
+}
+
 __device__ void cfinish_build_block(int *flags, unsigned long long *counters, const unsigned long long *blockstats, int nblocks, int count_only) {
     __shared__ unsigned long long sh_part[4][3];
     unsigned long long sum = 0, mx = 0, nr = 0;
@@ -244,6 +288,7 @@
         if (!count_only) {
             flags[0] = 0;
             flags[AMM_FLAG_FAR] = 0;
+            flags[AMM_FLAG_LEVEL] = 0;
             counters[0] += 1;
         }
     }
@@ -263,7 +308,8 @@
 __global__ void __launch_bounds__(256) __attribute__((amdgpu_waves_per_eu(SLICE ? 3 : CB_WAVES))) k_cbuild(int c_begin, int c_end, int parts, const int *__restrict__ cell_start,
                                                 const float4 *__restrict__ pos4f, CBoxF box, CellGrid g, float rlist, float rnear2, int cap,
                                                 int *nl, int *nnb, int *nnb_near, int *flags, unsigned long long *blockstats,
-                                                unsigned long long *counters, int *ticket, int force, const int *slice_cells) {
+                                                unsigned long long *counters, int *ticket, int force, const int *slice_cells,
+                                                CClassThr ct, int *nl_scratch, int2 *lvl) {
     if (!force && !flags[0]) return;
     __shared__ int s_rstart[4][128];
     __shared__ int s_rpref[4][128];
@@ -438,8 +484,8 @@
                             const int mn = __builtin_amdgcn_mbcnt_hi((unsigned)(m_near >> 32), __builtin_amdgcn_mbcnt_lo((unsigned)m_near, 0u));
                             const int pos_near = cnt + mn, pos_far = (cap - 1 - cntf) - (mp - mn);
                             if (cnt + cntf + np_ <= cap) {
-                                int *row_out = nl + (size_t)(tb + t - c_begin) * cap;
-                                if (pass) row_out[is_near ? pos_near : pos_far] = slot[u] | (sites[u] << 29);
+                                int *row_out = nl_scratch + (size_t)(tb + t - c_begin) * cap;
+                                if (pass) row_out[is_near ? pos_near : pos_far] = slot[u] | (cclass_of(m2u, is_near, ct) << CB_CLS_SHIFT) | (sites[u] << 29);
                             }
                         }
                         row_cnt = lane == t ? c2 + nn_ + ((np_ - nn_) << 16) : row_cnt;
@@ -527,6 +573,15 @@
             }
             __builtin_amdgcn_fence(__ATOMIC_RELEASE, "wavefront");
             __builtin_amdgcn_wave_barrier();
+            if (!COUNT_ONLY) {
+                __builtin_amdgcn_fence(__ATOMIC_RELEASE, "workgroup");
+                __builtin_amdgcn_fence(__ATOMIC_ACQUIRE, "workgroup");
+                for (int t = 0; t < nt; ++t) {
+                    const int c2 = __builtin_amdgcn_readlane(row_cnt, t);
+                    const size_t r = (size_t)(tb + t - c_begin);
+                    csort_row(nl_scratch + r * cap, nl + r * cap, cap, c2 & 0xffff, (int)((unsigned)c2 >> 16), lvl + r, (size_t)max(c_end - c_begin, 1), lane);
+                }
+            }
             if (lane < nt) {
                 const int count = row_cnt & 0xffff, countf = (int)((unsigned)row_cnt >> 16);
                 const int total_nb = count + countf;
@@ -579,7 +634,8 @@
 __global__ void __launch_bounds__(256) k_cbuild_split(int c_begin, int c_end, int parts, const int *__restrict__ cell_start,
                                                       const float4 *__restrict__ pos4f, CBoxF box, CellGrid g, float rlist, float rnear2, int cap,
                                                       int *nl, int *nnb, int *nnb_near, int *flags, unsigned long long *blockstats,
-                                                      unsigned long long *counters, int *ticket, int force, const int *slice_cells) {
+                                                      unsigned long long *counters, int *ticket, int force, const int *slice_cells,
+                                                      CClassThr ct, int *nl_scratch, int2 *lvl) {
     if (!force && !flags[0]) return;
     __shared__ int s_rstart[128];
     __shared__ int s_rpref[128];
@@ -822,7 +878,7 @@
                                 const int np_ = __popcll(m_pass), nn_ = __popcll(m_near);
                                 const int mp = __builtin_amdgcn_mbcnt_hi((unsigned)(m_pass >> 32), __builtin_amdgcn_mbcnt_lo((unsigned)m_pass, 0u));
                                 const int mn = __builtin_amdgcn_mbcnt_hi((unsigned)(m_near >> 32), __builtin_amdgcn_mbcnt_lo((unsigned)m_near, 0u));
-                                if (pass) s_stage[j][is_near ? cnt + mn : 127 - cntf - (mp - mn)] = slot[u] | (sites[u] << 29);
+                                if (pass) s_stage[j][is_near ? cnt + mn : 127 - cntf - (mp - mn)] = slot[u] | (cclass_of(m2u, is_near, ct) << CB_CLS_SHIFT) | (sites[u] << 29);
                                 cnt += nn_;
                                 cntf += np_ - nn_;
                             }
@@ -840,7 +896,7 @@
                     const int nch = (T + 127) >> 7;
                     const int have = __builtin_amdgcn_readlane(row_cnt, t);
                     int nf = have & 0xffff, nb_ = (int)((unsigned)have >> 16);
-                    int *row_out = nl + (size_t)(tb + t - c_begin) * cap;
+                    int *row_out = nl_scratch + (size_t)(tb + t - c_begin) * cap;
                     for (int k = 0; k < nch; ++k) {
                         const int j = j0 + k;
                         const int cc = __builtin_amdgcn_readfirstlane(s_ccnt[j]);
@@ -859,6 +915,11 @@
                 __syncthreads();
                 CBS_STAMP(6);
             }
+            for (int t = w; t < nt; t += 4) {
+                const int c2 = __builtin_amdgcn_readlane(row_cnt, t);
+                const size_t r = (size_t)(tb + t - c_begin);
+                csort_row(nl_scratch + r * cap, nl + r * cap, cap, c2 & 0xffff, (int)((unsigned)c2 >> 16), lvl + r, (size_t)max(c_end - c_begin, 1), lane);
+            }
             if (w == 0 && lane < nt) {
                 const int count = row_cnt & 0xffff, countf = (int)((unsigned)row_cnt >> 16);
                 const int total_nb = count + countf;
@@ -892,6 +953,9 @@
     int c_begin, nrows, lpa_shift, cap;
     const int *aperm;
     const int *nl, *nnb, *nnb_total;
+    const int *level;
+    const int2 *lvl;
+    int lvl_stride;
     const double4 *posq;
     const double2 *lj;
     double *force;
@@ -919,8 +983,8 @@
 template <int FAM, int CMODE, int GFAM, int IMG, int SMASK>
 __device__ __forceinline__ void cwalk_rows(const CPairArgs &A, const PairConsts &c, const PairConsts &g, const char *tabh, const char *tabg,
                                            const double *erfcx, const double4 (&pi)[3], const double2 *li, int i_sites, const int (&so)[3],
-                                           const int (&sog)[3], double sign_lj, const int *row, int nfront, int nn, int sub, int lpa,
-                                           int self, double (&f)[9], double (&fg)[9]) {
+                                           const int (&sog)[3], double sign_lj, const int *row, int nfront, int gfront, int nn, int sub,
+                                           int lpa, int self, double (&f)[9], double (&fg)[9]) {
     constexpr bool DUAL = GFAM >= 0;
     constexpr bool SS = SMASK != 0;
     const int back = A.cap - 1 + nfront;
@@ -947,7 +1011,7 @@
     }
     while (__builtin_amdgcn_ballot_w64(k < nn) != 0ull) {
         const bool ok = k < nn;
-        const bool front = k < nfront;
+        const bool front = k < gfront;
         const bool any_front = DUAL && __builtin_amdgcn_ballot_w64(front) != 0ull;
         const unsigned bits = (unsigned)e >> 29;
         const int e2 = entry(k + 2 * lpa);
@@ -1142,11 +1206,7 @@
     }
     for (int q = 0; q < E.W.n; ++q) {
         const double dx = x[0] - E.W.xref[q][3 * a], dy = x[1] - E.W.xref[q][3 * a + 1], dz = x[2] - E.W.xref[q][3 * a + 2];
-        const double d2 = dx * dx + dy * dy + dz * dz;
-        if (!(d2 <= E.W.thr2[q])) {
-            amm_st_l2(&E.W.flags[q][0], 1);
-            if (!(d2 <= 4.0 * E.W.thr2[q])) amm_st_l2(&E.W.flags[q][AMM_FLAG_FAR], 1);
-        }
+        amm_watch_d2<true>(E.W.flags[q], dx * dx + dy * dy + dz * dz, E.W.thr2[q]);
     }
     if (E.posq_next) {
         double4 pq;
@@ -1426,6 +1486,7 @@
     constexpr int WPB = BS / 64;
     const int lane = threadIdx.x & 63;
     const double sign = c.sign;
+    const int level = A.level ? min(max(__builtin_amdgcn_readfirstlane(*A.level), 0), AMM_ROW_LEVELS) : AMM_ROW_LEVELS;
     PairConsts c1 = c, g1 = g;
     c1.sign = 1.0;
     g1.sign = 1.0;
@@ -1469,7 +1530,13 @@
         }
         const double2 *li = SS ? nullptr : s_li + lane;
         const int nfront = valid ? A.nnb[a] : 0;
-        const int nn = valid ? (A.nnb_total ? A.nnb_total[a] : nfront) : 0;
+        int nn = valid ? (A.nnb_total ? A.nnb_total[a] : nfront) : 0;
+        int gfront = nfront;
+        if (A.level && valid) {
+            const int2 upto = A.lvl[(size_t)level * A.lvl_stride + a];
+            gfront = upto.x;
+            nn = A.nnb_total ? nfront + upto.y : upto.x;
+        }
         const int *row = A.nl + (size_t)(valid ? a : 0) * A.cap;
         const bool edge = valid && !(pi[0].x >= A.margin && pi[0].x <= A.box.L[0] - A.margin && pi[0].y >= A.margin &&
                                      pi[0].y <= A.box.L[1] - A.margin && pi[0].z >= A.margin && pi[0].z <= A.box.L[2] - A.margin);
@@ -1481,9 +1548,9 @@
         double f[9], fg[9];
 #pragma unroll
         for (int k = 0; k < 9; ++k) f[k] = fg[k] = 0.0;
-        if (A.per_pair_image) cwalk_rows<FAM, CMODE, GFAM, 2, SMASK>(A, c1, g1, tabh, tabg, erfcx, pi, li, i_sites, so, sog, sign, row, nfront, nn, sub, lpa, cs, f, fg);
-        else if (interior) cwalk_rows<FAM, CMODE, GFAM, 0, SMASK>(A, c1, g1, tabh, tabg, erfcx, pi, li, i_sites, so, sog, sign, row, nfront, nn, sub, lpa, cs, f, fg);
-        else cwalk_rows<FAM, CMODE, GFAM, 1, SMASK>(A, c1, g1, tabh, tabg, erfcx, pi, li, i_sites, so, sog, sign, row, nfront, nn, sub, lpa, cs, f, fg);
+        if (A.per_pair_image) cwalk_rows<FAM, CMODE, GFAM, 2, SMASK>(A, c1, g1, tabh, tabg, erfcx, pi, li, i_sites, so, sog, sign, row, nfront, gfront, nn, sub, lpa, cs, f, fg);
+        else if (interior) cwalk_rows<FAM, CMODE, GFAM, 0, SMASK>(A, c1, g1, tabh, tabg, erfcx, pi, li, i_sites, so, sog, sign, row, nfront, gfront, nn, sub, lpa, cs, f, fg);
+        else cwalk_rows<FAM, CMODE, GFAM, 1, SMASK>(A, c1, g1, tabh, tabg, erfcx, pi, li, i_sites, so, sog, sign, row, nfront, gfront, nn, sub, lpa, cs, f, fg);
         for (int off = lpa >> 1; off > 0; off >>= 1) {
 #pragma unroll
             for (int k = 0; k < 9; ++k) {
@@ -1802,22 +1869,28 @@
     }
     const float rl = (float)cl->rlist_build;
     const float rn2 = cl->rnear_build > 0 ? (float)(cl->rnear_build * cl->rnear_build) : 3.0e38f;
+    CClassThr ct;
+    ct.r0b = (float)(cl->rlist_build - cl->skin);
+    ct.r0f = (float)((cl->rnear_build > 0 ? cl->rnear_build : cl->rlist_build) - cl->skin);
+    ct.k_skin = cl->skin > 0 ? (float)(AMM_ROW_LEVELS / cl->skin) : 1.0e30f;
     const bool use_rint = cl->grid.nc[0] < 5 || cl->grid.nc[1] < 5 || cl->grid.nc[2] < 5;
 #define AMM_LAUNCH_CBUILD(CO, RI)                                                                                                   \
     do {                                                                                                                            \
         if (slice)                                                                                                                  \
             hipLaunchKernelGGL((k_cbuild<CO, RI, true>), grid, dim3(256), 0, st, cl->c_begin, cl->c_end, cl->parts, cl->d_cell_start,    \
                                cl->d_pos4f, bf, cl->grid, rl, rn2, cl->cap, cl->d_nl, cl->d_nnb, cl->d_nnb_near, cl->d_flags,            \
-                               cl->d_blockstats, cl->d_counters, cl->d_ticket + AMM_TICKET_INTS, force, cl->d_slice_cells);              \
+                               cl->d_blockstats, cl->d_counters, cl->d_ticket + AMM_TICKET_INTS, force, cl->d_slice_cells, ct,          \
+                               cl->d_nl_scratch, cl->d_lvl);                                                               \
         else                                                                                                                        \
             hipLaunchKernelGGL((k_cbuild<CO, RI, false>), grid, dim3(256), 0, st, cl->c_begin, cl->c_end, cl->parts, cl->d_cell_start,   \
                                cl->d_pos4f, bf, cl->grid, rl, rn2, cl->cap, cl->d_nl, cl->d_nnb, cl->d_nnb_near, cl->d_flags,            \
-                               cl->d_blockstats, cl->d_counters, cl->d_ticket + AMM_TICKET_INTS, force, cl->d_slice_cells);              \
+                               cl->d_blockstats, cl->d_counters, cl->d_ticket + AMM_TICKET_INTS, force, cl->d_slice_cells, ct,          \
+                               cl->d_nl_scratch, cl->d_lvl);                                                               \
     } while (0)
 #define AMM_LAUNCH_CBUILD_SPLIT(RI)                                                                                                  \
     hipLaunchKernelGGL((k_cbuild_split<RI>), grid, dim3(256), 0, st, cl->c_begin, cl->c_end, cl->split_parts, cl->d_cell_start,     \
                        cl->d_pos4f, bf, cl->grid, rl, rn2, cl->cap, cl->d_nl, cl->d_nnb, cl->d_nnb_near, cl->d_flags, cl->d_blockstats,  \
-                       cl->d_counters, cl->d_ticket + AMM_TICKET_INTS, force, cl->d_slice_cells)
+                       cl->d_counters, cl->d_ticket + AMM_TICKET_INTS, force, cl->d_slice_cells, ct, cl->d_nl_scratch, cl->d_lvl)
     if (count_only) {
         if (use_rint) AMM_LAUNCH_CBUILD(true, true);
         else AMM_LAUNCH_CBUILD(true, false);
@@ -1942,11 +2015,13 @@
         return 1;
     }
     cl->cap = ((int)(flags[2] * 1.5) + 32 + 15) / 16 * 16;
-    if (cl->cap > 65535 || nc >= (1 << 29)) {
-        amm_set_error("molecule-row list: rows longer than 65535 entries or more than 2^29 molecules are not supported");
+    if (cl->cap > 65535 || nc >= (1 << CB_CLS_SHIFT)) {
+        amm_set_error("molecule-row list: rows longer than 65535 entries or more than 2^25 molecules are not supported");
         return 1;
     }
     AMM_HIP(hipMalloc(&cl->d_nl, sizeof(int) * ns * cl->cap));
+    AMM_HIP(hipMalloc(&cl->d_nl_scratch, sizeof(int) * ns * cl->cap));
+    AMM_HIP(hipMalloc(&cl->d_lvl, sizeof(int2) * ns * (AMM_ROW_LEVELS + 1)));
     if (cluster_chain(ctx, L, cl, d_pos, 1, false, nullptr)) return 1;
     cl->built = true;
     return 0;
@@ -2059,6 +2134,17 @@
         if (pf == L && !(cl->rnear_build > 0)) {
             A.nnb = cl->d_nnb;
             A.nnb_total = nullptr;
+        }
+        A.level = nullptr;
+        A.lvl = cl->d_lvl;
+        A.lvl_stride = std::max(nrows, 1);
+        {
+            const double r_front = cl->rnear_build > 0 ? cl->rnear_build : cl->rlist_build;
+            bool ok = ctx->opt_row_cut != 0;
+            if (pf == L) ok = ok && pf->desc.rc + cl->skin <= cl->rlist_build;
+            else ok = ok && pf->desc.rc + cl->skin <= r_front;
+            if (guest) ok = ok && guest->desc.rc + cl->skin <= r_front;
+            if (ok) A.level = cl->d_flags + AMM_FLAG_LEVEL;
         }
         A.posq = pf->d_posq_s;
         A.lj = pf->d_lj_s;
@@ -2392,6 +2478,39 @@
     return 0;
 }
 
+__global__ void __launch_bounds__(256) k_clevel_sum(int nrows, const int2 *__restrict__ upto, const int *__restrict__ nnb_near, int host,
+                                                    unsigned long long *out) {
+    const int a = blockIdx.x * blockDim.x + threadIdx.x;
+    unsigned long long n = 0;
+    if (a < nrows) n = host ? (unsigned long long)(nnb_near[a] + upto[a].y) : (unsigned long long)upto[a].x;
+    for (int off = 32; off > 0; off >>= 1) n += __shfl_xor(n, off);
+    if ((threadIdx.x & 63) == 0 && n) atomicAdd(out, n);
+}
+
+int amm_cluster_level_stats_impl(amm_ctx *ctx, PairForce *pf, int *level, long long *walked) {
+    PairForce *L = pf->host ? pf->host : pf;
+    ClusterList *cl = L->cl;
+    hipStream_t st = ctx->stream;
+    int lev = 0;
+    AMM_HIP(hipMemcpyAsync(&lev, cl->d_flags + AMM_FLAG_LEVEL, sizeof(int), hipMemcpyDeviceToHost, st));
+    AMM_HIP(hipStreamSynchronize(st));
+    lev = std::min(std::max(lev, 0), AMM_ROW_LEVELS);
+    *level = lev;
+    const int nrows = cl->c_end - cl->c_begin;
+    const int at = ctx->opt_row_cut ? lev : AMM_ROW_LEVELS;
+    unsigned long long *d_out = cl->d_counters + 7;
+    AMM_HIP(hipMemsetAsync(d_out, 0, sizeof(unsigned long long), st));
+    const int host = (pf == L && cl->rnear_build > 0) ? 1 : 0;
+    if (nrows > 0)
+        hipLaunchKernelGGL(k_clevel_sum, dim3((unsigned)((nrows + 255) / 256)), dim3(256), 0, st, nrows, cl->d_lvl + (size_t)at * std::max(nrows, 1),
+                           cl->d_nnb_near, host, d_out);
+    unsigned long long h = 0;
+    AMM_HIP(hipMemcpyAsync(&h, d_out, sizeof(h), hipMemcpyDeviceToHost, st));
+    AMM_HIP(hipStreamSynchronize(st));
+    *walked = (long long)h;
+    return 0;
+}
+
 int amm_cluster_free(ClusterList *cl) {
 #ifdef AMM_CBS_TIMING
     {
@@ -2408,7 +2527,7 @@
     for (void *q : {(void *)cl->d_spec_count[0], (void *)cl->d_spec_count[1], (void *)cl->d_spec_ticket})
         if (q) (void)hipFree(q);
     if (cl->d_slice_cells) (void)hipFree(cl->d_slice_cells);
-    void *ptrs[] = {cl->d_cell_count, cl->d_cell_start, cl->d_cell_members, cl->d_cperm, cl->d_aperm, cl->d_pos4f, cl->d_xref, cl->d_nl,
+    void *ptrs[] = {cl->d_cell_count, cl->d_cell_start, cl->d_cell_members, cl->d_cperm, cl->d_aperm, cl->d_pos4f, cl->d_xref, cl->d_nl, cl->d_nl_scratch, cl->d_lvl,
                     cl->d_nnb, cl->d_nnb_near, cl->d_flags, cl->d_counters, cl->d_blockstats, cl->d_ticket};
     for (void *p : ptrs)
         if (p) (void)hipFree(p);
diff --git a/atomsmm_amd/csrc/pair.hip b/atomsmm_amd/csrc/pair.hip
--- a/atomsmm_amd/csrc/pair.hip
+++ b/atomsmm_amd/csrc/pair.hip
@@ -1982,9 +1982,9 @@
 extern "C" __attribute__((weak)) const char *amm_variant_tag(void);
 const char *amm_kernel_revision_impl() {
 #ifdef AMM_CLUSTER_TUNE
-    return "r05-epi5-tune";
+    return "r06-rowcut-tune";
 #else
-    return amm_variant_tag ? "r05-epi5-tune" : "r05-epi5";
+    return amm_variant_tag ? "r06-rowcut-tune" : "r06-rowcut";
 #endif
 }
 
diff --git a/include/atomsmm_hip.h b/include/atomsmm_hip.h
--- a/include/atomsmm_hip.h
+++ b/include/atomsmm_hip.h
@@ -175,8 +175,17 @@
     double rlist;
     int32_t shares_list;
     int32_t list_kind;
-    int64_t n_outer_builds;
-    int64_t n_outer_pairs;
+    union {
+        int64_t n_outer_builds;
+        struct {
+            int32_t row_level;
+            int32_t row_levels;
+        };
+    };
+    union {
+        int64_t n_outer_pairs;
+        int64_t n_walked_pairs;
+    };
     double rlist_outer;
     double tab_error;
     int32_t has_table;
```

After: 1043. 0.961x the previous value.
